# fgarciacardenas/SplaTAM

Hardware: AMD Instinct MI355X
Metric: rasterize fwd+bwd frames/sec @640×480, 300k Gaussians; HBM GB/s vs peak (higher is better)
Workload: dtype f32

## Files before the change

### include/gsr_glue.h

```cpp
#ifndef GSR_GLUE_H
#define GSR_GLUE_H

#include "gsr.h"

#ifdef __cplusplus
extern "C" {
#endif

int gsr_track_scratch_floats(int n);

int gsr_track_transform_fwd(int P, const float* means_world, const float* unnorm_rot, const float* logit_opac,
                            const float* log_scales, int scale_cols, const float* cam_q, const float* cam_t,
                            int q_stride, const float* w2c, float* means_cam, float* rotations, float* depth_colors,
                            float* opacities, float* scales, void* stream);

int gsr_track_transform_bwd(int P, const float* means_world, const float* unnorm_rot, int scale_cols,
                            const float* cam_q, const float* means_cam, const float* w2c,
                            const float* dL_dmeans_cam, const float* dL_drot, const float* dL_ddepth_colors,
                            float* dL_dcam_q, float* dL_dcam_t, int q_stride, float* scratch, void* stream);

typedef struct gsr_pose_track {
    const unsigned* status;
    unsigned capacity;
    const float* loss;
// ... 18 lines not shown
int gsr_track_l1_fwd_terms(int H, int W, const float* im, const float* depth_sil, const float* gt_im,
                           const float* gt_depth, float sil_thres, float w_im, float w_depth, float* loss,
                           float* terms, float* scratch, void* stream);
int gsr_track_l1_fwd_bwd_terms(int H, int W, const float* im, const float* depth_sil, const float* gt_im,
                               const float* gt_depth, float sil_thres, float w_im, float w_depth,
                               const float* dL_dloss, float* loss, float* terms, float* dL_dim, float* dL_ddepth_sil,
                               float* scratch, void* stream);

int gsr_track_l1_bwd(int H, int W, const float* im, const float* depth_sil, const float* gt_im,
                     const float* gt_depth, float sil_thres, float w_im, float w_depth, const float* dL_dloss,
                     float* dL_dim, float* dL_ddepth_sil, void* stream);

int gsr_track_forward_scratch_floats(int image_width, int image_height);
int gsr_track_forward_dual_static(const gsr_settings* settings, const gsr_gaussians* gaussians, const float* colors2,
                                  int capacity, unsigned* status, float* out_color, float* out_color2,
                                  float* out_depth, int* radii, const float* gt_im, const float* gt_depth,
                                  float sil_thres, float w_im, float w_depth, const float* dL_dloss, float* loss,
                                  float* dL_dim, float* dL_ddepth_sil, float* scratch, gsr_alloc_fn alloc,
                                  void* alloc_ctx, void* stream);
int gsr_track_forward_dual_static_terms(const gsr_settings* settings, const gsr_gaussians* gaussians,
                                        const float* colors2, int capacity, unsigned* status, float* out_color,
                                        float* out_color2, float* out_depth, int* radii, const float* gt_im,
                                        const float* gt_depth, float sil_thres, float w_im, float w_depth,
                                        const float* dL_dloss, float* loss, float* terms, float* dL_dim,
                                        float* dL_ddepth_sil, float* scratch, gsr_alloc_fn alloc, void* alloc_ctx,
                                        void* stream);

typedef struct gsr_track_xform {
    const float* means_world;
    const float* unnorm_rot;
    const float* logit_opac;
    const float* log_scales;
    int scale_cols;
    const float* cam_q;
    const float* cam_t;
    int q_stride;
    const float* w2c;
    int store_rendervars;
    const uint8_t* alive;
} gsr_track_xform;

int gsr_track_forward_dual_static_xf(const gsr_settings* settings, const gsr_gaussians* gaussians, float* colors2,
                                     const gsr_track_xform* xform, int capacity, unsigned* status, float* out_color,
                                     float* out_color2, float* out_depth, int* radii, const float* gt_im,
                                     const float* gt_depth, float sil_thres, float w_im, float w_depth,
                                     const float* dL_dloss, float* loss, float* dL_dim, float* dL_ddepth_sil,
                                     float* scratch, gsr_alloc_fn alloc, void* alloc_ctx, void* stream);
int gsr_track_forward_dual_static_xf_terms(const gsr_settings* settings, const gsr_gaussians* gaussians,
                                           float* colors2, const gsr_track_xform* xform, int capacity,
                                           unsigned* status, float* out_color, float* out_color2, float* out_depth,
                                           int* radii, const float* gt_im, const float* gt_depth, float sil_thres,
                                           float w_im, float w_depth, const float* dL_dloss, float* loss,
                                           float* terms, float* dL_dim, float* dL_ddepth_sil, float* scratch,
                                           gsr_alloc_fn alloc, void* alloc_ctx, void* stream);

int gsr_track_backward_scratch_floats(int P);
int gsr_track_backward_dual(const gsr_settings* settings, const gsr_gaussians* gaussians, const int* radii,
                            const float* colors2, const float* dL_dout_color, const float* dL_dout_color2,
                            int num_rendered, const void* geom_buffer, const void* binning_buffer,
                            const void* image_buffer, const float* means_world, const float* unnorm_rot,
                            int scale_cols, float* cam_q, float* cam_t, int q_stride, const float* w2c, double lr_q,
                            double lr_t, double beta1, double beta2, double eps, float* adam_state,
                            float* dL_dcam_q, float* dL_dcam_t, float* scratch, const gsr_pose_track* track,
                            const float* log_scales, gsr_alloc_fn alloc, void* alloc_ctx, void* stream);

int gsr_track_records_floats(int capacity);

int gsr_track_forward_backward_dual_static_xf(const gsr_settings* settings, const gsr_gaussians* gaussians,
                                              float* colors2, const gsr_track_xform* xform, int capacity,
                                              unsigned* status, float* out_color, float* out_color2,
                                              float* out_depth, int* radii, const float* gt_im,
                                              const float* gt_depth, float sil_thres, float w_im, float w_depth,
                                              const float* dL_dloss, float* loss, float* scratch,
                                              float* inst_records, gsr_alloc_fn alloc, void* alloc_ctx,
                                              void* stream);
int gsr_track_forward_backward_dual_static_xf_terms(const gsr_settings* settings, const gsr_gaussians* gaussians,
                                                    float* colors2, const gsr_track_xform* xform, int capacity,
                                                    unsigned* status, float* out_color, float* out_color2,
                                                    float* out_depth, int* radii, const float* gt_im,
                                                    const float* gt_depth, float sil_thres, float w_im,
                                                    float w_depth, const float* dL_dloss, float* loss, float* terms,
                                                    float* scratch, float* inst_records, gsr_alloc_fn alloc,
                                                    void* alloc_ctx, void* stream);
int gsr_track_backward_dual_records(const gsr_settings* settings, const gsr_gaussians* gaussians, const int* radii,
                                    const float* colors2, int num_rendered, const void* geom_buffer,
                                    const void* binning_buffer, const void* image_buffer, const float* means_world,
                                    const float* unnorm_rot, int scale_cols, float* cam_q, float* cam_t, int q_stride,
                                    const float* w2c, double lr_q, double lr_t, double beta1, double beta2,
                                    double eps, float* adam_state, float* dL_dcam_q, float* dL_dcam_t,
                                    float* scratch, const gsr_pose_track* track, const float* log_scales,
                                    const float* inst_records, gsr_alloc_fn alloc, void* alloc_ctx, void* stream);


int gsr_map_loss_scratch_floats(int H, int W);
int gsr_map_loss_state_floats(int H, int W);

int gsr_map_loss_fwd(int H, int W, const float* im, const float* depth_sil, const float* gt_im, const float* gt_depth,
                     float w_im, float w_depth, float* loss, float* state, float* scratch, void* stream);

int gsr_map_loss_bwd(int H, int W, const float* im, const float* depth_sil, const float* gt_im, const float* gt_depth,
                     float w_im, float w_depth, const float* dL_dloss, const float* state, float* dL_dim,
                     float* dL_ddepth_sil, void* stream);

int gsr_map_transform_bwd(int P, const float* unnorm_rot, const float* logit_opac, const float* log_scales,
                          int scale_cols, const float* cam_q, int q_stride, const float* means_cam, const float* w2c,
                          const float* dL_dmeans_cam, const float* dL_drot, const float* dL_ddepth_colors,
                          const float* dL_dopac, const float* dL_dscales, float* dL_dmeans, float* dL_dunnorm_rot,
                          float* dL_dlogit_opac, float* dL_dlog_scales, void* stream);

typedef struct gsr_map_adam {
    float* exp_avg[5];
    float* exp_avg_sq[5];
    double lr[5];
    int step;
    double beta1, beta2, eps;
    const unsigned* status;
    unsigned capacity;
    unsigned* halted;
} gsr_map_adam;

int gsr_backward_dual_sh_adam(const gsr_settings* settings, const gsr_gaussians* gaussians, const int* radii,
                              const float* colors2, const float* dL_dout_color, const float* dL_dout_color2,
                              int num_rendered, const void* geom_buffer, const void* binning_buffer,
                              const void* image_buffer, const gsr_grads* grads, float* dcolors2, int dl2_channels,
                              const gsr_map_adam* sh_adam, gsr_alloc_fn alloc, void* alloc_ctx, void* stream);

int gsr_map_transform_bwd_adam(int P, float* means_world, float* unnorm_rot, float* logit_opac, float* log_scales,
                               int scale_cols, float* colors, int color_cols, const float* cam_q, int q_stride,
                               const float* means_cam, const float* w2c, const float* dL_dmeans_cam,
                               const float* dL_drot, const float* dL_ddepth_colors, const float* dL_dopac,
                               const float* dL_dscales, const float* dL_dcolors, const gsr_map_adam* adam,
                               void* stream);

int gsr_map_prune(int P, const float* logit_opac, const float* log_scales, int scale_cols, float opac_thr,
                  float big_thr, int remove_big, unsigned char* alive, void* stream);
int gsr_forward_dual_static_alive(const gsr_settings* settings, const gsr_gaussians* gaussians, const float* colors2,
                                  int capacity, unsigned* status, float* out_color, float* out_color2,
                                  float* out_depth, int* radii, const unsigned char* alive, gsr_alloc_fn alloc,
                                  void* alloc_ctx, void* stream);
int gsr_forward_static_alive(const gsr_settings* settings, const gsr_gaussians* gaussians, int capacity,
                             unsigned* status, float* out_color, float* out_depth, int* radii,
                             const unsigned char* alive, gsr_alloc_fn alloc, void* alloc_ctx, void* stream);

int gsr_forward_dual_static_xf(const gsr_settings* settings, const gsr_gaussians* gaussians, float* colors2,
                               const gsr_track_xform* xform, int capacity, unsigned* status, float* out_color,
                               float* out_color2, float* out_depth, int* radii, gsr_alloc_fn alloc, void* alloc_ctx,
                               void* stream);

int gsr_accumulate_mean2d(int P, const int* radii, const float* dmeans2D, float* accum, float* denom,
                          float* max_2D_radius, void* stream);

typedef struct gsr_adam_tensor {
    float* param;
    const float* grad;
    float* exp_avg;
    float* exp_avg_sq;
    long long n;
    double lr;
} gsr_adam_tensor;
int gsr_adam_step(int n_tensors, const gsr_adam_tensor* tensors, int step, double beta1, double beta2, double eps,
                  void* stream);

int gsr_points_to_camera(int P, const float* means, const float* w2c, float* pts, void* stream);
int gsr_fisher_accumulate(int P, const float* dmeans3D, const float* dopacity, const float* weight, float* H,
                          void* stream);

// ... 52 lines not shown
```

### splatam_amd/_C.py

```python
from __future__ import annotations

import ctypes
import os
import threading
import weakref
from typing import NamedTuple

import torch

from ._lib import ALLOC_FN, GsrGaussians, GsrGrads, GsrSettings, GsrTrackXform, lib

_tls = threading.local()


def _alloc(ctx, kind, nbytes):
    try:
        t = torch.empty(max(int(nbytes), 1), dtype=torch.uint8, device=_tls.device)
        _tls.buffers[int(kind)] = t
        return t.data_ptr()
    except Exception as exc:
        _tls.alloc_error = exc
        return None


# ... 401 lines not shown
        if capacity > 0:
            _check_status(status, device)
            _check_alive(alive, P, device)
            static = (int(capacity), status.data_ptr())
            if xform is not None:
                _check_xform_outputs(device, means3D, colors2, opacity, scales, rotations)
                xf = xform_struct(xform)
                xf.store_rendervars, xf.alive = 1, _ptr(alive)
                fn, static = lib.gsr_forward_dual_static_xf, (ctypes.byref(xf),) + static
            elif alive is not None:
                fn, mask = lib.gsr_forward_dual_static_alive, (alive.data_ptr() if P else None,)
            else:
                fn = lib.gsr_forward_dual_static
        n, bufs = fr.call("rasterize_gaussians_dual", fn, _ptr(c2), *static, out_color.data_ptr(),
                          out_color2.data_ptr(), out_depth.data_ptr(), radii.data_ptr() if P else None, *mask)
        return (n, out_color, out_color2, radii, bufs[0], bufs[1], bufs[2], out_depth)


def rasterize_gaussians_dual_backward(background, means3D, radii, colors, colors2, scales, rotations, scale_modifier,
                                      cov3D_precomp, viewmatrix, projmatrix, tan_fovx, tan_fovy, dL_dout_color,
                                      dL_dout_color2, sh, degree, campos, geomBuffer, R, binningBuffer, imageBuffer,
                                      needs=None, dl2_channels=3, sh_adam=None, means2D_color1=False):
    if means2D_color1 and sh_adam is not None:
        raise ValueError("means2D_color1: gsr_backward_dual_sh_adam has no such sibling (step SH colours with "
                         "glue.FusedAdam)")
    device = means3D.device
    P = means3D.size(0)
    H, W = int(dL_dout_color.size(1)), int(dL_dout_color.size(2))
    M = sh.size(1) if (sh is not None and sh.numel() > 0 and sh.size(0) != 0) else 0
    f32 = dict(dtype=torch.float32, device=device)
    needs = [True] * 9 if needs is None else list(needs)
    needs[4] = True
    if sh_adam is not None:
        needs[6] = False
    shapes = [(P, 3), (P, 3), (P, 3), (P, 1), (P, 3), (P, 6), (P, M, 3), (P, 3), (P, 4)]
    res = [torch.empty(*sh_, **f32) if nd else None for sh_, nd in zip(shapes, needs)]
    out = [res[0], res[1], res[3], res[4], res[5], res[6], res[7], res[8]]
    dcolors2 = res[2]
    if P == 0:
        return (out[0], out[1], dcolors2, *out[2:])
    with torch.cuda.device(device):
        fr = _Frame(device, (background, viewmatrix, projmatrix, campos, tan_fovx, tan_fovy, H, W, scale_modifier,
                             degree, False), (means3D, sh, colors, None, scales, rotations, cov3D_precomp))
        c2 = _dev_f32(colors2, device, "colors2")
        dpix = _dev_f32(dL_dout_color, device, "dL_dout_color")
        dpix2 = _dev_f32(dL_dout_color2, device, "dL_dout_color2")
        radii_c = radii.to(device=device, dtype=torch.int32).contiguous()
        grads = GsrGrads(*[o.data_ptr() if (o is not None and o.numel() > 0) else None for o in out])
        fn, step = lib.gsr_backward_dual, ()
        if means2D_color1:
            if out[0] is None:
                raise ValueError("means2D_color1 needs dmeans2D among `needs`")
            grads.dmeans2D = None
            fn, step = lib.gsr_backward_dual_m2d, (out[0].data_ptr(),)
        if sh_adam is not None:
            if fr.keep_g[1] is None or fr.keep_g[1].data_ptr() != sh.data_ptr():
                raise RuntimeError("sh_adam steps the SH coefficients in place: sh must be contiguous float32")
            fn, step = lib.gsr_backward_dual_sh_adam, (ctypes.byref(sh_adam),)
        fr.call("rasterize_gaussians_dual_backward", fn, radii_c.data_ptr(), _ptr(c2), dpix.data_ptr(),
                dpix2.data_ptr(), *_forward_state(R, geomBuffer, binningBuffer, imageBuffer), ctypes.byref(grads),
                _ptr(dcolors2), int(dl2_channels), *step, release=True)
        return (out[0], out[1], dcolors2, *out[2:])


BINNING_CULLED, BINNING_REFERENCE = 0, 1


def binning_mode() -> int:
    return getattr(_tls, "binning", BINNING_CULLED)


class reference_binning:

    def __enter__(self):
        self.prev = binning_mode()
        _tls.binning = BINNING_REFERENCE
        return self

    def __exit__(self, *exc):
        _tls.binning = self.prev
        return False


def mark_visible(means3D, viewmatrix, projmatrix):
    device = means3D.device
    P = means3D.size(0)
    present = torch.zeros(P, dtype=torch.bool, device=device)
    if P == 0:
        return present
    with torch.cuda.device(device):
        m = _dev_f32(means3D, device, "means3D")
        v = _dev_f32(viewmatrix, device, "viewmatrix")
        p = _dev_f32(projmatrix, device, "projmatrix")
        rc = lib.gsr_mark_visible(P, m.data_ptr(), v.data_ptr(), p.data_ptr(), present.data_ptr(), _stream(device))
        _check(rc, "mark_visible")
    return present


def track_backward_dual(settings, means3D, radii, colors, colors2, scales, rotations, dL_dout_color, dL_dout_color2,
                        geomBuffer, R, binningBuffer, imageBuffer, means_world, unnorm_rot, scale_cols, cam_q_ptr,
                        cam_t_ptr, q_stride, w2c, scratch, adam=None, dq_ptr=None, dt_ptr=None, track=None,
                        log_scales=None, records=None):
    device = means3D.device
    with torch.cuda.device(device):
        fr = _Frame(device, _settings_of(settings, False), (means3D, None, colors, None, scales, rotations, None))
        c2 = _dev_f32(colors2, device, "colors2")
        lr_q, lr_t, b1, b2, eps, state = adam if adam is not None else (0.0, 0.0, 0.0, 0.0, 0.0, None)
        fn, what, images, rec = lib.gsr_track_backward_dual, "track_backward_dual", (), ()
        if records is not None:
            fn, what, rec = lib.gsr_track_backward_dual_records, "track_backward_dual_records", (records.data_ptr(),)
        else:
            dpix = _dev_f32(dL_dout_color, device, "dL_dout_color")
            dpix2 = _dev_f32(dL_dout_color2, device, "dL_dout_color2")
            images = (dpix.data_ptr(), dpix2.data_ptr())
        fr.call(what, fn, radii.data_ptr(), _ptr(c2), *images,
                *_forward_state(R, geomBuffer, binningBuffer, imageBuffer), means_world.data_ptr(),
                unnorm_rot.data_ptr(), int(scale_cols), cam_q_ptr, cam_t_ptr, int(q_stride), w2c.data_ptr(),
                float(lr_q), float(lr_t), float(b1), float(b2), float(eps), _ptr(state), dq_ptr, dt_ptr,
                scratch.data_ptr(), ctypes.byref(track) if track is not None else None, _ptr(log_scales), *rec,
                release=True)


def terms_ptr(terms: torch.Tensor, device) -> int:
    if (not torch.is_tensor(terms) or terms.device != device or terms.dtype != torch.float32 or
            terms.numel() != 2 or not terms.is_contiguous()):
        raise RuntimeError("terms: a contiguous float32 tensor of 2 elements on the forward's device")
    return terms.data_ptr()


def track_forward_dual_static(settings, means3D, colors, colors2, opacity, scales, rotations, capacity, status, gt_im,
                              gt_depth, sil_thres, w_im, w_depth, seed, scratch, xform=None, records=None,
                              images=True, terms=None):
    st = settings
    device = means3D.device
    P = means3D.size(0)
    H, W = int(st.image_height), int(st.image_width)
    f32 = dict(dtype=torch.float32, device=device)
    if records is not None and xform is None:
        raise RuntimeError("track_forward_dual_static: records needs the transform-fused forward (xform)")
    if not images and records is None:
        raise RuntimeError("track_forward_dual_static: images=False needs the fused render (xform and records)")
    with torch.cuda.device(device):
        fr = _Frame(device, _settings_of(st, st.prefiltered), (means3D, None, colors, opacity, scales, rotations, None))
        c2 = _dev_f32(colors2, device, "colors2")
        gi, gd, sd = (_dev_f32(gt_im, device, "gt_im"), _dev_f32(gt_depth, device, "gt_depth"),
                      _dev_f32(seed, device, "seed"))
        out_color = out_color2 = out_depth = None
        if images:
            out_color, out_color2 = torch.empty(3, H, W, **f32), torch.empty(3, H, W, **f32)
            out_depth = torch.empty(1, H, W, **f32)
        radii = torch.empty(P, dtype=torch.int32, device=device)
        loss = torch.empty((), **f32)
        _check_status(status, device)
        name, xf, dim, dds = "gsr_track_forward_dual_static", (), None, None
        if xform is not None:
            _check_xform_outputs(device, means3D, colors2, opacity, scales, rotations)
            _check_alive(xform.alive, P, device)
            xf_struct = xform_struct(xform)
            name, xf = name + "_xf", (ctypes.byref(xf_struct),)
        if records is not None:
            if (records.device != device or records.dtype != torch.float32 or not records.is_contiguous() or
                    records.numel() < lib.gsr_track_records_floats(int(capacity))):
                raise RuntimeError("records: contiguous float32 of gsr_track_records_floats(capacity) on the device")
            name = "gsr_track_forward_backward_dual_static_xf"
            tail = (scratch.data_ptr(), records.data_ptr())
        else:
            dim, dds = torch.empty(3, H, W, **f32), torch.empty(3, H, W, **f32)
            tail = (dim.data_ptr(), dds.data_ptr(), scratch.data_ptr())
        tp = () if terms is None else (terms_ptr(terms, device),)
        n, bufs = fr.call(name[4:], getattr(lib, name + "_terms" if tp else name), _ptr(c2), *xf, int(capacity),
                          status.data_ptr(), _ptr(out_color), _ptr(out_color2), _ptr(out_depth),
                          radii.data_ptr() if P else None, gi.data_ptr(), gd.data_ptr(), float(sil_thres),
                          float(w_im), float(w_depth), sd.data_ptr(), loss.data_ptr(), *tp, *tail)
        return (n, out_color, out_color2, radii, bufs[0], bufs[1], bufs[2], out_depth, loss, dim, dds)
```

### splatam_amd/_lib.py

```python
from __future__ import annotations

import ctypes
import os

_HERE = os.path.dirname(os.path.abspath(__file__))
LIB_PATH = os.environ.get("GSR_LIB", os.path.join(_HERE, "libgsr.so"))

c_int, c_float, c_void_p, c_size_t = ctypes.c_int, ctypes.c_float, ctypes.c_void_p, ctypes.c_size_t
c_double = ctypes.c_double


class GsrSettings(ctypes.Structure):
    _fields_ = [("image_height", c_int), ("image_width", c_int), ("tan_fovx", c_float), ("tan_fovy", c_float),
                ("bg", c_void_p), ("scale_modifier", c_float), ("viewmatrix", c_void_p), ("projmatrix", c_void_p),
                ("sh_degree", c_int), ("campos", c_void_p), ("prefiltered", c_int), ("binning", c_int)]


class GsrGaussians(ctypes.Structure):
    _fields_ = [("P", c_int), ("M", c_int), ("means3D", c_void_p), ("shs", c_void_p), ("colors_precomp", c_void_p),
                ("opacities", c_void_p), ("scales", c_void_p), ("rotations", c_void_p), ("cov3D_precomp", c_void_p)]


class GsrGrads(ctypes.Structure):
    _fields_ = [("dmeans2D", c_void_p), ("dcolors", c_void_p), ("dopacity", c_void_p), ("dmeans3D", c_void_p),
# ... 30 lines not shown
                             c_void_p, c_void_p, c_void_p, c_int, ctypes.POINTER(GsrGrads), ALLOC_FN, c_void_p,
                             c_void_p]),
    "gsr_forward_dual": (c_int, [ctypes.POINTER(GsrSettings), ctypes.POINTER(GsrGaussians), c_void_p, c_void_p,
                                 c_void_p, c_void_p, c_void_p, ALLOC_FN, c_void_p, c_void_p]),
    "gsr_forward_static": (c_int, [ctypes.POINTER(GsrSettings), ctypes.POINTER(GsrGaussians), c_int, c_void_p,
                                   c_void_p, c_void_p, c_void_p, ALLOC_FN, c_void_p, c_void_p]),
    "gsr_forward_dual_static": (c_int, [ctypes.POINTER(GsrSettings), ctypes.POINTER(GsrGaussians), c_void_p, c_int,
                                        c_void_p, c_void_p, c_void_p, c_void_p, c_void_p, ALLOC_FN, c_void_p,
                                        c_void_p]),
    "gsr_backward_dual": (c_int, [ctypes.POINTER(GsrSettings), ctypes.POINTER(GsrGaussians), c_void_p, c_void_p,
                                  c_void_p, c_void_p, c_int, c_void_p, c_void_p, c_void_p, ctypes.POINTER(GsrGrads),
                                  c_void_p, c_int, ALLOC_FN, c_void_p, c_void_p]),
    "gsr_backward_dual_m2d": (c_int, [ctypes.POINTER(GsrSettings), ctypes.POINTER(GsrGaussians), c_void_p, c_void_p,
                                      c_void_p, c_void_p, c_int, c_void_p, c_void_p, c_void_p,
                                      ctypes.POINTER(GsrGrads), c_void_p, c_int, c_void_p, ALLOC_FN, c_void_p,
                                      c_void_p]),
    "gsr_forward_reuse": (c_int, [ctypes.POINTER(GsrSettings), ctypes.POINTER(GsrGaussians), c_int, c_void_p,
                                  c_void_p, c_void_p, c_void_p, c_void_p, c_void_p, c_void_p, ALLOC_FN, c_void_p,
                                  c_void_p]),
    "gsr_forward_reuse_if_equal": (c_int, [ctypes.POINTER(GsrSettings), ctypes.POINTER(GsrGaussians), c_int,
                                           c_void_p, c_void_p, c_void_p, c_int, c_void_p, c_void_p, c_void_p,
                                           c_void_p, c_void_p, c_void_p, c_void_p, c_void_p, ALLOC_FN, c_void_p,
                                           c_void_p]),
    "gsr_bitwise_equal": (c_int, [c_int, c_void_p, c_void_p, c_void_p, c_void_p, c_void_p]),
    "gsr_mark_visible": (c_int, [c_int, c_void_p, c_void_p, c_void_p, c_void_p, c_void_p]),
    "gsr_geom_buffer_bytes": (c_size_t, [c_int]),
    "gsr_geom_counters_offset": (c_size_t, [c_int]),
    "gsr_binning_buffer_bytes": (c_size_t, [c_int, c_int, c_int]),
    "gsr_image_buffer_bytes": (c_size_t, [c_int, c_int]),
    "gsr_last_error": (ctypes.c_char_p, []),
    "gsr_abi_version": (c_int, []),
    "gsr_selftest_reduce9": (c_int, [c_void_p, c_void_p, c_void_p]),
    "gsr_timing_enable": (c_int, [c_int]),
    "gsr_timing_read": (c_int, [c_void_p, c_void_p, c_void_p, c_int]),
    "gsr_track_scratch_floats": (c_int, [c_int]),
    "gsr_track_transform_fwd": (c_int, [c_int, c_void_p, c_void_p, c_void_p, c_void_p, c_int, c_void_p, c_void_p,
                                        c_int, c_void_p, c_void_p, c_void_p, c_void_p, c_void_p, c_void_p, c_void_p]),
    "gsr_track_transform_bwd": (c_int, [c_int, c_void_p, c_void_p, c_int, c_void_p, c_void_p, c_void_p, c_void_p,
                                        c_void_p, c_void_p, c_void_p, c_void_p, c_int, c_void_p, c_void_p]),
    "gsr_track_transform_bwd_adam": (c_int, [c_int, c_void_p, c_void_p, c_int, c_void_p, c_void_p, c_int, c_void_p,
                                             c_void_p, c_void_p, c_void_p, c_void_p, c_double, c_double,
                                             c_double, c_double, c_double, c_void_p, c_void_p,
                                             ctypes.POINTER(GsrPoseTrack), c_void_p]),
    "gsr_track_l1_fwd": (c_int, [c_int, c_int, c_void_p, c_void_p, c_void_p, c_void_p, ctypes.c_float,
                                 ctypes.c_float, ctypes.c_float, c_void_p, c_void_p, c_void_p]),
    "gsr_track_l1_bwd": (c_int, [c_int, c_int, c_void_p, c_void_p, c_void_p, c_void_p, ctypes.c_float,
                                 ctypes.c_float, ctypes.c_float, c_void_p, c_void_p, c_void_p, c_void_p]),
    "gsr_track_l1_fwd_bwd": (c_int, [c_int, c_int, c_void_p, c_void_p, c_void_p, c_void_p, ctypes.c_float,
                                     ctypes.c_float, ctypes.c_float, c_void_p, c_void_p, c_void_p, c_void_p,
                                     c_void_p, c_void_p]),
    "gsr_track_forward_scratch_floats": (c_int, [c_int, c_int]),
    "gsr_track_forward_dual_static": (c_int, [ctypes.POINTER(GsrSettings), ctypes.POINTER(GsrGaussians), c_void_p,
                                              c_int, c_void_p, c_void_p, c_void_p, c_void_p, c_void_p, c_void_p,
                                              c_void_p, c_float, c_float, c_float, c_void_p, c_void_p, c_void_p,
                                              c_void_p, c_void_p, ALLOC_FN, c_void_p, c_void_p]),
    "gsr_track_forward_dual_static_xf": (c_int, [ctypes.POINTER(GsrSettings), ctypes.POINTER(GsrGaussians), c_void_p,
                                                 ctypes.POINTER(GsrTrackXform), c_int, c_void_p, c_void_p, c_void_p,
                                                 c_void_p, c_void_p, c_void_p, c_void_p, c_float, c_float, c_float,
                                                 c_void_p, c_void_p, c_void_p, c_void_p, c_void_p, ALLOC_FN, c_void_p,
                                                 c_void_p]),
    "gsr_track_l1_fwd_terms": (c_int, [c_int, c_int, c_void_p, c_void_p, c_void_p, c_void_p, ctypes.c_float,
                                       ctypes.c_float, ctypes.c_float, c_void_p, c_void_p, c_void_p, c_void_p]),
    "gsr_track_l1_fwd_bwd_terms": (c_int, [c_int, c_int, c_void_p, c_void_p, c_void_p, c_void_p, ctypes.c_float,
                                           ctypes.c_float, ctypes.c_float, c_void_p, c_void_p, c_void_p, c_void_p,
                                           c_void_p, c_void_p, c_void_p]),
    "gsr_track_forward_dual_static_terms": (c_int, [ctypes.POINTER(GsrSettings), ctypes.POINTER(GsrGaussians),
                                                    c_void_p, c_int, c_void_p, c_void_p, c_void_p, c_void_p, c_void_p,
                                                    c_void_p, c_void_p, c_float, c_float, c_float, c_void_p, c_void_p,
                                                    c_void_p, c_void_p, c_void_p, c_void_p, ALLOC_FN, c_void_p,
                                                    c_void_p]),
    "gsr_track_forward_dual_static_xf_terms": (c_int, [ctypes.POINTER(GsrSettings), ctypes.POINTER(GsrGaussians),
                                                       c_void_p, ctypes.POINTER(GsrTrackXform), c_int, c_void_p,
                                                       c_void_p, c_void_p, c_void_p, c_void_p, c_void_p, c_void_p,
                                                       c_float, c_float, c_float, c_void_p, c_void_p, c_void_p,
                                                       c_void_p, c_void_p, c_void_p, ALLOC_FN, c_void_p, c_void_p]),
    "gsr_track_forward_backward_dual_static_xf_terms": (c_int, [ctypes.POINTER(GsrSettings),
                                                                ctypes.POINTER(GsrGaussians), c_void_p,
                                                                ctypes.POINTER(GsrTrackXform), c_int, c_void_p,
                                                                c_void_p, c_void_p, c_void_p, c_void_p, c_void_p,
                                                                c_void_p, c_float, c_float, c_float, c_void_p,
                                                                c_void_p, c_void_p, c_void_p, c_void_p, ALLOC_FN,
                                                                c_void_p, c_void_p]),
    "gsr_track_records_floats": (c_int, [c_int]),
    "gsr_track_forward_backward_dual_static_xf": (c_int, [ctypes.POINTER(GsrSettings), ctypes.POINTER(GsrGaussians),
                                                          c_void_p, ctypes.POINTER(GsrTrackXform), c_int, c_void_p,
                                                          c_void_p, c_void_p, c_void_p, c_void_p, c_void_p, c_void_p,
                                                          c_float, c_float, c_float, c_void_p, c_void_p, c_void_p,
                                                          c_void_p, ALLOC_FN, c_void_p, c_void_p]),
    "gsr_track_backward_dual_records": (c_int, [ctypes.POINTER(GsrSettings), ctypes.POINTER(GsrGaussians), c_void_p,
                                                c_void_p, c_int, c_void_p, c_void_p, c_void_p, c_void_p, c_void_p,
                                                c_int, c_void_p, c_void_p, c_int, c_void_p, c_double, c_double,
                                                c_double, c_double, c_double, c_void_p, c_void_p, c_void_p, c_void_p,
                                                ctypes.POINTER(GsrPoseTrack), c_void_p, c_void_p, ALLOC_FN, c_void_p,
                                                c_void_p]),
    "gsr_backward_dual_sh_adam": (c_int, [ctypes.POINTER(GsrSettings), ctypes.POINTER(GsrGaussians), c_void_p,
                                          c_void_p, c_void_p, c_void_p, c_int, c_void_p, c_void_p, c_void_p,
                                          ctypes.POINTER(GsrGrads), c_void_p, c_int, ctypes.POINTER(GsrMapAdam),
                                          ALLOC_FN, c_void_p, c_void_p]),
    "gsr_track_backward_scratch_floats": (c_int, [c_int]),
    "gsr_track_backward_dual": (c_int, [ctypes.POINTER(GsrSettings), ctypes.POINTER(GsrGaussians), c_void_p, c_void_p,
                                        c_void_p, c_void_p, c_int, c_void_p, c_void_p, c_void_p, c_void_p, c_void_p,
                                        c_int, c_void_p, c_void_p, c_int, c_void_p, c_double, c_double, c_double,
                                        c_double, c_double, c_void_p, c_void_p, c_void_p, c_void_p,
                                        ctypes.POINTER(GsrPoseTrack), c_void_p, ALLOC_FN, c_void_p, c_void_p]),
    "gsr_map_loss_scratch_floats": (c_int, [c_int, c_int]),
    "gsr_map_loss_state_floats": (c_int, [c_int, c_int]),
    "gsr_map_loss_fwd": (c_int, [c_int, c_int, c_void_p, c_void_p, c_void_p, c_void_p, c_float, c_float, c_void_p,
                                 c_void_p, c_void_p, c_void_p]),
    "gsr_map_loss_bwd": (c_int, [c_int, c_int, c_void_p, c_void_p, c_void_p, c_void_p, c_float, c_float, c_void_p,
                                 c_void_p, c_void_p, c_void_p, c_void_p]),
    "gsr_map_transform_bwd": (c_int, [c_int, c_void_p, c_void_p, c_void_p, c_int, c_void_p, c_int, c_void_p,
                                      c_void_p, c_void_p, c_void_p, c_void_p, c_void_p, c_void_p, c_void_p, c_void_p,
                                      c_void_p, c_void_p, c_void_p]),
    "gsr_map_transform_bwd_adam": (c_int, [c_int, c_void_p, c_void_p, c_void_p, c_void_p, c_int, c_void_p, c_int,
                                           c_void_p, c_int, c_void_p, c_void_p, c_void_p, c_void_p, c_void_p,
                                           c_void_p, c_void_p, c_void_p, ctypes.POINTER(GsrMapAdam), c_void_p]),
    "gsr_adam_step": (c_int, [c_int, ctypes.POINTER(GsrAdamTensor), c_int, c_double, c_double, c_double, c_void_p]),
    "gsr_map_prune": (c_int, [c_int, c_void_p, c_void_p, c_int, c_float, c_float, c_int, c_void_p, c_void_p]),
    "gsr_forward_dual_static_alive": (c_int, [ctypes.POINTER(GsrSettings), ctypes.POINTER(GsrGaussians), c_void_p,
                                              c_int, c_void_p, c_void_p, c_void_p, c_void_p, c_void_p, c_void_p,
                                              ALLOC_FN, c_void_p, c_void_p]),
    "gsr_forward_static_alive": (c_int, [ctypes.POINTER(GsrSettings), ctypes.POINTER(GsrGaussians), c_int, c_void_p,
                                         c_void_p, c_void_p, c_void_p, c_void_p, ALLOC_FN, c_void_p, c_void_p]),
    "gsr_forward_dual_static_xf": (c_int, [ctypes.POINTER(GsrSettings), ctypes.POINTER(GsrGaussians), c_void_p,
                                           ctypes.POINTER(GsrTrackXform), c_int, c_void_p, c_void_p, c_void_p,
                                           c_void_p, c_void_p, ALLOC_FN, c_void_p, c_void_p]),
    "gsr_accumulate_mean2d": (c_int, [c_int, c_void_p, c_void_p, c_void_p, c_void_p, c_void_p, c_void_p]),
    "gsr_points_to_camera": (c_int, [c_int, c_void_p, c_void_p, c_void_p, c_void_p]),
    "gsr_fisher_accumulate": (c_int, [c_int, c_void_p, c_void_p, c_void_p, c_void_p, c_void_p]),
    "gsr_silhouette_count": (c_int, [ctypes.POINTER(GsrSettings), c_int, c_int, c_void_p, c_void_p, c_void_p, c_float,
                                     c_void_p, c_void_p]),
    "gsr_fisher_score_workspace_bytes": (c_size_t, []),
    "gsr_fisher_score": (c_int, [c_int, c_void_p, c_void_p, c_void_p, c_void_p, c_void_p, c_void_p, c_void_p]),
    "gsr_keyframe_workspace_bytes": (c_size_t, [c_int, c_int]),
    "gsr_keyframe_select": (c_int, [c_int, c_int, c_void_p, c_float, c_float, c_float, c_float, c_void_p, c_void_p,
                                    c_int, c_int, c_int, c_void_p, c_void_p, c_int, c_void_p, c_void_p,
                                    ctypes.c_longlong, c_int, c_void_p, c_void_p, c_void_p, c_void_p, c_void_p,
                                    c_void_p, c_void_p, c_void_p, c_void_p]),
    "gsr_eval_workspace_bytes": (c_size_t, [c_int, c_int, c_int]),
    "gsr_eval_frame": (c_int, [c_int, c_int, c_void_p, c_void_p, c_void_p, c_void_p, c_float, c_int, c_int, c_void_p,
                               c_void_p, c_void_p]),
    "gsr_densify_workspace_bytes": (c_size_t, [c_int, c_int]),
    "gsr_densify_frame": (c_int, [c_int, c_int, c_void_p, c_void_p, c_void_p, c_float, c_float, c_float, c_float,
                                  c_void_p, c_float, c_int, c_void_p, c_void_p, c_void_p, c_void_p, c_void_p,
                                  c_void_p, c_void_p, c_void_p, c_void_p, c_void_p, c_void_p, c_void_p]),
    "gsr_densify_frame_capped": (c_int, [c_int, c_int, c_void_p, c_void_p, c_void_p, c_float, c_float, c_float,
                                         c_float, c_void_p, c_float, c_int, c_void_p, c_void_p, c_void_p, c_void_p,
                                         c_void_p, c_void_p, c_void_p, c_void_p, c_void_p, c_void_p, c_void_p,
                                         c_void_p, c_int, c_float, c_float]),
    "gsr_init_frame": (c_int, [c_int, c_int, c_void_p, c_void_p, c_float, c_float, c_float, c_float, c_void_p, c_int,
                               c_void_p, c_void_p, c_void_p, c_void_p, c_void_p, c_void_p, c_void_p, c_void_p,
                               c_void_p, c_void_p, c_void_p, c_void_p]),
    "gsr_resize_frame": (c_int, [c_int, c_int, c_void_p, c_void_p, c_int, c_int, c_void_p, c_void_p, c_int, c_int,
                                 c_void_p, c_void_p, c_void_p]),
    "gsr_ingest_frame": (c_int, [c_int, c_int, c_void_p, c_void_p, c_double, c_int, c_float, c_void_p, c_void_p,
                                 c_int, c_int, c_void_p, c_void_p, c_int, c_int, c_void_p, c_void_p, c_void_p]),
}


def load(path: str = LIB_PATH) -> ctypes.CDLL:
    if not os.path.exists(path):
        raise ImportError(f"libgsr.so not found at {path}: build it with `python -m splatam_amd.build` "
                          "(no CPU fallback exists for the rasterizer)")
    lib = ctypes.CDLL(path)
    ab = os.environ.get("GSR_LIB_AB") == "1" and bool(os.environ.get("GSR_LIB"))
    for name, (res, args) in SIGNATURES.items():
# ... 16 lines not shown
```

### splatam_amd/csrc/gsr_backward.hip

```cpp
#include <cstdlib>

#include "gsr_chain.h"
#include "gsr_clock.h"
#include "gsr_diag.h"
#include "gsr_dispatch.h"
#include "gsr_glue_common.h"
#include "gsr_launch.h"
#include "gsr_layout.h"
#include "gsr_math.h"
#include "gsr_render_bwd.h"
#include "gsr_render_fwd.h"
#include "gsr_wave.h"

namespace gsr {

__global__ void __launch_bounds__(TILE_PIX, GSR_BWD_M2D_WAVES)
render_bwd_m2d_kernel(Camera cam, const uint2* __restrict__ ranges, const PointEntry* __restrict__ point_list,
                      const float4* __restrict__ rr, const uint32_t* __restrict__ blocksums,
                      const float* __restrict__ final_T, const uint32_t* __restrict__ n_contrib,
                      const float* __restrict__ dL_dpix, const float* __restrict__ dL_dpix2, float* __restrict__ inst,
                      BwdGuard guard, unsigned long long* clk) {
    using V = MapM2dVariant;
    kclock_begin(clk);
    RenderDiag dg;
    dg.begin();
    if (guard.overflow()) {
        kclock_end(clk);
        return;
    }
    __shared__ __attribute__((aligned(16))) char smem[BwdShape<V>::bytes];
    const int tid = threadIdx.x;
    const int tile = sched_tile(cam), tx = tile % cam.gx, ty = tile / cam.gx;
    dg.tile(tile);
    const int px = tx * TILE_X + tile_px(tid);
    const int py = ty * TILE_Y + tile_py(tid);
    BwdPix pin{0.f, 0u, 0.f, 0.f, 0.f, 0.f, 0.f, 0.f};
    load_bwd_pix<V::DUAL, V::Q2>(pin, cam, px, py, final_T, n_contrib, dL_dpix, dL_dpix2);
    bwd_tile<V>(cam, tile, pin, ranges, point_list, rr, blocksums, inst, guard, smem, dg);
    dg.end();
    kclock_end(clk);
}

constexpr size_t track_lds_bytes() {
    return FwdShape<true>::bytes > BwdShape<TrackVariant>::bytes ? FwdShape<true>::bytes : BwdShape<TrackVariant>::bytes;
}
template <bool IMAGES>
__global__ void __launch_bounds__(TILE_PIX, 5)
render_track_kernel(Camera cam, const uint2* __restrict__ ranges, PointEntry* __restrict__ point_list,
                    uint64_t* __restrict__ keys, const float4* __restrict__ rr, const uint32_t* __restrict__ blocksums,
                    float* __restrict__ final_T, uint32_t* __restrict__ n_contrib, float* __restrict__ out_color,
                    float* __restrict__ out_color2, float* __restrict__ out_depth, SpecGuard guard,
                    unsigned long long* clk, TrackL1 l1, float* __restrict__ inst) {
    kclock_begin(clk);
    RenderDiag dg;
    dg.begin();
    if (guard.overflow()) {
        kclock_end(clk);
        return;
    }
    __shared__ __attribute__((aligned(16))) char smem[track_lds_bytes()];
    if constexpr (!IMAGES) {
        final_T = nullptr;
        cam.rowmax = nullptr;
    }
    const int tile = sched_tile(cam);
    dg.tile(tile);
    const FwdPix f = fwd_tile<true>(cam, tile, ranges, point_list, keys, rr, guard, smem, dg);
    float grad[4];
    constexpr bool kStoreGrads = false;
    static_assert(!kStoreGrads, "render_track_kernel's callers pass no gradient images");
    fwd_epilogue<true, true, kStoreGrads>(cam, tile, f, final_T, n_contrib, out_color, out_color2, out_depth, l1,
                                          grad);
    __syncthreads();
    const BwdPix pin{f.T, f.last16 >> 4, grad[0], grad[1], grad[2], grad[3], 0.f, 0.f};
    Camera cb = cam;
    cb.rowmax = nullptr;
    bwd_tile<TrackVariant>(cb, tile, pin, ranges, point_list, rr, blocksums, inst,
                           BwdGuard{guard.counters, guard.cap_inst}, smem, dg);
    dg.end();
    kclock_end(clk);
}

int track_records_stride() { return BwdShape<TrackVariant>::RS; }

hipError_t launch_render_track(const Camera& cam, const uint2* ranges, uint64_t* point_list, uint64_t* keys,
                               GeomPtrs geo, float* final_T, uint32_t* n_contrib, float* out_color,
                               float* out_color2, float* out_depth, SpecGuard guard, const TrackL1& l1, float* inst,
                               hipStream_t s, unsigned long long* clk) {
    auto k = final_T != nullptr ? render_track_kernel<true> : render_track_kernel<false>;
    hipLaunchKernelGGL(k, dim3(cam.gx * cam.gy), dim3(TILE_PIX), 0, s, cam, ranges, point_list,
                       keys, geo.rr, geo.blocksums, final_T, n_contrib, out_color, out_color2, out_depth, guard, clk,
                       l1, inst);
    return hipGetLastError();
}

struct BwdTerms {
    bool op, c1, c2;
    int q2;
};
static BwdTerms bwd_terms(unsigned need, bool dual) {
    return {(need & NEED_OPACITY) != 0, (need & NEED_COLORS) != 0, dual && (need & NEED_COLORS2),
            (dual && (need & NEED_DL2_CH0_ONLY)) ? 1 : 3};
}

RecLayout bwd_rec_layout(unsigned need, bool dual) {
    const auto [op, c1, c2, q2] = bwd_terms(need, dual);
    return rec_sums(op, c1, c2, q2).rec;
}

using RenderBwdFn = decltype(render_bwd_of<TrackVariant>());
struct PickRenderBwd {
    template <bool DUAL, bool OP, bool C1, bool C2, bool Q1>
    RenderBwdFn operator()() const {
        if constexpr (!DUAL && (C2 || Q1)) return nullptr;
        else return render_bwd_of<BwdVariant<DUAL, OP, C1, C2, Q1 ? 1 : 3>>();
    }
};

hipError_t launch_render_bwd(const Camera& cam, const uint2* ranges, const uint64_t* point_list, GeomPtrs geo,
                             const float* final_T, const uint32_t* n_contrib, const float* dL_dpix,
                             const float* colors2, const float* dL_dpix2, unsigned need, float* inst,
                             BwdGuard guard, hipStream_t s, unsigned long long* clk) {
    const auto [op, c1, c2, q2] = bwd_terms(need, colors2 != nullptr);
    const auto k = dispatch_bools(PickRenderBwd{}, colors2 != nullptr, op, c1, c2, q2 == 1);
    hipLaunchKernelGGL(k, dim3(cam.gx * cam.gy), dim3(TILE_PIX), 0, s, cam, ranges, point_list, geo.rr, geo.blocksums,
                       final_T, n_contrib, dL_dpix, dL_dpix2, inst, guard, clk);
    return hipGetLastError();
}

int m2d_record_stride() { return BwdShape<MapM2dVariant>::RS; }
static_assert(BwdShape<MapM2dVariant>::O_M1 == M2D_REC_PAIR && BwdShape<MapM2dVariant>::NV == M2D_REC_PAIR + 2 &&
                  BwdShape<MapM2dVariant>::RS <= INST_REC_MAX,
              "the M2D1 record: the mapping variant's ten sums, then the pair");

hipError_t launch_render_bwd_m2d(const Camera& cam, const uint2* ranges, const uint64_t* point_list, GeomPtrs geo,
                                 const float* final_T, const uint32_t* n_contrib, const float* dL_dpix,
                                 const float* dL_dpix2, float* inst, BwdGuard guard, hipStream_t s,
                                 unsigned long long* clk) {
    hipLaunchKernelGGL(render_bwd_m2d_kernel, dim3(cam.gx * cam.gy), dim3(TILE_PIX), 0, s, cam, ranges, point_list,
                       geo.rr, geo.blocksums, final_T, n_contrib, dL_dpix, dL_dpix2, inst, guard, clk);
    return hipGetLastError();
}

template <bool POSE, bool SHL, bool M2D1 = false>
__device__ __forceinline__ void gauss_bwd_body(Camera cam, GaussIn g, GeomPtrs geo, const int* __restrict__ radii,
                                               const float* __restrict__ inst, RecLayout rec, GradsOut out,
                                               BwdGuard guard, PoseFuse pf, M2dOut m1 = M2dOut{}) {
    static_assert(!M2D1 || !POSE, "M2D1: the mapping backward only");
    if constexpr (!SHL) {
        g.shs = nullptr;
        g.M = 0;
    }
    const int i = blockIdx.x * blockDim.x + threadIdx.x;
    if (!POSE && i >= g.P) return;
    const bool live = i < g.P;
    const int nsh = g.shs ? (cam.sh_degree + 1) * (cam.sh_degree + 1) : 0;
    float g2[9] = {0.f, 0.f, 0.f, 0.f, 0.f, 0.f, 0.f, 0.f, 0.f};
    float dcol2[3] = {0.f, 0.f, 0.f};
    [[maybe_unused]] float m2d1[2] = {0.f, 0.f};
    float dmean[3] = {0.f, 0.f, 0.f}, dcov[6] = {0.f, 0.f, 0.f, 0.f, 0.f, 0.f}, dscale[3] = {0.f, 0.f, 0.f},
          drot[4] = {0.f, 0.f, 0.f, 0.f};
    float dsh[48];
#pragma unroll
    for (int k = 0; k < 48; k++) dsh[k] = 0.f;
    GaussGeom gg;
    gg.m = make_float3(0.f, 0.f, 0.f);
    gg.s = make_float3(0.f, 0.f, 0.f);
    gg.q = make_float4(0.f, 0.f, 0.f, 0.f);
    const int rad = live ? radii[i] : 0;
    const bool xf_geom = POSE && pf.ls;
    TrackXf x;
    x.mw = pf.means_world; x.ur = pf.unnorm_rot; x.ls = pf.ls; x.scols = pf.scols;
    XfRaw xr{};
    if (xf_geom && live) xr = track_xform_load(x, i, false);
    uint32_t off = 0, cnt = 0, tl = 0xFFFFFFFFu;
    if (POSE && live && rad > 0) {
        off = geo.offsets[i];
        cnt = geo.tiles[i];
        tl = reinterpret_cast<const uint32_t*>(geo.bin)[4 * (size_t)i + 3];
    }
    __shared__ Pose s_pose;
    if constexpr (POSE) {
        if (pf.ls || pf.scols != 1) {
            if (threadIdx.x == 0) s_pose = make_pose(pf.cam_q, pf.cam_t, pf.qs);
            __syncthreads();
        }
    }
    if (live && (POSE || rad > 0)) {
        if (xf_geom) {
            const Pose ps = s_pose;
            float m[3], sv[3];
            track_xform_geom_raw(xr, x.scols, ps, m, gg.q, sv);
            gg.m = make_float3(m[0], m[1], m[2]);
            gg.s = make_float3(sv[0], sv[1], sv[2]);
        } else {
            gg = load_geom(g, i);
        }
    }
    if (live && rad > 0 && !guard.overflow()) {
        if (!POSE) {
            off = geo.offsets[i];
            cnt = geo.tiles[i];
            tl = reinterpret_cast<const uint32_t*>(geo.bin)[4 * (size_t)i + 3];
        }
        float acc[INST_REC_MAX];
#pragma unroll
        for (int m = 0; m < INST_REC_MAX; m++) acc[m] = 0.f;
        const int np = rec.stride / 2;
        constexpr int RU = 4;
// ... 258 lines not shown
```

### splatam_amd/csrc/gsr_binning.hip

```cpp
#include "gsr_clock.h"
#include "gsr_dispatch.h"
#include "gsr_launch.h"
#include "gsr_layout.h"
#include "gsr_wave.h"

namespace gsr {

constexpr int SCAN_THREADS = 1024;
constexpr int SCAN_ITEMS = 4;

template <bool AGENT_TILES>
__device__ void scan_counts_body(const uint32_t* __restrict__ wgsum, uint32_t* __restrict__ blocksums, uint32_t nb,
                                 const uint32_t* __restrict__ tile_count, uint32_t tile_stride, uint32_t ntiles,
                                 uint2* __restrict__ ranges, uint32_t* __restrict__ counters, uint32_t sort_cap,
                                 uint32_t* __restrict__ status) {
    __shared__ uint32_t wsums[SCAN_THREADS / 64];
    __shared__ uint32_t s_carry, s_max, s_viol;
    const int tid = threadIdx.x, lane = tid & 63, w = tid >> 6;
    if (tid == 0) s_viol = 0;
    for (int pass = 0; pass < 2; pass++) {
        const uint32_t n = pass == 0 ? nb : ntiles;
        const uint32_t* src = pass == 0 ? wgsum : tile_count;
        if (tid == 0) { s_carry = 0; s_max = 0; }
        __syncthreads();
        uint32_t vmax = 0, viol = 0;
        for (uint32_t base = 0; base < n; base += SCAN_THREADS * SCAN_ITEMS) {
            uint32_t x[SCAN_ITEMS], sum = 0;
            const uint32_t i0 = base + (uint32_t)tid * SCAN_ITEMS;
#pragma unroll
            for (int k = 0; k < SCAN_ITEMS; k++) {
                const uint32_t* ps = src + (size_t)(i0 + k) * (pass == 0 ? 1u : tile_stride);
                x[k] = (i0 + k < n) ? ((AGENT_TILES && pass == 1) ? ld_agent(ps) : *ps) : 0u;
                if (pass == 0) {
                    viol |= x[k] >> 31;
                    x[k] &= 0x7fffffffu;
                }
                sum += x[k];
                vmax = max(vmax, x[k]);
            }
            uint32_t incl = wave_incl_scan(sum);
            if (lane == 63) wsums[w] = incl;
            __syncthreads();
            if (w == 0) {
                uint32_t ws = (lane < SCAN_THREADS / 64) ? wsums[lane] : 0u;
                uint32_t wi = wave_incl_scan(ws);
                if (lane < SCAN_THREADS / 64) wsums[lane] = wi - ws;
            }
            __syncthreads();
            uint32_t run = s_carry + wsums[w] + incl - sum;
#pragma unroll
            for (int k = 0; k < SCAN_ITEMS; k++) {
                if (i0 + k < n) {
                    if (pass == 0) blocksums[i0 + k] = run;
                    else ranges[i0 + k] = make_uint2(run, run + x[k]);
                }
                run += x[k];
            }
            __syncthreads();
            if (tid == SCAN_THREADS - 1) s_carry = run;
            __syncthreads();
        }
        atomicMax(&s_max, vmax);
        if (viol) atomicOr(&s_viol, 1u);
        __syncthreads();
        if (tid == 0) {
            if (pass == 0) {
                counters[0] = s_carry;
                counters[1] = s_viol;
                if (status) status_merge(status, s_carry, s_viol, 0u, 0u);
            } else {
                counters[2] = s_max;
                counters[3] = sort_cap;
                if (status) status_merge(status, 0u, 0u, s_max, sort_cap);
            }
        }
        __syncthreads();
    }
}

__global__ void __launch_bounds__(SCAN_THREADS)
scan_counts_kernel(const uint32_t* __restrict__ wgsum, uint32_t* __restrict__ blocksums, uint32_t nb,
                   const uint32_t* __restrict__ tile_count,
                   uint32_t tile_stride, uint32_t ntiles, uint2* __restrict__ ranges,
                   uint32_t* __restrict__ counters, uint32_t sort_cap, uint32_t* __restrict__ status) {
    scan_counts_body<false>(wgsum, blocksums, nb, tile_count, tile_stride, ntiles, ranges, counters, sort_cap, status);
}
// ... 31 lines not shown
    const bool in_regs = rq <= CS_RQ;
    if (t < ntiles) {
        if (in_regs) {
#pragma unroll
            for (int k = 0; k < CS_RQ; k++) {
                vals[k] = b0 + k < b1 ? counts[(size_t)(b0 + k) * ntiles + t] : 0u;
                sum += vals[k];
            }
        } else {
#pragma unroll 4
            for (int b = b0; b < b1; b++) sum += counts[(size_t)b * ntiles + t];
        }
    }
    s_part[q][tl] = sum;
    __syncthreads();
    {
        static_assert(CS_PARTS == 64 || CS_PARTS == 32, "one or two tile columns per wave");
        constexpr int CPW = 64 / CS_PARTS;
        const int w = threadIdx.x >> 6, lane = threadIdx.x & 63;
        const int part = lane % CS_PARTS, colw = CPW * w + lane / CS_PARTS;
        const uint32_t v = s_part[part][colw];
        uint32_t inc = wave_incl_scan(v);
        if (CPW == 2) {
            const uint32_t lo_tot = (uint32_t)__shfl((int)inc, 31);
            if (lane >= 32) inc -= lo_tot;
        }
        s_part[part][colw] = inc - v;
    }
    __syncthreads();
    uint32_t run = s_part[q][tl];
    if (t < ntiles) {
        if (in_regs) {
#pragma unroll
            for (int k = 0; k < CS_RQ; k++)
                if (b0 + k < b1) {
                    counts[(size_t)(b0 + k) * ntiles + t] = run;
                    run += vals[k];
                }
        } else {
#pragma unroll 4
            for (int b = b0; b < b1; b++) {
                const uint32_t v = counts[(size_t)b * ntiles + t];
                counts[(size_t)b * ntiles + t] = run;
                run += v;
            }
        }
        if (q == CS_PARTS - 1) {
            if (TAIL) st_agent(&tot[t], run);
            else tot[t] = run;
        }
    }
    if (!TAIL) return;
    if (!last_block_arrive(&geo.counters[4])) return;
    scan_counts_body<true>(geo.wgsum, geo.blocksums, (uint32_t)nb, tot, 1u, (uint32_t)ntiles, ranges, geo.counters,
                           sort_cap, status);
}
template <bool TAIL, int CT, bool CLK>
__global__ void __launch_bounds__(CS_THREADS)
tile_colscan_kernel(uint32_t* __restrict__ counts, int nb, int ntiles, uint32_t* __restrict__ tot, GeomPtrs geo,
                    uint2* __restrict__ ranges, uint32_t sort_cap, uint32_t* __restrict__ status,
                    unsigned long long* clk, Gate gate) {
    if (gate.off()) return;
    if constexpr (CLK) kclock_begin(clk);
    tile_colscan_body<TAIL, CT>(counts, nb, ntiles, tot, geo, ranges, sort_cap, status);
    if constexpr (CLK) kclock_end(clk);
}

struct PickTileColscan {
    template <bool TAIL, bool WIDE, bool CLK>
    auto operator()() const { return &tile_colscan_kernel<TAIL, WIDE ? 32 : 16, CLK>; }
};

hipError_t launch_tile_colscan(uint32_t* counts, int nb, int ntiles, uint32_t* tot, GeomPtrs geo, uint2* ranges,
                               uint32_t* status, bool tail, hipStream_t s, unsigned long long* clk, Gate gate) {
    static_assert(CS_THREADS == SCAN_THREADS, "the last colscan workgroup runs the scan body");
    const bool wide = nb > CS_ROWS_SMALL;
    const int ct = wide ? 32 : 16;
    const auto k = dispatch_bools(PickTileColscan{}, tail, wide, clk != nullptr);
    hipLaunchKernelGGL(k, dim3((ntiles + ct - 1) / ct), dim3(CS_THREADS), 0, s, counts, nb, ntiles, tot, geo, ranges,
                       (uint32_t)TILE_SORT_CAP, status, clk, gate);
    return hipGetLastError();
}

constexpr int PLAN_BUCKETS = 1024, PLAN_SHIFT = 2;
__device__ __forceinline__ uint32_t plan_bucket(uint32_t len) {
    return (uint32_t)(PLAN_BUCKETS - 1) - min(len >> PLAN_SHIFT, (uint32_t)(PLAN_BUCKETS - 1));
}
__device__ __forceinline__ uint32_t plan_slot(uint32_t p, uint32_t n, uint32_t ncu) {
    const uint32_t q = n / ncu, m = n - q * ncu, heavy = q * (ncu - m);
    const bool hv = p < heavy;
    const uint32_t g0 = hv ? m : 0u, gs = hv ? ncu - m : m, pp = hv ? p : p - heavy;
    const uint32_t rd = pp / gs, k = pp - rd * gs;
    return rd * ncu + g0 + ((rd & 1u) ? gs - 1u - k : k);
}
template <int NT, int TPT = 0>
__device__ void tile_plan(const uint32_t* __restrict__ tot, int ntiles, int ncu, uint32_t* __restrict__ order,
                          uint32_t* s_hist, uint32_t* s_wsum, const uint32_t* tv = nullptr, int t0 = 0,
                          int t1 = 0) {
    constexpr int BPT = PLAN_BUCKETS / NT;
    static_assert(BPT * NT == PLAN_BUCKETS, "buckets per thread");
    const int tid = threadIdx.x, lane = tid & 63, w = tid >> 6;
#pragma unroll
    for (int k = 0; k < BPT; k++) s_hist[tid * BPT + k] = 0u;
    __syncthreads();
    if constexpr (TPT > 0) {
#pragma unroll
        for (int k = 0; k < TPT; k++)
            if (t0 + k < t1) atomicAdd(&s_hist[plan_bucket(tv[k])], 1u);
    } else {
        for (int u = tid; u < ntiles; u += NT) atomicAdd(&s_hist[plan_bucket(tot[u])], 1u);
    }
    __syncthreads();
    uint32_t c[BPT], cs = 0;
#pragma unroll
    for (int k = 0; k < BPT; k++) {
        c[k] = s_hist[tid * BPT + k];
        cs += c[k];
    }
    const uint32_t incl = wave_incl_scan(cs);
    if (lane == 63) s_wsum[w] = incl;
    __syncthreads();
    uint32_t run = incl - cs;
    for (int k = 0; k < w; k++) run += s_wsum[k];
#pragma unroll
    for (int k = 0; k < BPT; k++) {
        s_hist[tid * BPT + k] = run;
        run += c[k];
    }
    __syncthreads();
    if constexpr (TPT > 0) {
#pragma unroll
        for (int k = 0; k < TPT; k++)
            if (t0 + k < t1) {
                const uint32_t p = atomicAdd(&s_hist[plan_bucket(tv[k])], 1u);
                order[plan_slot(p, (uint32_t)ntiles, (uint32_t)ncu)] = (uint32_t)(t0 + k);
            }
    } else {
        for (int u = tid; u < ntiles; u += NT) {
            const uint32_t p = atomicAdd(&s_hist[plan_bucket(tot[u])], 1u);
            order[plan_slot(p, (uint32_t)ntiles, (uint32_t)ncu)] = (uint32_t)u;
        }
    }
}

__global__ void identity_order_kernel(uint32_t* __restrict__ order, int n) {
    const int i = blockIdx.x * blockDim.x + threadIdx.x;
    if (i < n) order[i] = (uint32_t)i;
}
hipError_t launch_identity_order(uint32_t* order, int ntiles, hipStream_t s) {
    if (ntiles <= 0) return hipSuccess;
    hipLaunchKernelGGL(identity_order_kernel, dim3((ntiles + 255) / 256), dim3(256), 0, s, order, ntiles);
    return hipGetLastError();
}

constexpr int DUP_T = 512;
#ifndef GSR_DUP_LOOP_MAX
#define GSR_DUP_LOOP_MAX 16
#endif
__device__ __forceinline__ void store_host_snap(uint32_t* snap, uint4 lo, uint4 hi) {
    reinterpret_cast<uint4*>(snap)[0] = lo;
    reinterpret_cast<uint4*>(snap)[1] = hi;
}
__device__ __forceinline__ void dup_gate_off_snap(const Camera& cam, const GeomPtrs& geo) {
    if (cam.host_snap && blockIdx.x == 0 && threadIdx.x == 0)
        store_host_snap(cam.host_snap, *reinterpret_cast<const uint4*>(geo.counters),
                        *reinterpret_cast<const uint4*>(geo.counters + 4));
}
template <bool LDS_HIST, int DUP_G, bool EXACT>
__device__ __forceinline__ void duplicate_bucket_body(Camera cam, int P, GeomPtrs geo, uint2* __restrict__ ranges,
                                                      const uint32_t* __restrict__ tot, uint32_t* __restrict__ cursor,
                                                      int ntiles, uint64_t* __restrict__ keys,
                                                      uint64_t* __restrict__ point_list, SpecGuard guard,
                                                      uint32_t sort_cap, uint32_t* __restrict__ status,
                                                      uint32_t* __restrict__ s_cur) {
    constexpr int ROW = DUP_G * DUP_T;
    __shared__ uint32_t s_incl[ROW];
    __shared__ uint32_t s_x0[ROW], s_y0[ROW], s_w[ROW], s_depth[ROW], s_live[ROW];
    __shared__ uint32_t s_cx[EXACT ? ROW : 1];
    __shared__ uint32_t wsum[DUP_T / 64], s_tmax[DUP_T / 64], s_cws[DUP_T / 64];
    __shared__ uint32_t s_cred[2][DUP_T / 64];
    const int tid = threadIdx.x, lane = tid & 63, w = tid >> 6;
    const int i0 = blockIdx.x * ROW + DUP_G * tid;
    uint32_t t[DUP_G];
    uint4 r[DUP_G];
#pragma unroll
    for (int g = 0; g < DUP_G; g++) {
        t[g] = (i0 + g < P) ? geo.tiles[i0 + g] : 0u;
        r[g] = (i0 + g < P) ? geo.bin[i0 + g] : make_uint4(0u, 0u, 0u, 0u);
    }
    uint32_t base, ctail = 0, ltot = 0xFFFFFFFFu;
    if (LDS_HIST) {
        constexpr int TPT = 4;
        __shared__ uint32_t s_red[5][DUP_T / 64];
        const uint32_t b = blockIdx.x, nb = gridDim.x;
        const int per = (ntiles + DUP_T - 1) / DUP_T;
        const int t0 = min(ntiles, tid * per), t1 = min(ntiles, t0 + per);
        const bool in_regs = per <= TPT;
        uint32_t tv[TPT], cv[TPT];
#pragma unroll
        for (int k = 0; k < TPT; k++) {
            const bool ok = in_regs && t0 + k < t1;
            tv[k] = ok ? tot[t0 + k] : 0u;
            cv[k] = ok ? cursor[(size_t)b * ntiles + t0 + k] : 0u;
        }
        uint32_t pre = 0, all = 0, viol = 0, vmax = 0, cpre = 0, call = 0;
        for (uint32_t k = tid; k < nb; k += 2 * DUP_T) {
            const uint32_t k2 = k + DUP_T;
            const uint32_t v = geo.wgsum[k], v2 = k2 < nb ? geo.wgsum[k2] : 0u;
            const uint32_t c = EXACT ? geo.wgcull[k] : 0u, c2 = (EXACT && k2 < nb) ? geo.wgcull[k2] : 0u;
            viol |= (v | v2) >> 31;
            all += (v & 0x7fffffffu) + (v2 & 0x7fffffffu);
            pre += (k < b ? (v & 0x7fffffffu) : 0u) + (k2 < b ? (v2 & 0x7fffffffu) : 0u);
            if (EXACT) {
                call += c + c2;
                cpre += (k < b ? c : 0u) + (k2 < b ? c2 : 0u);
            }
        }
        uint32_t csum = 0;
        if (in_regs) {
#pragma unroll
            for (int k = 0; k < TPT; k++) {
                csum += tv[k];
                vmax = max(vmax, tv[k]);
            }
        } else {
            for (int u = t0; u < t1; u++) {
                const uint32_t v = tot[u];
// ... 254 lines not shown
```

### splatam_amd/csrc/gsr_capi.hip

```cpp
#include <cstdio>
#include <cstdlib>
#include <cstring>
#include <algorithm>
#include <atomic>
#include <string>

#include "../../include/gsr.h"
#include "../../include/gsr_glue.h"
#include "gsr_adam.h"
#include "gsr_errors.h"
#include "gsr_host.h"
#include "gsr_launch.h"
#include "gsr_layout.h"

using namespace gsr;

namespace {
thread_local std::string g_last_error;

__global__ void zero_words_kernel(uint32_t* __restrict__ p, size_t n) {
    for (size_t k = blockIdx.x * (size_t)blockDim.x + threadIdx.x; k < n; k += (size_t)gridDim.x * blockDim.x) p[k] = 0u;
}
std::atomic<int> g_cus[kMaxDevices];
}

namespace gsr {
int fail(int code, const std::string& msg) {
    g_last_error = msg;
    return code;
}

int hip_fail(hipError_t e, const char* where) {
    return fail(GSR_ERR_HIP, std::string(where) + ": " + hipGetErrorString(e));
}

int check_terms(const char* entry, const float* terms) {
    if (!terms) return fail(GSR_ERR_INVALID_ARG, std::string(entry) + ": null terms");
    if ((uintptr_t)terms % sizeof(float) != 0)
        return fail(GSR_ERR_INVALID_ARG, std::string(entry) + ": terms must be 4-byte aligned");
    return GSR_OK;
}

int stream_device(hipStream_t s) {
    thread_local hipStream_t last_s = nullptr;
    thread_local int last_d = -1;
    if (last_d >= 0 && s == last_s && s != nullptr) return last_d;
    int d = 0;
    if (hipStreamGetDevice(s, &d) != hipSuccess && hipGetDevice(&d) != hipSuccess) d = 0;
    (void)hipGetLastError();
    if (d < 0 || d >= kMaxDevices) d = 0;
    last_s = s;
    last_d = d;
    return d;
}
int current_device() {
    int d = 0;
    if (hipGetDevice(&d) != hipSuccess || d < 0 || d >= kMaxDevices) d = 0;
    return d;
}
int device_cus(int dev) {
    int n = g_cus[dev].load(std::memory_order_relaxed);
    if (n > 0) return n;
    if (hipDeviceGetAttribute(&n, hipDeviceAttributeMultiprocessorCount, dev) != hipSuccess || n <= 0) n = 256;
    (void)hipGetLastError();
    g_cus[dev].store(n, std::memory_order_relaxed);
    return n;
}
hipError_t zero_async(void* p, size_t bytes, hipStream_t s) {
    const size_t n = bytes / 4;
    if (n == 0) return hipSuccess;
    const unsigned blocks = (unsigned)std::min<size_t>(1024, (n + 255) / 256);
    hipLaunchKernelGGL(zero_words_kernel, dim3(blocks), dim3(256), 0, s, (uint32_t*)p, n);
    return hipGetLastError();
}
int geom_pre_shift(int P) { return pre_shift_for(P, device_cus(current_device())); }
int current_device_cus() { return device_cus(current_device()); }
}

namespace {

struct Pinned {
    uint32_t* p = nullptr;
    uint32_t* dp = nullptr;
    hipEvent_t ev = nullptr;
    ~Pinned() {
        if (p) (void)hipHostFree(p);
        if (ev) (void)hipEventDestroy(ev);
    }
    int ensure(int dev) {
        hipError_t e;
        if (!p) {
            if ((e = hipHostMalloc((void**)&p, 32,
                                   hipHostMallocMapped | hipHostMallocCoherent | hipHostMallocPortable)) != hipSuccess)
                return hip_fail(e, "hipHostMalloc");
            if ((e = hipHostGetDevicePointer((void**)&dp, p, 0)) != hipSuccess)
// ... 33 lines not shown
    c.bg = s->bg;
    c.scale_modifier = s->scale_modifier;
    c.sh_degree = s->sh_degree;
    c.prefiltered = s->prefiltered;
    return c;
}

GaussIn make_gauss(const gsr_gaussians* g) {
    GaussIn o;
    o.P = g->P;
    o.M = g->shs ? g->M : 0;
    o.means3D = g->means3D;
    o.shs = (g->shs && g->M > 0) ? g->shs : nullptr;
    o.colors = g->colors_precomp;
    o.opacities = g->opacities;
    o.scales = g->scales;
    o.rotations = g->rotations;
    o.cov3D = g->cov3D_precomp;
    o.colors2 = nullptr;
    o.sh_staged = 0;
    o.alive = nullptr;
    return o;
}

int validate(const gsr_settings* s, const gsr_gaussians* g, bool forward) {
    if (!s || !g) return fail(GSR_ERR_INVALID_ARG, "null settings or gaussians");
    if (g->P < 0) return fail(GSR_ERR_INVALID_ARG, "P must be >= 0");
    if (s->binning != GSR_BINNING_CULLED && s->binning != GSR_BINNING_REFERENCE)
        return fail(GSR_ERR_INVALID_ARG, "settings.binning must be GSR_BINNING_CULLED or GSR_BINNING_REFERENCE");
    if (s->image_width <= 0 || s->image_height <= 0) return fail(GSR_ERR_INVALID_ARG, "image size must be positive");
    if (s->image_width > 16 * 65535 || s->image_height > 16 * 65535)
        return fail(GSR_ERR_INVALID_ARG, "image too large for 16-bit tile coordinates");
    if (g->P == 0) return GSR_OK;
    if (!g->means3D) return fail(GSR_ERR_INVALID_ARG, "means3D is required");
    if (forward && !g->opacities) return fail(GSR_ERR_INVALID_ARG, "opacities are required");
    if (!s->viewmatrix || !s->projmatrix || !s->bg) return fail(GSR_ERR_INVALID_ARG, "camera matrices / bg missing");
    const bool has_sh = g->shs && g->M > 0;
    if (!g->colors_precomp && !has_sh)
        return fail(GSR_ERR_INVALID_ARG, "Please provide excatly one of either SHs or precomputed colors!");
    if (!g->colors_precomp && !s->campos) return fail(GSR_ERR_INVALID_ARG, "campos required for SH colours");
    if (has_sh && (s->sh_degree < 0 || s->sh_degree > 3 || (s->sh_degree + 1) * (s->sh_degree + 1) > g->M))
        return fail(GSR_ERR_INVALID_ARG, "sh_degree must be in [0,3] with (deg+1)^2 <= M");
    const bool has_sr = g->scales && g->rotations;
    if (!has_sr && !g->cov3D_precomp)
        return fail(GSR_ERR_INVALID_ARG,
                    "Please provide exactly one of either scale/rotation pair or precomputed 3D covariance!");
    return GSR_OK;
}

template <class T>
int obtain(gsr_alloc_fn alloc, void* ctx, int kind, size_t bytes, const char* what, T** out) {
    *out = (T*)alloc(ctx, kind, bytes);
    return *out ? GSR_OK : fail(GSR_ERR_ALLOC, std::string("allocator returned NULL (") + what + ")");
}

struct ReuseIn {
    EqualPairs pairs;
    int prev_num_rendered;
    const void* prev_geom;
    void* prev_binning;
    void* prev_image;
    const int* prev_radii;
    int* reused;
};

struct FwdCall {
    const gsr_settings* settings = nullptr;
    const gsr_gaussians* gaussians = nullptr;
    const float* colors2 = nullptr;
    float* out_color = nullptr;
    float* out_color2 = nullptr;
    float* out_depth = nullptr;
    int* radii = nullptr;
    gsr_alloc_fn alloc = nullptr;
    void* alloc_ctx = nullptr;
    void* stream = nullptr;
    int capacity = 0;
    uint32_t* status = nullptr;
    const TrackL1* l1 = nullptr;
    const TrackXf* xf = nullptr;
    float* track_inst = nullptr;
    const uint8_t* alive = nullptr;
    const ReuseIn* reuse = nullptr;
};

FwdCall fwd_call(const gsr_settings* settings, const gsr_gaussians* gaussians, float* out_color, float* out_depth,
                 int* radii, gsr_alloc_fn alloc, void* alloc_ctx, void* stream) {
    FwdCall c;
    c.settings = settings; c.gaussians = gaussians;
    c.out_color = out_color; c.out_depth = out_depth; c.radii = radii;
    c.alloc = alloc; c.alloc_ctx = alloc_ctx; c.stream = stream;
    return c;
}
FwdCall& dual(FwdCall& c, const float* colors2, float* out_color2) {
    c.colors2 = colors2; c.out_color2 = out_color2;
    return c;
}
FwdCall& statics(FwdCall& c, int capacity, uint32_t* status) {
    c.capacity = capacity; c.status = status;
    return c;
}

bool stores_no_images(const FwdCall& c) { return c.track_inst && !c.out_color && !c.out_color2 && !c.out_depth; }

int check_forward(const FwdCall& c) {
    const int rc = validate(c.settings, c.gaussians, true);
    if (c.track_inst && (!c.l1 || !c.colors2 || c.capacity <= 0))
        return fail(GSR_ERR_INVALID_ARG, "the fused render backward needs the static dual forward with the L1 loss");
    if (rc != GSR_OK) return rc;
    if (!c.alloc) return fail(GSR_ERR_INVALID_ARG, "allocator callback required");
    if (!stores_no_images(c)) {
        if (!c.out_color || !c.out_depth) return fail(GSR_ERR_INVALID_ARG, "output image pointers required");
        if (c.colors2 && !c.out_color2) return fail(GSR_ERR_INVALID_ARG, "out_color2 required with colors2");
    }
    if (c.colors2 && c.gaussians->P > 0 && !c.gaussians->means3D)
        return fail(GSR_ERR_INVALID_ARG, "means3D is required");
    return GSR_OK;
}

struct Forward {
    const FwdCall& c;
    hipStream_t stream;
    int dev;
    Pinned& pin;
    Camera cam;
    GaussIn g;
    int P, W, H, ntiles;
    GeomLayout GL;
    ImgLayout IL;
    void* geom = nullptr;
    GeomPtrs geo{};
    ImgPtrs img{};
    uint32_t* cursor = nullptr;
    bool lds_hist;
    uint32_t* cmat = nullptr;
    uint32_t* tile_tot = nullptr;
    bool force_radix;
    bool scan_in_duplicate;
    bool eager;
    bool gated = false;
    Gate eq_gate;
    uint32_t epoch = 0;
    uint32_t cap = 0;

    static bool force_radix_env() {
        static const bool on = getenv("GSR_FORCE_RADIX") && atoi(getenv("GSR_FORCE_RADIX")) != 0;
        return on;
    }
    explicit Forward(const FwdCall& call)
        : c(call), stream((hipStream_t)call.stream), dev(stream_device(stream)), pin(g_pinned[dev]),
          cam(make_camera(call.settings)), g(make_gauss(call.gaussians)), P(g.P), W(cam.W), H(cam.H),
          ntiles(cam.gx * cam.gy), GL(GeomLayout::make(P)), IL(ImgLayout::make(W, H)),
          lds_hist(ntiles <= MAX_LDS_TILES), force_radix(force_radix_env() && call.capacity <= 0),
          scan_in_duplicate(lds_hist && !force_radix), eager(call.capacity <= 0) {
        g.colors2 = c.colors2;
        g.alive = c.alive;
        if (c.xf) g.xf = *c.xf;
        cam.pre_shift = GL.shift;
        cam.cull = c.settings->binning != GSR_BINNING_REFERENCE ? 1 : 0;
        cam.tail_exact = eager ? 1 : 0;
    }
    uint32_t* status() const { return eager ? nullptr : c.status; }
    template <class T>
    int obtain(int kind, size_t bytes, const char* what, T** out) {
        return ::obtain(c.alloc, c.alloc_ctx, kind, bytes, what, out);
    }
// ... 53 lines not shown
            return hip_fail(e, "geometry comparison");
        cam.gate = Gate{word, epoch, 1u};
        eq_gate = Gate{word, epoch, 0u};
        if ((e = launch_reuse_copy(eq_gate, c.reuse->prev_geom, geom, GL.counters, GL.tiles, g.colors,
                                   c.reuse->prev_radii, c.radii, P, stream)) != hipSuccess)
            return hip_fail(e, "geometry reuse");
        return GSR_OK;
    }

    int snapshot_counters(bool stored_by_kernel) {
        if (int rc = pin.ensure(dev)) return rc;
        hipError_t e;
        if (!stored_by_kernel &&
            (e = hipMemcpyAsync(pin.p, geo.counters, 32, hipMemcpyDeviceToHost, stream)) != hipSuccess)
            return hip_fail(e, "copy num_rendered");
        if ((e = hipEventRecord(pin.ev, stream)) != hipSuccess) return hip_fail(e, "record num_rendered");
        return GSR_OK;
    }

    int counts_and_ranges() {
        hipError_t e;
        if (!scan_in_duplicate && (e = launch_identity_order(img.order, ntiles, stream)) != hipSuccess)
            return hip_fail(e, "render schedule");
        if (!c.radii) return fail(GSR_ERR_INVALID_ARG, "radii output required");
        {
            StageTimer t(GSR_STAGE_PREPROCESS, P, stream, true);
            if (sh_staged(cam, g)) {
                if ((e = launch_sh_eval(cam, g, geo, stream)) != hipSuccess) return hip_fail(e, "sh_eval");
                g.sh_staged = 1;
            }
            if ((e = launch_preprocess(cam, g, geo, c.radii, lds_hist ? cmat : img.tile_count, lds_hist, ntiles,
                                       GL.nb, stream, t.kclock())) != hipSuccess)
                return hip_fail(e, "preprocess");
        }
        {
            StageTimer t(GSR_STAGE_RANGES, ntiles, stream, lds_hist);
            if (lds_hist) {
                if ((e = launch_tile_colscan(cmat, GL.nb, ntiles, tile_tot, geo, img.ranges, status(),
                                             !scan_in_duplicate, stream, t.kclock(), cam.gate)) != hipSuccess)
                    return hip_fail(e, "tile count scan");
            } else if ((e = launch_scan_counts(geo, GL.nb, img.tile_count, TILE_CTR_STRIDE, ntiles, img.ranges,
                                               status(), stream)) != hipSuccess) {
                return hip_fail(e, "scan");
            }
        }
        if (eager && !scan_in_duplicate) return snapshot_counters(false);
        return GSR_OK;
    }

    int render(const BinPtrs& bin, uint64_t* keys, const SpecGuard& guard, long long units) {
        StageTimer t(GSR_STAGE_RENDER_FWD, units, stream, true);
        hipError_t e;
        if (c.track_inst) {
            if ((e = launch_render_track(cam, img.ranges, bin.point_list, keys, geo,
                                         stores_no_images(c) ? nullptr : img.final_T, img.n_contrib, c.out_color,
                                         c.out_color2, c.out_depth, guard, *c.l1, c.track_inst, stream,
                                         t.kclock())) != hipSuccess)
                return hip_fail(e, "render (fused tracking forward + backward)");
        } else if ((e = launch_render_fwd(cam, img.ranges, bin.point_list, keys, geo, c.colors2, img.final_T,
                                          img.n_contrib, c.out_color, c.out_color2, c.out_depth, guard, stream,
                                          t.kclock(), c.l1)) != hipSuccess) {
            return hip_fail(e, "render");
        }
        return GSR_OK;
    }

    int duplicate_render(const BinPtrs& bin, const SpecGuard& guard, uint32_t* host_snap, bool snapshot,
                         long long units) {
        Camera cplan = cam;
        cplan.tile_order_out = scan_in_duplicate ? img.order : nullptr;
        cplan.host_snap = host_snap;
        {
            StageTimer t(GSR_STAGE_DUPLICATE, P, stream, true);
            hipError_t e = launch_duplicate_bucket(cplan, P, geo, img.ranges, tile_tot, lds_hist ? cmat : cursor,
                                                   lds_hist, ntiles, bin.keys[0], bin.point_list, GL.nb, guard,
                                                   status(), stream, t.kclock());
            if (e != hipSuccess) return hip_fail(e, "duplicate");
        }
        if (snapshot)
            if (int rc = snapshot_counters(host_snap != nullptr)) return rc;
        return render(bin, bin.keys[0], guard, units);
    }

    int speculate() {
        void* buf;
        if (int rc = obtain(GSR_BUF_BINNING, BinLayout::make((int)cap, W, H).total, "binning buffer", &buf)) return rc;
        const BinPtrs bin = BinPtrs::at(buf, BinLayout::make((int)cap, W, H));
        const bool snapshot = eager && scan_in_duplicate;
        const bool dup_snap = snapshot && !g_snap_copy;
        if (dup_snap)
            if (int rc = pin.ensure(dev)) return rc;
        const SpecGuard guard{geo.counters, cap, (uint32_t)TILE_SORT_CAP};
        if (int rc = duplicate_render(bin, guard, dup_snap ? pin.dp : nullptr, snapshot, 0)) return rc;
        if (gated) {
            Camera cr = cam;
            cr.gate = eq_gate;
            const ImgPtrs prev = ImgPtrs::at(c.reuse->prev_image, IL);
            bind_schedule(cr, prev, dev);
            const SpecGuard rg{geo.counters, (uint32_t)c.reuse->prev_num_rendered, 0xFFFFFFFFu};
            hipError_t e = launch_render_fwd(cr, prev.ranges, (uint64_t*)c.reuse->prev_binning, nullptr, geo, nullptr,
                                             prev.final_T, prev.n_contrib, c.out_color, nullptr, c.out_depth, rg,
                                             stream);
            if (e != hipSuccess) return hip_fail(e, "render (geometry reuse)");
        }
        return GSR_OK;
    }

    int radix_binning(const BinPtrs& bin, const BinLayout& BL, uint32_t I) {
        hipError_t e;
        if ((e = hipMemsetD32Async((hipDeviceptr_t)(geo.counters + 3), 0xffffffffu, 1, stream)) != hipSuccess)
            return hip_fail(e, "sort path flag");
        {
            StageTimer t(GSR_STAGE_DUPLICATE, P, stream);
            if ((e = launch_duplicate(cam, P, geo, bin.keys[0], bin.gid, GL.nb, stream)) != hipSuccess)
                return hip_fail(e, "duplicate");
        }
        {
            StageTimer t(GSR_STAGE_SORT, I, stream);
            uint64_t* keys[2] = {bin.keys[0], bin.keys[1]};
            uint32_t* vals[2] = {bin.vals[0], bin.vals[1]};
            if ((e = launch_radix_sort(keys, vals, bin.hist, I, BL.nsb, BL.npass, stream)) != hipSuccess)
                return hip_fail(e, "radix sort");
        }
        StageTimer t(GSR_STAGE_RANGES, I, stream);
        if ((e = launch_gather_ids(bin.vals[BL.final_buf], bin.gid, bin.point_list, I, stream)) != hipSuccess)
            return hip_fail(e, "gather ids");
        return GSR_OK;
    }

    int wait_and_finish() {
        hipError_t e;
        if ((e = hipEventSynchronize(pin.ev)) != hipSuccess) return hip_fail(e, "sync num_rendered");
        if (gated && pin.p[5] != epoch) {
            *c.reuse->reused = 1;
            return c.reuse->prev_num_rendered;
        }
        const uint32_t I = pin.p[0];
        const uint32_t longest = pin.p[2];
        if (pin.p[1] != 0)
            return fail(GSR_ERR_PREFILTERED, "Point is filtered although prefiltered is set. This shouldn't happen!");
        if (I > 0x7fffffffu) return fail(GSR_ERR_INVALID_ARG, "num_rendered overflows int32");
        g_inst_ratio[dev].v.store(std::max(0.05, (double)I / P), std::memory_order_relaxed);
        if (!force_radix && I <= cap && longest <= (uint32_t)TILE_SORT_CAP) {
            g_timing_units(dev, GSR_STAGE_SORT, I);
            g_timing_units(dev, GSR_STAGE_RENDER_FWD, I);
            return (int)I;
        }
        const BinLayout BL = BinLayout::make((int)I, W, H);
        void* buf;
        if (int rc = obtain(GSR_BUF_BINNING, BL.total, "binning buffer", &buf)) return rc;
        const BinPtrs bin = BinPtrs::at(buf, BL);
        const SpecGuard none{geo.counters, 0xffffffffu, 0xffffffffu};
        int rc;
        if (I > 0 && longest <= (uint32_t)TILE_SORT_CAP && !force_radix) {
            rc = duplicate_render(bin, none, nullptr, false, I);
        } else {
            rc = I > 0 ? radix_binning(bin, BL, I) : GSR_OK;
            if (rc == GSR_OK) rc = render(bin, nullptr, none, I);
        }
        return rc != GSR_OK ? rc : (int)I;
    }
};

int forward_impl(const FwdCall& c) {
    if (int rc = check_forward(c)) return rc;
    Forward F(c);
    if (int rc = F.setup_buffers()) return rc;
    if (F.P == 0) return F.empty_map();
    int rc;
    if ((rc = F.gate_on_comparison()) != GSR_OK || (rc = F.counts_and_ranges()) != GSR_OK) return rc;
    const double ratio = g_inst_ratio[F.dev].v.load(std::memory_order_relaxed);
    F.cap = F.eager ? (uint32_t)std::min(2.0e9, std::max(1024.0, 1.5 * ratio * F.P)) : (uint32_t)c.capacity;
    if (!F.force_radix && (rc = F.speculate()) != GSR_OK) return rc;
    if (!F.eager) return (int)F.cap;
    return F.wait_and_finish();
}

struct BwdCall {
    const gsr_settings* settings = nullptr;
    const gsr_gaussians* gaussians = nullptr;
    const int* radii = nullptr;
    const float* dL_dout_color = nullptr;
    const float* colors2 = nullptr;
    const float* dL_dout_color2 = nullptr;
    int num_rendered = 0;
    const void* geom_buffer = nullptr;
    const void* binning_buffer = nullptr;
    const void* image_buffer = nullptr;
    int power = 1;
    const gsr_grads* grads = nullptr;
    float* dcolors2 = nullptr;
    int dl2_channels = 3;
    gsr_alloc_fn alloc = nullptr;
    void* alloc_ctx = nullptr;
    void* stream = nullptr;
    const PoseFuse* pose = nullptr;
    const ShAdam* sh_adam = nullptr;
    const float* pre_inst = nullptr;
    float* dmeans2D_c1 = nullptr;
};

BwdCall bwd_call(const gsr_settings* settings, const gsr_gaussians* gaussians, const int* radii, int num_rendered,
                 const void* geom_buffer, const void* binning_buffer, const void* image_buffer) {
    BwdCall c;
    c.settings = settings; c.gaussians = gaussians; c.radii = radii; c.num_rendered = num_rendered;
    c.geom_buffer = geom_buffer; c.binning_buffer = binning_buffer; c.image_buffer = image_buffer;
    return c;
}
BwdCall& on(BwdCall& c, gsr_alloc_fn alloc, void* alloc_ctx, void* stream) {
    c.alloc = alloc; c.alloc_ctx = alloc_ctx; c.stream = stream;
    return c;
}

struct Backward {
    const BwdCall& c;
    hipStream_t stream;
    Camera cam;
    GaussIn g;
    int P, R;
    GeomPtrs geo{};
    ImgPtrs img{};
    const uint64_t* point_list = nullptr;
    GradsOut out;
    BwdGuard guard{};

    explicit Backward(const BwdCall& call)
        : c(call), stream((hipStream_t)call.stream), cam(make_camera(call.settings)),
          g(make_gauss(call.gaussians)), P(g.P), R(call.num_rendered),
          out{c.grads->dmeans2D, c.grads->dcolors, c.grads->dopacity, c.grads->dmeans3D,
              c.grads->dcov3D,   c.grads->dsh,     c.grads->dscales,  c.grads->drotations} {}

    void bind_forward_state() {
        const GeomLayout GL = GeomLayout::make(P);
        cam.pre_shift = GL.shift;
        geo = GeomPtrs::at(const_cast<void*>(c.geom_buffer), GL);
        img = ImgPtrs::at(const_cast<void*>(c.image_buffer), ImgLayout::make(cam.W, cam.H));
        bind_schedule(cam, img, current_device());
        if (c.binning_buffer)
            point_list = (const uint64_t*)((const char*)c.binning_buffer + BinLayout::make(R, cam.W, cam.H).point_list);
        guard = BwdGuard{geo.counters, (uint32_t)R};
    }

    int power_scratch(size_t bytes, char** scratch) {
        *scratch = nullptr;
        if (R > 0 && !c.binning_buffer) return fail(GSR_ERR_INVALID_ARG, "missing binning buffer");
        if (!c.alloc) return fail(GSR_ERR_INVALID_ARG, "allocator callback required");
        if (bytes == 0) return GSR_OK;
        return obtain(c.alloc, c.alloc_ctx, GSR_BUF_SCRATCH, bytes, "backward scratch", scratch);
    }

    int fisher() {
// ... 340 lines not shown
    return track_forward_static(
        fwd_call(settings, gaussians, out_color, out_depth, radii, alloc, alloc_ctx, stream), colors2, out_color2,
        capacity, status,
        TrackL1{gt_im, gt_depth, sil_thres, w_im, w_depth, dL_dloss, dL_dim, dL_ddepth_sil, scratch, loss, nullptr});
}

int gsr_track_forward_dual_static_terms(const gsr_settings* settings, const gsr_gaussians* gaussians,
                                        const float* colors2, int capacity, unsigned* status, float* out_color,
                                        float* out_color2, float* out_depth, int* radii, const float* gt_im,
                                        const float* gt_depth, float sil_thres, float w_im, float w_depth,
                                        const float* dL_dloss, float* loss, float* terms, float* dL_dim,
                                        float* dL_ddepth_sil, float* scratch, gsr_alloc_fn alloc, void* alloc_ctx,
                                        void* stream) {
    if (int rc = check_terms("track_forward_dual_static_terms", terms)) return rc;
    return track_forward_static(
        fwd_call(settings, gaussians, out_color, out_depth, radii, alloc, alloc_ctx, stream), colors2, out_color2,
        capacity, status,
        TrackL1{gt_im, gt_depth, sil_thres, w_im, w_depth, dL_dloss, dL_dim, dL_ddepth_sil, scratch, loss, terms});
}

int gsr_track_forward_dual_static_xf(const gsr_settings* settings, const gsr_gaussians* gaussians, float* colors2,
                                     const gsr_track_xform* xform, int capacity, unsigned* status, float* out_color,
                                     float* out_color2, float* out_depth, int* radii, const float* gt_im,
                                     const float* gt_depth, float sil_thres, float w_im, float w_depth,
                                     const float* dL_dloss, float* loss, float* dL_dim, float* dL_ddepth_sil,
                                     float* scratch, gsr_alloc_fn alloc, void* alloc_ctx, void* stream) {
    FwdCall c = fwd_call(settings, gaussians, out_color, out_depth, radii, alloc, alloc_ctx, stream);
    statics(dual(c, colors2, out_color2), capacity, status);
    return track_forward_xf(c, xform,
                            TrackL1{gt_im, gt_depth, sil_thres, w_im, w_depth, dL_dloss, dL_dim, dL_ddepth_sil,
                                    scratch, loss, nullptr});
}

int gsr_track_forward_dual_static_xf_terms(const gsr_settings* settings, const gsr_gaussians* gaussians,
                                           float* colors2, const gsr_track_xform* xform, int capacity,
                                           unsigned* status, float* out_color, float* out_color2, float* out_depth,
                                           int* radii, const float* gt_im, const float* gt_depth, float sil_thres,
                                           float w_im, float w_depth, const float* dL_dloss, float* loss,
                                           float* terms, float* dL_dim, float* dL_ddepth_sil, float* scratch,
                                           gsr_alloc_fn alloc, void* alloc_ctx, void* stream) {
    if (int rc = check_terms("track_forward_dual_static_xf_terms", terms)) return rc;
    FwdCall c = fwd_call(settings, gaussians, out_color, out_depth, radii, alloc, alloc_ctx, stream);
    statics(dual(c, colors2, out_color2), capacity, status);
    return track_forward_xf(c, xform,
                            TrackL1{gt_im, gt_depth, sil_thres, w_im, w_depth, dL_dloss, dL_dim, dL_ddepth_sil,
                                    scratch, loss, terms});
}

int gsr_track_records_floats(int capacity) { return track_records_stride() * (capacity > 1 ? capacity : 1); }

static int track_forward_backward_xf(FwdCall c, float* colors2, float* out_color2, const gsr_track_xform* xform,
                                     int capacity, unsigned* status, float* inst_records, const TrackL1& l1) {
    if (!inst_records) return fail(GSR_ERR_INVALID_ARG, "track_forward_backward_dual_static_xf: null records");
    statics(dual(c, colors2, out_color2), capacity, status).track_inst = inst_records;
    return track_forward_xf(c, xform, l1);
}

int gsr_track_forward_backward_dual_static_xf(const gsr_settings* settings, const gsr_gaussians* gaussians,
                                              float* colors2, const gsr_track_xform* xform, int capacity,
                                              unsigned* status, float* out_color, float* out_color2,
                                              float* out_depth, int* radii, const float* gt_im,
                                              const float* gt_depth, float sil_thres, float w_im, float w_depth,
                                              const float* dL_dloss, float* loss, float* scratch,
                                              float* inst_records, gsr_alloc_fn alloc, void* alloc_ctx,
                                              void* stream) {
    return track_forward_backward_xf(
        fwd_call(settings, gaussians, out_color, out_depth, radii, alloc, alloc_ctx, stream), colors2, out_color2,
        xform, capacity, status, inst_records,
        TrackL1{gt_im, gt_depth, sil_thres, w_im, w_depth, dL_dloss, nullptr, nullptr, scratch, loss, nullptr});
}

int gsr_track_forward_backward_dual_static_xf_terms(const gsr_settings* settings, const gsr_gaussians* gaussians,
                                                    float* colors2, const gsr_track_xform* xform, int capacity,
                                                    unsigned* status, float* out_color, float* out_color2,
                                                    float* out_depth, int* radii, const float* gt_im,
                                                    const float* gt_depth, float sil_thres, float w_im,
                                                    float w_depth, const float* dL_dloss, float* loss, float* terms,
                                                    float* scratch, float* inst_records, gsr_alloc_fn alloc,
                                                    void* alloc_ctx, void* stream) {
    if (int rc = check_terms("track_forward_backward_dual_static_xf_terms", terms)) return rc;
    return track_forward_backward_xf(
        fwd_call(settings, gaussians, out_color, out_depth, radii, alloc, alloc_ctx, stream), colors2, out_color2,
        xform, capacity, status, inst_records,
        TrackL1{gt_im, gt_depth, sil_thres, w_im, w_depth, dL_dloss, nullptr, nullptr, scratch, loss, terms});
}

int gsr_forward_reuse(const gsr_settings* settings, const gsr_gaussians* gaussians, int num_rendered,
                      const void* prev_geom, void* binning_buffer, void* image_buffer, const int* prev_radii,
                      float* out_color, float* out_depth, int* radii, gsr_alloc_fn alloc, void* alloc_ctx,
                      void* stream_) {
    int rc = validate(settings, gaussians, true);
    if (rc != GSR_OK) return rc;
    if (!alloc) return fail(GSR_ERR_INVALID_ARG, "allocator callback required");
    if (!gaussians->colors_precomp || (gaussians->shs && gaussians->M > 0))
        return fail(GSR_ERR_INVALID_ARG, "geometry reuse needs precomputed colours (no SH)");
    if (gaussians->P <= 0 || num_rendered < 0 || !prev_geom || !binning_buffer || !image_buffer || !prev_radii ||
        !out_color || !out_depth || !radii)
        return fail(GSR_ERR_INVALID_ARG, "geometry reuse needs the previous call's state and the outputs");
    hipStream_t stream = (hipStream_t)stream_;
    const int dev = stream_device(stream);
    Camera cam = make_camera(settings);
    const GaussIn g = make_gauss(gaussians);
    const int P = g.P;
    const GeomLayout GL = GeomLayout::make(P);
    cam.pre_shift = GL.shift;
    void* geom;
    if ((rc = obtain(alloc, alloc_ctx, GSR_BUF_GEOM, GL.total, "geom buffer", &geom)) != GSR_OK) return rc;
    const GeomPtrs geo = GeomPtrs::at(geom, GL);
    const ImgPtrs img = ImgPtrs::at(image_buffer, ImgLayout::make(cam.W, cam.H));
    bind_schedule(cam, img, dev);
    hipError_t e;
    {
        StageTimer t(GSR_STAGE_PREPROCESS, P, stream);
        if ((e = hipMemcpyAsync(geom, prev_geom, GL.total, hipMemcpyDeviceToDevice, stream)) != hipSuccess ||
            (e = hipMemcpyAsync(radii, prev_radii, sizeof(int) * (size_t)P, hipMemcpyDeviceToDevice, stream)) !=
                hipSuccess)
            return hip_fail(e, "copy previous geometry");
        if ((e = launch_recolour(P, g.colors, geo, stream)) != hipSuccess) return hip_fail(e, "recolour");
    }
    const SpecGuard guard{geo.counters, (uint32_t)num_rendered, 0xFFFFFFFFu};
    StageTimer t(GSR_STAGE_RENDER_FWD, num_rendered, stream, true);
    if ((e = launch_render_fwd(cam, img.ranges, (uint64_t*)binning_buffer, nullptr, geo, nullptr, img.final_T,
                               img.n_contrib, out_color, nullptr, out_depth, guard, stream, t.kclock())) != hipSuccess)
        return hip_fail(e, "render");
    return num_rendered;
}

int gsr_forward_reuse_if_equal(const gsr_settings* settings, const gsr_gaussians* gaussians, int npairs,
                               const float* const* a, const float* const* b, const long long* n,
                               int prev_num_rendered, const void* prev_geom, void* prev_binning, void* prev_image,
                               const int* prev_radii, float* out_color, float* out_depth, int* radii, int* reused,
                               gsr_alloc_fn alloc, void* alloc_ctx, void* stream) {
    if (!gaussians || !gaussians->colors_precomp || (gaussians->shs && gaussians->M > 0) || gaussians->cov3D_precomp)
        return fail(GSR_ERR_INVALID_ARG, "geometry reuse needs precomputed colours (no SH, no cov3D)");
    if (npairs < 1 || npairs > 8 || !a || !b || !n || !reused)
        return fail(GSR_ERR_INVALID_ARG, "gsr_forward_reuse_if_equal: 1..8 pairs and `reused`");
    if (prev_num_rendered < 0 || !prev_geom || !prev_binning || !prev_image || !prev_radii)
        return fail(GSR_ERR_INVALID_ARG, "geometry reuse needs the previous call's state");
    ReuseIn r{};
    r.pairs.npairs = npairs;
    for (int k = 0; k < npairs; k++) {
        if (n[k] < 0 || (n[k] > 0 && (!a[k] || !b[k])))
            return fail(GSR_ERR_INVALID_ARG, "gsr_forward_reuse_if_equal: pair");
        r.pairs.a[k] = a[k];
        r.pairs.b[k] = b[k];
        r.pairs.n[k] = n[k];
    }
    r.prev_num_rendered = prev_num_rendered;
    r.prev_geom = prev_geom;
    r.prev_binning = prev_binning;
    r.prev_image = prev_image;
    r.prev_radii = prev_radii;
    r.reused = reused;
    FwdCall c = fwd_call(settings, gaussians, out_color, out_depth, radii, alloc, alloc_ctx, stream);
    c.reuse = &r;
    return forward_impl(c);
}

int gsr_bitwise_equal(int npairs, const float* const* a, const float* const* b, const long long* n, int* flag,
                      void* stream) {
    if (npairs < 0 || npairs > 8 || (npairs > 0 && (!a || !b || !n)) || !flag)
        return fail(GSR_ERR_INVALID_ARG, "gsr_bitwise_equal: 0..8 pairs and a flag");
    EqualPairs q{};
    q.npairs = npairs;
    for (int k = 0; k < npairs; k++) {
        if (n[k] < 0 || (n[k] > 0 && (!a[k] || !b[k]))) return fail(GSR_ERR_INVALID_ARG, "gsr_bitwise_equal: pair");
// ... 125 lines not shown
```

### splatam_amd/csrc/gsr_forward.hip

```cpp
#include "gsr_clock.h"
#include "gsr_diag.h"
#include "gsr_launch.h"
#include "gsr_layout.h"
#include "gsr_render_fwd.h"
#include "gsr_wave.h"

namespace gsr {

template <bool DUAL, bool L1 = false>
__global__ void __launch_bounds__(TILE_PIX, 5)
render_fwd_kernel(Camera cam, const uint2* __restrict__ ranges, PointEntry* __restrict__ point_list,
                  uint64_t* __restrict__ keys, const float4* __restrict__ rr, float* __restrict__ final_T, uint32_t* __restrict__ n_contrib,
                  float* __restrict__ out_color, float* __restrict__ out_color2, float* __restrict__ out_depth,
                  SpecGuard guard, unsigned long long* clk, TrackL1 l1) {
    static_assert(DUAL || !L1, "the tracking loss needs the depth / silhouette colour set");
    if (cam.gate.off()) return;
    kclock_begin(clk);
    RenderDiag dg;
    dg.begin();
    if (guard.overflow()) {
        kclock_end(clk);
        return;
    }
    __shared__ __attribute__((aligned(16))) char smem[FwdShape<DUAL>::bytes];
    const int tile = sched_tile(cam);
    dg.tile(tile);
    const FwdPix f = fwd_tile<DUAL>(cam, tile, ranges, point_list, keys, rr, guard, smem, dg);
    float g[4];
    fwd_epilogue<DUAL, L1, true>(cam, tile, f, final_T, n_contrib, out_color, out_color2, out_depth, l1, g);
    dg.phase(5);
    dg.end();
    kclock_end(clk);
}

#if GSR_PHASE
extern "C" int gsr_diag_phase_fwd(unsigned long long* host) {
    if (hipMemcpyFromSymbol(host, HIP_SYMBOL(g_phase), sizeof(g_phase), 0, hipMemcpyDeviceToHost) != hipSuccess)
        return -1;
    const unsigned long long z[8] = {0, 0, 0, 0, 0, 0, 0, 0};
    return hipMemcpyToSymbol(HIP_SYMBOL(g_phase), z, sizeof(z), 0, hipMemcpyHostToDevice) == hipSuccess ? 0 : -1;
}
#endif
#if GSR_WGTIME
extern "C" int gsr_diag_wgtime_fwd(unsigned long long* host, int n) {
    const size_t bytes = sizeof(unsigned long long) * 4 * (size_t)(n < GSR_WGTIME_MAX ? n : GSR_WGTIME_MAX);
    return hipMemcpyFromSymbol(host, HIP_SYMBOL(g_wgtime), bytes, 0, hipMemcpyDeviceToHost) == hipSuccess ? 0 : -1;
}
#endif

int track_l1_fused_scratch_floats(int ntiles) { return 2 * ntiles + ARRIVE_GROUPED_WORDS; }

hipError_t launch_render_fwd(const Camera& cam, const uint2* ranges, uint64_t* point_list,
                             uint64_t* keys, GeomPtrs geo,
                             const float* colors2, float* final_T, uint32_t* n_contrib, float* out_color,
                             float* out_color2, float* out_depth, SpecGuard guard, hipStream_t s,
                             unsigned long long* clk, const TrackL1* l1) {
    auto k = colors2 ? (l1 ? render_fwd_kernel<true, true> : render_fwd_kernel<true, false>)
                     : render_fwd_kernel<false, false>;
    hipLaunchKernelGGL(k, dim3(cam.gx * cam.gy), dim3(TILE_PIX), 0, s, cam, ranges, point_list, keys,
                       geo.rr, final_T,
                       n_contrib, out_color, out_color2, out_depth, guard, clk, l1 ? *l1 : TrackL1{});
    return hipGetLastError();
}

}
```

### splatam_amd/csrc/gsr_launch.h

```cpp
#pragma once
#include "gsr_adam.h"
#include "gsr_layout.h"

namespace gsr {

hipError_t launch_preprocess(const Camera& cam, const GaussIn& g, GeomPtrs geo, int* radii, uint32_t* counts,
                             bool lds_hist, int ntiles, int nb, hipStream_t s, unsigned long long* clk = nullptr);
hipError_t launch_mark_visible(int P, const float* means3D, const float* view, uint8_t* vis, hipStream_t s);
hipError_t launch_tile_colscan(uint32_t* counts, int nb, int ntiles, uint32_t* tot, GeomPtrs geo, uint2* ranges,
                               uint32_t* status, bool tail, hipStream_t s, unsigned long long* clk = nullptr,
                               Gate gate = Gate{});
hipError_t launch_scan_counts(GeomPtrs geo, int nb, const uint32_t* tile_count, int tile_stride, int ntiles,
                              uint2* ranges, uint32_t* status, hipStream_t s);
hipError_t launch_identity_order(uint32_t* order, int ntiles, hipStream_t s);
hipError_t launch_duplicate_bucket(const Camera& cam, int P, GeomPtrs geo, uint2* ranges, const uint32_t* tot,
                                   uint32_t* cursor, bool lds_hist, int ntiles, uint64_t* keys, uint64_t* point_list,
                                   int nb, SpecGuard guard, uint32_t* status, hipStream_t s, unsigned long long* clk = nullptr);
hipError_t launch_duplicate(const Camera& cam, int P, GeomPtrs geo, uint64_t* keys, uint32_t* gid,
                            int nb, hipStream_t s);
hipError_t launch_radix_sort(uint64_t* keys[2], uint32_t* vals[2], uint32_t* hist, uint32_t n, int nsb, int npass,
                             hipStream_t s);
hipError_t launch_gather_ids(const uint32_t* vals, const uint32_t* gid, uint64_t* point_list, uint32_t n, hipStream_t s);
struct TrackL1 {
    const float* gt_im;
    const float* gt_depth;
    float sil_thres, w_im, w_depth;
    const float* seed;
    float* dL_dim;
    float* dL_dds;
    float* scratch;
    float* loss;
    float* terms;
};
int track_l1_fused_scratch_floats(int ntiles);
hipError_t launch_render_fwd(const Camera& cam, const uint2* ranges, uint64_t* point_list, uint64_t* keys,
                             GeomPtrs geo, const float* colors2, float* final_T, uint32_t* n_contrib,
                             float* out_color, float* out_color2, float* out_depth, SpecGuard guard, hipStream_t s,
                             unsigned long long* clk = nullptr, const TrackL1* l1 = nullptr);
hipError_t launch_recolour(int P, const float* colors, GeomPtrs geo, hipStream_t s, Gate gate = Gate{});
hipError_t launch_reuse_copy(Gate gate, const void* prev_geom, void* geom, size_t geom_bytes, size_t tiles_offset,
                             const float* colors, const int* prev_radii, int* radii, int P, hipStream_t s);
struct EqualPairs {
    int npairs;
    const float* a[8];
    const float* b[8];
    long long n[8];
};
hipError_t launch_epoch_mismatch(const EqualPairs& q, uint32_t* word, uint32_t e, hipStream_t s);
hipError_t launch_bitwise_equal(const EqualPairs& q, int* flag, hipStream_t s);
hipError_t launch_render_track(const Camera& cam, const uint2* ranges, uint64_t* point_list, uint64_t* keys,
                               GeomPtrs geo, float* final_T, uint32_t* n_contrib, float* out_color,
                               float* out_color2, float* out_depth, SpecGuard guard, const TrackL1& l1, float* inst,
                               hipStream_t s, unsigned long long* clk = nullptr);
int track_records_stride();
struct RecLayout {
    int stride;
    int o_op, o_c1, o_c2, n_c2;
};
struct RecSums {
    RecLayout rec;
    int o_col;
    int o_m1;
    int nv;
};
constexpr RecSums rec_sums(bool op, bool c1, bool c2, int q2, bool m2d = false) {
    RecSums s{};
    int nv = 5;
    s.rec.o_op = op ? nv : -1;
    nv += op ? 1 : 0;
    s.o_col = nv;
    s.rec.o_c1 = c1 ? nv : -1;
    nv += c1 ? 3 : 0;
    s.rec.o_c2 = c2 ? nv : -1;
    s.rec.n_c2 = c2 ? q2 : 0;
    nv += s.rec.n_c2;
    s.o_m1 = m2d ? nv : -1;
    nv += m2d ? 2 : 0;
    s.nv = nv;
    s.rec.stride = (nv + 1) & ~1;
    return s;
}
static_assert(rec_sums(true, true, true, 3).rec.stride == INST_REC_MAX && rec_sums(true, true, true, 1, true).nv == INST_REC_MAX,
              "INST_REC_MAX: the largest records, every sum of a dual render and the M2D1 form");
RecLayout bwd_rec_layout(unsigned need, bool dual);
hipError_t launch_render_bwd(const Camera& cam, const uint2* ranges, const uint64_t* point_list, GeomPtrs geo,
                             const float* final_T, const uint32_t* n_contrib, const float* dL_dpix,
                             const float* colors2, const float* dL_dpix2, unsigned need, float* inst, BwdGuard guard,
                             hipStream_t s, unsigned long long* clk = nullptr);
constexpr unsigned NEED_OPACITY = 1u, NEED_COLORS = 2u, NEED_COLORS2 = 4u;
constexpr unsigned NEED_DL2_CH0_ONLY = 8u;
struct GradsOut {
    float* dmeans2D;
    float* dcolors;
    float* dopacity;
    float* dmeans3D;
    float* dcov3D;
    float* dsh;
    float* dscales;
    float* drot;
    float* dcolors2;
};
constexpr int M2D_REC_PAIR = rec_sums(true, true, true, 1, true).o_m1;
static_assert(M2D_REC_PAIR == 10, "the mapping variant's ten sums, then the pair");
struct M2dOut {
    float* dmeans2D_c1 = nullptr;
    int o_m1 = -1;
};
int m2d_record_stride();
hipError_t launch_render_bwd_m2d(const Camera& cam, const uint2* ranges, const uint64_t* point_list, GeomPtrs geo,
                                 const float* final_T, const uint32_t* n_contrib, const float* dL_dpix,
                                 const float* dL_dpix2, float* inst, BwdGuard guard, hipStream_t s,
                                 unsigned long long* clk = nullptr);
hipError_t launch_gauss_bwd_m2d(const Camera& cam, const GaussIn& g, GeomPtrs geo, const int* radii, const float* inst,
                                RecLayout rec, const GradsOut& out, M2dOut m1, BwdGuard guard, hipStream_t s,
                                unsigned long long* clk = nullptr);
struct PoseFuse {
    const float* means_world;
    const float* unnorm_rot;
    int scols;
    float* cam_q;
    float* cam_t;
    int qs;
    const float* w2c;
    float* scratch;
    float* adam_state;
    double lr_q, lr_t, beta1, beta2, eps;
    float* dq;
    float* dt;
    const uint32_t* guard = nullptr;
    uint32_t cap = 0;
    const float* loss = nullptr;
    float* best = nullptr;
    const float* ls = nullptr;
};
int pose_fuse_scratch_floats(int P);
hipError_t launch_gauss_bwd(const Camera& cam, const GaussIn& g, GeomPtrs geo, const int* radii, const float* inst,
// ... 43 lines not shown
```

### splatam_amd/csrc/gsr_layout.h

```cpp
#pragma once
#include <hip/hip_runtime.h>
#include <stddef.h>
#include <stdint.h>

namespace gsr {

constexpr int TILE_X = 16;
constexpr int TILE_Y = 16;
constexpr int TILE_PIX = TILE_X * TILE_Y;
constexpr int PRE_BLOCK = 1024;
__host__ __device__ inline int pre_shift_for(int P, int cus) { return ((P + 1023) >> 10) < 2 * cus ? 9 : 10; }
int geom_pre_shift(int P);
int current_device_cus();
constexpr int MAX_LDS_TILES = 16384;
constexpr int SORT_THREADS = 256;
constexpr int SORT_ITEMS = 8;
constexpr int SORT_TILE = SORT_THREADS * SORT_ITEMS;
constexpr int RADIX = 256;
constexpr int RENDER_BATCH = 256;
constexpr int INST_REC_MAX = 12;
constexpr int TILE_CTR_STRIDE = 64;

__host__ __device__ inline size_t align_up(size_t x, size_t a) { return (x + a - 1) / a * a; }

// ... 60 lines not shown
    while (b < 32 && (n >> b) != 0) b++;
    return b;
}

constexpr int TILE_SORT_CAP = 4096;

struct BinLayout {
    size_t point_list;
    size_t keys[2];
    size_t vals[2];
    size_t gid;
    size_t hist;
    size_t total;
    int nsb;
    int npass;
    int final_buf;
    static BinLayout make(int I, int W, int H) {
        BinLayout L;
        size_t n = (size_t)(I > 0 ? I : 1);
        uint32_t tiles = (uint32_t)(((W + TILE_X - 1) / TILE_X) * ((H + TILE_Y - 1) / TILE_Y));
        int bits = 32 + higher_msb(tiles);
        L.npass = (bits + 7) / 8;
        L.final_buf = L.npass & 1;
        L.nsb = (int)((n + SORT_TILE - 1) / SORT_TILE);
        size_t o = 0;
        L.point_list = o; o = align_up(o + 8 * n, 256);
        L.keys[0] = o; o = align_up(o + 8 * n, 256);
        L.keys[1] = o; o = align_up(o + 8 * n, 256);
        L.vals[0] = o; o = align_up(o + 4 * n, 256);
        L.vals[1] = o; o = align_up(o + 4 * n, 256);
        L.gid = o; o = align_up(o + 4 * n, 256);
        L.hist = o; o = align_up(o + 4 * ((size_t)RADIX * L.nsb + RADIX), 256);
        L.total = o;
        return L;
    }
};

struct Gate {
    const uint32_t* p = nullptr;
    uint32_t e = 0;
    uint32_t run = 1;
    __device__ __forceinline__ bool off() const { return p != nullptr && ((*p == e) != (run != 0u)); }
};

struct Camera {
    int W, H;
    float tan_fovx, tan_fovy, focal_x, focal_y;
    int gx, gy;
    const float* view;
    const float* proj;
    const float* campos;
    const float* bg;
    float scale_modifier;
    int sh_degree;
    int prefiltered;
    const uint32_t* tile_order = nullptr;
    uint32_t* tile_order_out = nullptr;
    uint32_t* rowmax = nullptr;
    int sched_cus = 256;
    int pre_shift = 10;
    int cull = 0;
    int tail_exact = 0;
    Gate gate;
    uint32_t* host_snap = nullptr;
};
__device__ __forceinline__ bool tile_live(uint32_t live, uint32_t k) { return k >= 32u || ((live >> k) & 1u); }
__device__ __forceinline__ uint32_t culled_below(uint32_t live, uint32_t k) {
    const uint32_t m = k >= 32u ? 0xFFFFFFFFu : ((1u << k) - 1u);
    return (uint32_t)__popc(~live & m);
}
__device__ __forceinline__ void prio_by_remaining(int remaining, uint32_t mean4, bool multi) {
    const uint32_t r = 4u * (uint32_t)remaining;
    const uint32_t t3 = multi ? 200u : 70u, t2 = multi ? 100u : 45u, t1 = multi ? 50u : 22u;
    if (100u * r > t3 * mean4) __builtin_amdgcn_s_setprio(3);
    else if (100u * r > t2 * mean4) __builtin_amdgcn_s_setprio(2);
    else if (100u * r > t1 * mean4) __builtin_amdgcn_s_setprio(1);
    else __builtin_amdgcn_s_setprio(0);
}
__device__ __forceinline__ bool sched_multi_round(const Camera& cam) { return cam.gx * cam.gy > 5 * cam.sched_cus; }
__device__ __forceinline__ uint32_t sched_mean4(const Camera& cam, const uint32_t* counters) {
    const uint32_t nt = (uint32_t)(cam.gx * cam.gy);
    return max(1u, (uint32_t)(4ull * counters[0] / (nt ? nt : 1u)));
}
__device__ __forceinline__ int sched_tile(const Camera& cam) {
    return cam.tile_order ? (int)cam.tile_order[blockIdx.x] : (int)blockIdx.x;
}

struct TrackXf {
    const float* mw = nullptr;
    const float* ur = nullptr;
    const float* lo = nullptr;
    const float* ls = nullptr;
    int scols = 1;
    const float* cq = nullptr;
    const float* ct = nullptr;
    int qs = 1;
    const float* w2c = nullptr;
    int store = 1;
};

struct GaussIn {
    TrackXf xf;
    int P, M;
    const float* means3D;
    const float* shs;
    const float* colors;
    const float* opacities;
    const float* scales;
    const float* rotations;
    const float* cov3D;
    const float* colors2;
    int sh_staged;
    const uint8_t* alive = nullptr;
};

struct GeomPtrs {
    float4* rr;
    uint32_t* clamp;
    uint4* bin;
    uint32_t* tiles;
    uint32_t* offsets;
    uint32_t* blocksums;
    uint32_t* counters;
    uint32_t* wgsum;
    uint32_t* wgcull;
    static GeomPtrs at(void* base, const GeomLayout& L) {
        char* b = (char*)base;
        return {(float4*)(b + L.rr), (uint32_t*)(b + L.clamp), (uint4*)(b + L.bin), (uint32_t*)(b + L.tiles),
                (uint32_t*)(b + L.offsets), (uint32_t*)(b + L.blocksums), (uint32_t*)(b + L.counters),
                (uint32_t*)(b + L.wgsum), (uint32_t*)(b + L.wgcull)};
    }
};

struct SpecGuard {
    const uint32_t* counters;
    uint32_t cap_inst, cap_tile;
    __device__ __forceinline__ bool overflow() const {
        return counters[0] > cap_inst || counters[2] > cap_tile;
    }
};
struct BwdGuard {
    const uint32_t* counters;
    uint32_t cap_inst;
    __device__ __forceinline__ bool overflow() const {
        return counters[0] > cap_inst || counters[2] > counters[3];
    }
};
__device__ __forceinline__ void status_merge(uint32_t* st, uint32_t n, uint32_t viol, uint32_t longest,
                                             uint32_t sort_cap) {
    if (n) atomicMax(st + 0, n);
    if (viol) atomicOr(st + 1, viol);
    if (longest) atomicMax(st + 2, longest);
    if (sort_cap) atomicMax(st + 3, sort_cap);
}

struct RenderRec {
    float4 q0, q1, q2, q3;
};
__device__ __forceinline__ RenderRec load_rr(const float4* __restrict__ rr, uint32_t i) {
    const float4* r = rr + (size_t)RR_F4 * i;
    return {r[0], r[1], r[2], r[3]};
}
__device__ __forceinline__ uint2 rr_rect(const RenderRec& r) {
    return make_uint2(__float_as_uint(r.q2.w), __float_as_uint(r.q3.w));
}
__device__ __forceinline__ uint32_t rr_offset(const RenderRec& r, const uint32_t* blocksums, uint32_t i, int shift) {
// ... 10 lines not shown
```

### splatam_amd/csrc/gsr_preprocess.hip

```cpp
#include "gsr_clock.h"
#include "gsr_dispatch.h"
#include "gsr_glue_common.h"
#include "gsr_launch.h"
#include "gsr_layout.h"
#include "gsr_math.h"
#include "gsr_wave.h"

namespace gsr {

template <bool LDS_HIST, bool XF, bool CLK, bool EXACT>
__global__ void __launch_bounds__(PRE_BLOCK)
preprocess_kernel(Camera cam, GaussIn g, GeomPtrs geo, int* radii, uint32_t* __restrict__ counts, int ntiles,
                  unsigned long long* clk) {
#pragma clang fp contract(off)
    if (cam.gate.off()) return;
    if constexpr (CLK) kclock_begin(clk);
    extern __shared__ uint32_t s_hist[];
    __shared__ float s_pose[16];
    const int i = (blockIdx.x << cam.pre_shift) + threadIdx.x;
    XfRaw xr{};
    if (XF && i < g.P) xr = track_xform_load(g.xf, i, true);
    float pre_rgb[3] = {0.f, 0.f, 0.f}, pre_c2[3] = {0.f, 0.f, 0.f}, pre_op = 0.f;
    if (!XF && i < g.P) {
        if (g.colors) {
            pre_rgb[0] = g.colors[3 * i]; pre_rgb[1] = g.colors[3 * i + 1]; pre_rgb[2] = g.colors[3 * i + 2];
        } else if (g.sh_staged) {
            const uint4 c = geo.bin[i];
            pre_rgb[0] = __uint_as_float(c.x); pre_rgb[1] = __uint_as_float(c.y); pre_rgb[2] = __uint_as_float(c.z);
        }
        pre_op = g.opacities[i];
        if (g.colors2) {
            pre_c2[0] = g.colors2[3 * i]; pre_c2[1] = g.colors2[3 * i + 1]; pre_c2[2] = g.colors2[3 * i + 2];
        }
    }
    if (XF && threadIdx.x < 64) {
        const Pose ps = make_pose(g.xf.cq, g.xf.ct, g.xf.qs);
        if (threadIdx.x == 0) {
#pragma unroll
            for (int k = 0; k < 9; k++) s_pose[k] = ps.R[k / 3][k % 3];
#pragma unroll
            for (int k = 0; k < 3; k++) s_pose[9 + k] = ps.t[k];
#pragma unroll
            for (int k = 0; k < 4; k++) s_pose[12 + k] = ps.c[k];
        }
    }
    if (LDS_HIST)
        for (int t = threadIdx.x; t < ntiles; t += blockDim.x) s_hist[t] = 0u;
    if (LDS_HIST || XF) __syncthreads();
    if (i == 0) geo.counters[4] = 0u;
    uint32_t tiles = 0, culled = 0;
    bool violation = false;
    float4 q0, q1, q2, q3;
    if (i < g.P) {
        int radius = 0;
        float3 p;
        float xs[3], xc2[3], xop = 0.f;
        float4 xq;
        if (XF) {
            Pose ps;
#pragma unroll
            for (int k = 0; k < 9; k++) ps.R[k / 3][k % 3] = s_pose[k];
#pragma unroll
            for (int k = 0; k < 3; k++) ps.t[k] = s_pose[9 + k];
#pragma unroll
            for (int k = 0; k < 4; k++) ps.c[k] = s_pose[12 + k];
            float m[3];
            track_xform_compute_raw(g.xf, xr, ps, m, xq, xc2, xop, xs);
            p = make_float3(m[0], m[1], m[2]);
        } else {
            p = make_float3(g.means3D[3 * i], g.means3D[3 * i + 1], g.means3D[3 * i + 2]);
        }
        float4 hom = xform4x4(p, cam.proj);
        float pw = 1.0f / (hom.w + 0.0000001f);
        float3 pv = xform4x3(p, cam.view);
        bool ok = pv.z > 0.001f;
        if (!ok && cam.prefiltered) violation = true;
        if (g.alive != nullptr && g.alive[i] == 0) ok = false;
        float cov3[6];
        Proj pj;
        float det = 0.f, ca = 0.f, cb = 0.f, cc = 0.f;
        if (ok) {
            if (g.cov3D) {
#pragma unroll
                for (int k = 0; k < 6; k++) cov3[k] = g.cov3D[6 * i + k];
            } else {
                float3 s = XF ? make_float3(xs[0], xs[1], xs[2])
                              : make_float3(g.scales[3 * i], g.scales[3 * i + 1], g.scales[3 * i + 2]);
                float4 q = XF ? xq : make_float4(g.rotations[4 * i], g.rotations[4 * i + 1], g.rotations[4 * i + 2],
                                                 g.rotations[4 * i + 3]);
                cov3d_fwd(s, cam.scale_modifier, q, cov3);
            }
            cov2d_fwd(p, cam.focal_x, cam.focal_y, cam.tan_fovx, cam.tan_fovy, cov3, cam.view, pj);
            det = conic_of(pj, ca, cb, cc);
            ok = det != 0.0f;
        }
        if (ok) {
            float mid = 0.5f * (pj.a + pj.c);
            float l1 = mid + sqrtf(fmaxf(0.1f, mid * mid - det));
            float l2 = mid - sqrtf(fmaxf(0.1f, mid * mid - det));
            float rad = ceilf(3.f * sqrtf(fmaxf(l1, l2)));
            float px = ndc2pix(hom.x * pw, cam.W), py = ndc2pix(hom.y * pw, cam.H);
            int x0, y0, x1, y1;
            get_rect(px, py, (int)rad, cam.gx, cam.gy, x0, y0, x1, y1);
            tiles = (uint32_t)((x1 - x0) * (y1 - y0));
            if (tiles != 0) {
                float rgb[3] = {pre_rgb[0], pre_rgb[1], pre_rgb[2]};
                unsigned clamped = 0;
                if (XF && g.colors) {
                    rgb[0] = g.colors[3 * i]; rgb[1] = g.colors[3 * i + 1]; rgb[2] = g.colors[3 * i + 2];
                } else if (XF && g.sh_staged) {
                    const uint4 c = geo.bin[i];
                    rgb[0] = __uint_as_float(c.x); rgb[1] = __uint_as_float(c.y); rgb[2] = __uint_as_float(c.z);
                } else if (!g.colors && !g.sh_staged) {
                    sh_fwd(cam.sh_degree, p, cam.campos, g.shs + (size_t)3 * g.M * i, rgb, clamped);
                }
                radius = (int)rad;
                float c2[3] = {0.f, 0.f, 0.f};
                if (XF) {
                    c2[0] = xc2[0]; c2[1] = xc2[1]; c2[2] = xc2[2];
                } else if (g.colors2) {
                    c2[0] = pre_c2[0]; c2[1] = pre_c2[1]; c2[2] = pre_c2[2];
                }
                const uint32_t rlo = (uint32_t)x0 | ((uint32_t)y0 << 16), rhi = (uint32_t)x1 | ((uint32_t)y1 << 16);
                q0 = make_float4(px, py, K_AC * ca, K_AC * cc);
                q2 = make_float4(rgb[0], rgb[1], rgb[2], __uint_as_float(rlo));
                q3 = make_float4(c2[0], c2[1], c2[2], __uint_as_float(rhi));
                if (XF) {
                    float4* rr = geo.rr + (size_t)RR_F4 * i;
                    rr[0] = q0;
                    rr[2] = q2;
                    rr[3] = q3;
                }
                q1 = make_float4(K_B * cb, XF ? xop : pre_op, pv.z, 0.f);
                uint32_t live = 0xFFFFFFFFu;
                if (cam.cull && tiles <= 32u) {
                    const MaskGeom mg = mask_geom(q0, q1);
                    live = 0u;
                    for (int ty = y0, k = 0; ty < y1; ty++)
                        for (int tx = x0; tx < x1; tx++, k++)
                            live |= tile_reached(mg, (float)(tx * TILE_X), (float)(ty * TILE_Y)) ? 1u << k : 0u;
                }
                if constexpr (EXACT) culled = culled_below(live, tiles);
                geo.bin[i] = make_uint4(rlo, rhi, __float_as_uint(pv.z), live);
                if (!g.sh_staged && !g.colors) geo.clamp[i] = clamped;
                for (int ty = y0, k = 0; ty < y1; ty++)
                    for (int tx = x0; tx < x1; tx++, k++) {
                        if (!tile_live(live, (uint32_t)k)) continue;
                        if (LDS_HIST) atomicAdd(&s_hist[ty * cam.gx + tx], 1u);
                        else atomicAdd(&counts[(ty * cam.gx + tx) * TILE_CTR_STRIDE], 1u);
                    }
            }
        }
        radii[i] = radius;
        geo.tiles[i] = tiles;
        if (tiles == 0) geo.bin[i] = make_uint4(0u, 0u, 0u, 0u);
        if (XF && g.xf.store) {
            const float m[3] = {p.x, p.y, p.z};
            track_xform_store(i, m, xq, xc2, xop, xs, const_cast<float*>(g.means3D), const_cast<float*>(g.rotations),
                              const_cast<float*>(g.colors2), const_cast<float*>(g.opacities),
                              const_cast<float*>(g.scales));
        }
    }
    __shared__ uint32_t wsum[PRE_BLOCK / 64], wcul[PRE_BLOCK / 64];
    const int lane = threadIdx.x & 63, wv = threadIdx.x >> 6;
    uint32_t incl = wave_incl_scan(tiles);
    if (lane == 63) wsum[wv] = incl;
    if constexpr (EXACT) {
        const uint32_t cincl = wave_incl_scan(culled);
        if (lane == 63) wcul[wv] = cincl;
    }
    __syncthreads();
    uint32_t woff = 0;
    for (int k = 0; k < wv; k++) woff += wsum[k];
    if (tiles) {
        q1.w = __uint_as_float(woff + incl - tiles);
        float4* rr = geo.rr + (size_t)RR_F4 * i;
        if (!XF) {
            rr[0] = q0;
            rr[2] = q2;
            rr[3] = q3;
        }
        rr[1] = q1;
    }
    const bool viol = __syncthreads_or(violation);
    if (threadIdx.x == blockDim.x - 1) {
        geo.wgsum[blockIdx.x] = (woff + incl) | (viol ? 0x80000000u : 0u);
        if constexpr (EXACT) {
            uint32_t cw = 0;
            for (int k = 0; k < (int)(blockDim.x >> 6); k++) cw += wcul[k];
            geo.wgcull[blockIdx.x] = cw;
        }
    }
    if (LDS_HIST)
        for (int t = threadIdx.x; t < ntiles; t += blockDim.x) counts[(size_t)blockIdx.x * ntiles + t] = s_hist[t];
    if constexpr (CLK) kclock_end(clk);
}

struct PickPreprocess {
    template <bool LDS_HIST, bool XF, bool CLK, bool EXACT>
    auto operator()() const { return &preprocess_kernel<LDS_HIST, XF, CLK, EXACT && !XF>; }
};

hipError_t launch_preprocess(const Camera& cam, const GaussIn& g, GeomPtrs geo, int* radii, uint32_t* counts,
                             bool lds_hist, int ntiles, int nb, hipStream_t s, unsigned long long* clk) {
    if (nb == 0) return hipSuccess;
    const bool xf = g.xf.mw != nullptr;
    const bool exact = cam.tail_exact && cam.cull && !xf;
    const auto k = dispatch_bools(PickPreprocess{}, lds_hist, xf, clk != nullptr, exact);
    hipLaunchKernelGGL(k, dim3(nb), dim3(1 << cam.pre_shift), lds_hist ? sizeof(uint32_t) * ntiles : 0, s, cam, g,
                       geo, radii, counts, ntiles, clk);
    return hipGetLastError();
}

__global__ void mark_visible_kernel(int P, const float* __restrict__ means3D, const float* __restrict__ view,
                                    uint8_t* __restrict__ vis) {
    const int i = blockIdx.x * blockDim.x + threadIdx.x;
    if (i >= P) return;
    float3 p = make_float3(means3D[3 * i], means3D[3 * i + 1], means3D[3 * i + 2]);
    vis[i] = xform4x3(p, view).z > 0.001f ? 1 : 0;
}

hipError_t launch_mark_visible(int P, const float* means3D, const float* view, uint8_t* vis, hipStream_t s) {
    if (P == 0) return hipSuccess;
    hipLaunchKernelGGL(mark_visible_kernel, dim3((P + 255) / 256), dim3(256), 0, s, P, means3D, view, vis);
    return hipGetLastError();
}

}
```

### splatam_amd/csrc/gsr_render_bwd.h

```cpp
#pragma once
#include "gsr_clock.h"
#include "gsr_diag.h"
#include "gsr_launch.h"
#include "gsr_layout.h"
#include "gsr_math.h"
#include "gsr_moments.h"
#include "gsr_wave.h"

namespace gsr {

template <bool DUAL_, bool OPAC_, bool COL1_, bool COL2_, int Q2_ = 3, int MOM_ = 0, int C1_ = 3, bool M2D1_ = false>
struct BwdVariant {
    static constexpr bool DUAL = DUAL_, OPAC = OPAC_, COL1 = COL1_, COL2 = COL2_, M2D1 = M2D1_;
    static constexpr int Q2 = Q2_, MOM = MOM_, C1 = C1_;
    static_assert(DUAL || !COL2, "COL2 needs the dual colour set");
    static_assert(!MOM || (!DUAL && OPAC && COL1), "the moment variants form every single-image gradient");
    static_assert(Q2 == 1 || Q2 == 3, "Q2 is 1 or 3 channels");
    static_assert(C1 == 3 || (C1 == 1 && COL1 && !DUAL && !MOM), "one colour sum: single-image colour variants only");
    static_assert(!M2D1 || (DUAL && OPAC && COL1 && COL2 && Q2 == 1 && !MOM && C1 == 3), "M2D1: the mapping form only");
};
using TrackVariant = BwdVariant<true, false, false, true, 1>;
using MapM2dVariant = BwdVariant<true, true, true, true, 1, 0, 3, true>;
template <int MOM>
using MomVariant = BwdVariant<false, true, true, false, 3, MOM>;
// ... 64 lines not shown
template <int NV, int MOM = 0>
constexpr int bwd_batch() { return MOM ? 128 : (NV <= 6 ? GSR_BWD_BB : GSR_BWD_WBB); }
#ifndef GSR_BWD_WBS
#define GSR_BWD_WBS 384
#endif
#ifndef GSR_BWD_BS
#define GSR_BWD_BS (4 * GSR_BWD_BB)
#endif
#ifndef GSR_BWD_M2D_BS
#define GSR_BWD_M2D_BS GSR_BWD_WBS
#endif
template <int NV, int MOM = 0>
constexpr int bwd_slots() { return MOM == 1 ? 256 : (MOM == 2 ? 128 : (NV <= 6 ? GSR_BWD_BS : GSR_BWD_WBS)); }

template <class V>
constexpr RecSums bwd_sums() { return rec_sums(V::OPAC, V::COL1, V::COL2, V::Q2, V::M2D1); }
template <class V>
constexpr int bwd_nv() { return V::MOM ? mom_nv(V::MOM) : bwd_sums<V>().nv - (V::COL1 ? 3 - V::C1 : 0); }
#ifndef GSR_BWD_WIDE_WAVES
#define GSR_BWD_WIDE_WAVES 5
#endif
#ifndef GSR_BWD_MAP_WAVES
#define GSR_BWD_MAP_WAVES 4
#endif
#ifndef GSR_BWD_M2D_WAVES
#define GSR_BWD_M2D_WAVES 4
#endif
template <class V>
constexpr int bwd_waves() {
    return V::MOM ? 4 : ((V::DUAL && V::Q2 == 3) ? GSR_BWD_MAP_WAVES : ((V::OPAC && V::COL1) ? GSR_BWD_WIDE_WAVES : 5));
}

template <class V>
struct BwdShape {
    static constexpr int NV = bwd_nv<V>();
    static constexpr int NV3 = V::MOM ? NV : bwd_sums<V>().nv;
    static constexpr int O_COL = bwd_sums<V>().o_col, O_M1 = bwd_sums<V>().o_m1;
    static constexpr int BB = bwd_batch<NV3, V::MOM>(), BS = V::M2D1 ? GSR_BWD_M2D_BS : bwd_slots<NV3, V::MOM>();
    static constexpr int RS = V::MOM ? (NV3 + 1) & ~1 : bwd_sums<V>().rec.stride;
    static constexpr int LS = BB + 4;
    static constexpr int SL = BB + 1;
    static constexpr bool PACKC = V::DUAL && V::Q2 == 1;
    static constexpr size_t o_a = 0, o_b = o_a + 16 * SL, o_c = o_b + 16 * SL, o_d = o_c + 16 * SL;
    static constexpr size_t o_acc = o_d + 16 * ((V::DUAL && !PACKC) ? SL : 1);
    static constexpr size_t o_list = o_acc + (4 * (BS + 1) * NV + 15) / 16 * 16;
    static constexpr size_t o_u = o_list + 4 * 16 * LS, o_mask = o_u + 4 * BB, o_base = o_mask + 2 * BB;
    static constexpr size_t o_rmax = (o_base + 2 * BB + 3) / 4 * 4;
    static constexpr size_t bytes = o_rmax + 64;
};

struct BwdPix {
    float T_final;
    uint32_t last;
    float dp0, dp1, dp2, dq0, dq1, dq2;
};
template <bool DUAL, int Q2>
__device__ __forceinline__ void load_bwd_pix(BwdPix& pin, const Camera& cam, int px, int py,
                                             const float* __restrict__ final_T, const uint32_t* __restrict__ n_contrib,
                                             const float* __restrict__ dL_dpix, const float* __restrict__ dL_dpix2) {
    const bool inside = px < cam.W && py < cam.H;
    const int pid = py * cam.W + px;
    const int HW = cam.W * cam.H;
    if (inside) {
        pin.T_final = final_T[pid];
        pin.last = n_contrib[pid];
        pin.dp0 = dL_dpix[pid];
        pin.dp1 = dL_dpix[HW + pid];
        pin.dp2 = dL_dpix[2 * HW + pid];
        if (DUAL) {
            pin.dq0 = dL_dpix2[pid];
            if (Q2 == 3) {
                pin.dq1 = dL_dpix2[HW + pid];
                pin.dq2 = dL_dpix2[2 * HW + pid];
            }
        }
    }
}

template <class V>
__device__ __forceinline__ void bwd_tile(const Camera& cam, int tile, const BwdPix& pin,
                                         const uint2* __restrict__ ranges, const PointEntry* __restrict__ point_list,
                                         const float4* __restrict__ rr, const uint32_t* __restrict__ blocksums,
                                         float* __restrict__ inst, const BwdGuard& guard, char* smem,
                                         RenderDiag& dg) {
    constexpr bool DUAL = V::DUAL, OPAC = V::OPAC, COL1 = V::COL1, COL2 = V::COL2, M2D1 = V::M2D1;
    constexpr int Q2 = V::Q2, MOM = V::MOM, C1 = V::C1;
    using L = BwdShape<V>;
    constexpr int NV = L::NV;
    constexpr int BB = L::BB, BS = L::BS, RS = L::RS, LS = L::LS;
    constexpr bool PACKC = L::PACKC;
    float4* const s_a = reinterpret_cast<float4*>(smem + L::o_a);
    float4* const s_b = reinterpret_cast<float4*>(smem + L::o_b);
    float4* const s_c = reinterpret_cast<float4*>(smem + L::o_c);
    [[maybe_unused]] float4* const s_d = reinterpret_cast<float4*>(smem + L::o_d);
    uint32_t* const s_u = reinterpret_cast<uint32_t*>(smem + L::o_u);
    uint16_t* const s_mask = reinterpret_cast<uint16_t*>(smem + L::o_mask);
    uint16_t* const s_base = reinterpret_cast<uint16_t*>(smem + L::o_base);
    float* const s_acc = reinterpret_cast<float*>(smem + L::o_acc);
    uint32_t* const s_rmax = reinterpret_cast<uint32_t*>(smem + L::o_rmax);
    uint32_t* const s_list = reinterpret_cast<uint32_t*>(smem + L::o_list);
    const int tid = threadIdx.x, lane = tid & 63, w = tid >> 6, row = (tid >> 4) & 3;
    const int tx = tile % cam.gx, ty = tile / cam.gx;
    const int px = tx * TILE_X + tile_px(tid);
    const int py = ty * TILE_Y + tile_py(tid);
    const float x0 = (float)(tx * TILE_X), y0 = (float)(ty * TILE_Y);
    const uint2 range = ranges[tile];
    const float T_final = pin.T_final;
    const uint32_t last = pin.last;
    const float dp0 = pin.dp0, dp1 = pin.dp1, dp2 = pin.dp2, dq0 = pin.dq0, dq1 = pin.dq1, dq2 = pin.dq2;
    uint32_t bmax = 0;
    int rm[4];
    if (cam.rowmax) {
        const uint4* rp = reinterpret_cast<const uint4*>(cam.rowmax + 16 * tile);
#pragma unroll
        for (int b = 0; b < 4; b++) {
            const uint4 q = rp[b];
            bmax = max(bmax, max(max(q.x, q.y), max(q.z, q.w)));
        }
        const uint4 qw = rp[w];
        rm[0] = (int)qw.x; rm[1] = (int)qw.y; rm[2] = (int)qw.z; rm[3] = (int)qw.w;
    } else {
        uint32_t rmax = last;
#pragma unroll
        for (int o = 8; o > 0; o >>= 1) rmax = max(rmax, (uint32_t)__shfl_xor((int)rmax, o));
        if ((lane & 15) == 0) s_rmax[4 * w + row] = rmax;
        __syncthreads();
#pragma unroll
        for (int b = 0; b < 16; b++) bmax = max(bmax, s_rmax[b]);
#pragma unroll
        for (int r = 0; r < 4; r++) rm[r] = (int)s_rmax[4 * w + r];
    }
    for (uint32_t k = range.x + bmax + tid; k < range.y; k += TILE_PIX) {
        const uint32_t gk = pe_id(point_list[k]);
        const RenderRec r = load_rr(rr, gk);
        const uint32_t u = instance_slot(rr_rect(r), rr_offset(r, blocksums, gk, cam.pre_shift), tx, ty);
        float2* dst = reinterpret_cast<float2*>(inst + (size_t)RS * u);
#pragma unroll
        for (int m = 0; m < RS / 2; m++) dst[m] = make_float2(0.f, 0.f);
    }
    float bg_dot = cam.bg[0] * dp0 + cam.bg[1] * dp1 + cam.bg[2] * dp2;
    [[maybe_unused]] float A1 = 0.f;
    if constexpr (M2D1) A1 = bg_dot;
    if (DUAL) bg_dot += cam.bg[0] * dq0 + cam.bg[1] * dq1 + cam.bg[2] * dq2;
    const v2f pix = v2f{(float)px, (float)py};
    const v2f dp01 = v2f{dp0, dp1}, dq01 = v2f{dq0, dq1};
    const v2f dp2q0 = v2f{dp2, dq0};
    [[maybe_unused]] const float mdp2[3] = {dp0 * dp0, dp1 * dp1, dp2 * dp2};
    [[maybe_unused]] const float mdpp[6] = {dp0 * dp0, dp0 * dp1, dp0 * dp2, dp1 * dp1, dp1 * dp2, dp2 * dp2};
    float T = T_final, A = bg_dot;
    [[maybe_unused]] float ablate_sink = 0.f;
    const int my_e = row_entry(lane);
    constexpr bool kBulkClear = !OPAC;
    for (int q = tid; q < (BS + 1) * NV; q += TILE_PIX) s_acc[q] = 0.f;
    const uint32_t* my_list = s_list + (4 * w + row) * LS;
    if (tid == 0) {
        const float4 z = make_float4(0.f, 0.f, 0.f, 0.f);
        s_a[BB] = z;
        s_b[BB] = z;
        s_c[BB] = z;
        if (DUAL && !PACKC) s_d[BB] = z;
    }
    float4 pa = make_float4(0.f, 0.f, 0.f, 0.f), pb = pa, pc = pa, pd = pa;
    uint32_t pbs = 0, pm = 0, prh = 0;
    PointEntry pn = 0;
    auto fetch_entry = [&](int hi_) {
        if (tid < min(BB, hi_)) pn = point_list[range.x + (uint32_t)(hi_ - 1 - tid)];
    };
    auto fetch_rec = [&](int hi_) {
        if (tid < min(BB, hi_)) {
            const uint32_t gi = pe_id(pn);
            pm = pe_mask(pn);
            const RenderRec r = load_rr(rr, gi);
            pbs = blocksums[gi >> cam.pre_shift];
            pa = r.q0; pb = r.q1; pc = r.q2;
            if (DUAL && !PACKC) {
                pd = r.q3;
            } else {
                prh = __float_as_uint(r.q3.w);
                if (PACKC) pd.x = r.q3.x;
            }
        }
    };
    fetch_entry((int)bmax);
    fetch_rec((int)bmax);
    fetch_entry((int)bmax - BB);
    const uint32_t mean4 = sched_mean4(cam, guard.counters);
    const bool multi_round = sched_multi_round(cam);
    int hi_pf = (int)bmax;
    dg.phase(0);
// ... 266 lines not shown
```

### splatam_amd/csrc/gsr_render_fwd.h

```cpp
#pragma once
#include "gsr_diag.h"
#include "gsr_launch.h"
#include "gsr_layout.h"
#include "gsr_math.h"
#include "gsr_wave.h"

namespace gsr {

constexpr int TILE_SORT_THREADS = 256;
constexpr uint32_t TILE_SORT_REGS = 1024;

template <int M>
__device__ __forceinline__ uint32_t lane_xor(uint32_t x) {
    static_assert(M == 1 || M == 2 || M == 4 || M == 8 || M == 16 || M == 32, "lane xor distance");
    if constexpr (M == 1) {
        return (uint32_t)__builtin_amdgcn_mov_dpp((int)x, 0xB1, 0xF, 0xF, false);
    } else if constexpr (M == 2) {
        return (uint32_t)__builtin_amdgcn_mov_dpp((int)x, 0x4E, 0xF, 0xF, false);
    } else if constexpr (M == 4) {
        const uint32_t up = (uint32_t)__builtin_amdgcn_mov_dpp((int)x, 0x104, 0xF, 0xF, false);
        const uint32_t dn = (uint32_t)__builtin_amdgcn_mov_dpp((int)x, 0x114, 0xF, 0xF, false);
        return (__lane_id() & 4) ? dn : up;
    } else if constexpr (M == 8) {
        return (uint32_t)__builtin_amdgcn_mov_dpp((int)x, 0x128, 0xF, 0xF, false);
    } else if constexpr (M == 16) {
        const auto p = __builtin_amdgcn_permlane16_swap(x, x, false, false);
        return (__lane_id() & 16) ? p[0] : p[1];
    } else {
        const auto p = __builtin_amdgcn_permlane32_swap(x, x, false, false);
        return (__lane_id() & 32) ? p[0] : p[1];
    }
}
template <int M>
__device__ __forceinline__ uint64_t lane_xor64(uint64_t v) {
    return ((uint64_t)lane_xor<M>((uint32_t)(v >> 32)) << 32) | lane_xor<M>((uint32_t)v);
}

template <int E, int J>
__device__ __forceinline__ void bitonic_reg_stage(uint64_t (&v)[E], uint32_t base, uint32_t k) {
#pragma unroll
    for (int e = 0; e < E; e++) {
        if (e & J) continue;
        const bool up = ((base + (uint32_t)e) & k) == 0;
        const uint64_t a = v[e], b = v[e + J];
        const bool sw = (b < a) == up;
        v[e] = sw ? b : a;
        v[e + J] = sw ? a : b;
    }
}

__device__ __forceinline__ uint64_t bitonic_pick(uint64_t v, uint64_t o, bool keep_min) {
    return ((o < v) == keep_min) ? o : v;
}

template <int E, int LK, int LJ>
__device__ __forceinline__ void bitonic_net(uint64_t (&v)[E], uint32_t base, uint64_t* sk) {
    constexpr uint32_t k = 1u << LK, j = 1u << LJ;
    if constexpr (j >= (uint32_t)E) {
        const bool up = (base & k) == 0, keep_min = ((base & j) == 0) == up;
        if constexpr (j >= 64u * E) {
#pragma unroll
            for (int e = 0; e < E; e++) sk[base + e] = v[e];
            __syncthreads();
#pragma unroll
            for (int e = 0; e < E; e++) v[e] = bitonic_pick(v[e], sk[(base + e) ^ j], keep_min);
            __syncthreads();
        } else {
#pragma unroll
            for (int e = 0; e < E; e++) v[e] = bitonic_pick(v[e], lane_xor64<(int)(j / E)>(v[e]), keep_min);
        }
    } else {
        bitonic_reg_stage<E, (int)j>(v, base, k);
    }
    constexpr int LOGN = E == 1 ? 8 : E == 2 ? 9 : 10;
    if constexpr (LJ > 0) bitonic_net<E, LK, LJ - 1>(v, base, sk);
    else if constexpr (LK < LOGN) bitonic_net<E, LK + 1, LK>(v, base, sk);
}

template <int E, typename Emit>
__device__ void tile_sort_regs(const uint64_t* __restrict__ src, uint32_t cnt, Emit emit, uint64_t* sk) {
    static_assert(E == 1 || E == 2 || E == 4, "256 x E keys");
    const uint32_t base = threadIdx.x * E;
    uint64_t v[E];
#pragma unroll
    for (int e = 0; e < E; e++) v[e] = base + e < cnt ? src[base + e] : ~0ull;
    bitonic_net<E, 1, 0>(v, base, sk);
#pragma unroll
    for (int e = 0; e < E; e++)
        if (base + e < cnt) emit(base + e, v[e] == ~0ull ? 0u : (uint32_t)v[e]);
}

#if GSR_FWD_ABLATE == 7
static __device__ uint16_t g_fab_mask[1u << 23];
#endif
__device__ __forceinline__ void tile_sort_bucket(uint64_t* __restrict__ src, uint32_t cnt,
                                                 PointEntry* __restrict__ dst, uint64_t* sk) {
    auto emit = [&](uint32_t i, uint32_t gi) { dst[i] = (PointEntry)gi; };
    if (GSR_FWD_ABLATE == 1) {
        for (uint32_t i = threadIdx.x; i < cnt; i += TILE_SORT_THREADS) emit(i, (uint32_t)src[i]);
        return;
    }
    if (cnt <= 1) {
        if (cnt == 1 && threadIdx.x == 0) emit(0, (uint32_t)src[0]);
        return;
    }
    if (cnt <= 256) {
        tile_sort_regs<1>(src, cnt, emit, sk);
        return;
    }
    if (cnt <= 512) {
        tile_sort_regs<2>(src, cnt, emit, sk);
        return;
    }
    const uint32_t nch = (cnt + TILE_SORT_REGS - 1) / TILE_SORT_REGS;
    const uint32_t base = threadIdx.x * 4;
    for (uint32_t c = 0; c < nch; c++) {
        const uint32_t c0 = c * TILE_SORT_REGS, len = min(TILE_SORT_REGS, cnt - c0);
        uint64_t v[4];
#pragma unroll
        for (int e = 0; e < 4; e++) v[e] = base + e < len ? src[c0 + base + e] : ~0ull;
        bitonic_net<4, 1, 0>(v, base, sk);
#pragma unroll
        for (int e = 0; e < 4; e++) {
            if (base + e >= len) continue;
            if (nch == 1) emit(base + e, v[e] == ~0ull ? 0u : (uint32_t)v[e]);
            else src[c0 + base + e] = v[e];
        }
    }
    if (nch == 1) return;
    __syncthreads();
    for (uint32_t c = 0; c < nch; c++) {
        const uint32_t c0 = c * TILE_SORT_REGS, len = min(TILE_SORT_REGS, cnt - c0);
        uint64_t v[4];
        uint32_t pos[4];
#pragma unroll
        for (int e = 0; e < 4; e++) {
            v[e] = base + e < len ? src[c0 + base + e] : ~0ull;
            pos[e] = base + e;
        }
        for (uint32_t c2 = 0; c2 < nch; c2++) {
            if (c2 == c) continue;
            const uint32_t d0 = c2 * TILE_SORT_REGS, dlen = min(TILE_SORT_REGS, cnt - d0);
            __syncthreads();
            for (uint32_t i = threadIdx.x; i < dlen; i += TILE_SORT_THREADS) sk[i] = src[d0 + i];
            __syncthreads();
#pragma unroll
            for (int e = 0; e < 4; e++) {
                uint32_t lo = 0;
#pragma unroll
                for (uint32_t st = TILE_SORT_REGS; st > 0; st >>= 1)
                    if (lo + st <= dlen && sk[lo + st - 1] < v[e]) lo += st;
                pos[e] += lo;
            }
        }
#pragma unroll
        for (int e = 0; e < 4; e++)
            if (base + e < len) emit(pos[e], (uint32_t)v[e]);
    }
    __syncthreads();
}

template <bool DUAL>
struct FwdShape {
    static constexpr int LS = RENDER_BATCH + 4;
    static constexpr size_t o_ab = 0, o_c = o_ab + 2 * 16 * (RENDER_BATCH + 1), o_d = o_c + 16 * (RENDER_BATCH + 1);
    static constexpr size_t o_list = o_d + 16 * (DUAL ? RENDER_BATCH + 1 : 1);
    static constexpr size_t o_mask = o_list + 2 * 16 * LS;
    static constexpr size_t bytes = o_mask + 2 * RENDER_BATCH;
    static_assert(2 * 16 * (RENDER_BATCH + 1) >= TILE_SORT_REGS * sizeof(uint64_t) && TILE_SORT_THREADS == TILE_PIX,
                  "tile sort (256 x 4 keys) LDS aliases s_a / s_b");
};

struct FwdPix {
    float T, C2, C5, D;
    v2f C01, C34;
    uint32_t last16;
};

template <bool DUAL>
__device__ __forceinline__ FwdPix fwd_tile(const Camera& cam, int tile, const uint2* __restrict__ ranges,
                                           PointEntry* __restrict__ point_list, uint64_t* __restrict__ keys,
                                           const float4* __restrict__ rr, const SpecGuard& guard, char* smem,
                                           RenderDiag& dg) {
    using L = FwdShape<DUAL>;
    constexpr int LS = L::LS;
    float4* const s_ab = reinterpret_cast<float4*>(smem + L::o_ab);
    float4* const s_a = s_ab;
    float4* const s_b = s_ab + RENDER_BATCH + 1;
    float4* const s_c = reinterpret_cast<float4*>(smem + L::o_c);
    [[maybe_unused]] float4* const s_d = reinterpret_cast<float4*>(smem + L::o_d);
    uint16_t* const s_mask = reinterpret_cast<uint16_t*>(smem + L::o_mask);
    uint16_t* const s_list = reinterpret_cast<uint16_t*>(smem + L::o_list);
    const int tid = threadIdx.x, w = tid >> 6, row = (tid >> 4) & 3;
    const int tx = tile % cam.gx, ty = tile / cam.gx;
    const int px = tx * TILE_X + tile_px(tid);
    const int py = ty * TILE_Y + tile_py(tid);
    const float x0 = (float)(tx * TILE_X), y0 = (float)(ty * TILE_Y);
    const bool inside = px < cam.W && py < cam.H;
    const v2f pix = v2f{(float)px, (float)py};
    const uint2 range = ranges[tile];
    bool done = !inside;
    float T = 1.f, C2 = 0.f, D = 15.0f;
    float C5 = 0.f;
    v2f C01 = v2f{0.f, 0.f}, C34 = v2f{0.f, 0.f};
    uint32_t last16 = 0;
    float4 pa = make_float4(0.f, 0.f, 0.f, 0.f), pb = pa, pc = pa, pd = pa;
    uint32_t pg = 0, pgn = 0;
    if (keys != nullptr) {
        tile_sort_bucket(keys + range.x, range.y - range.x, point_list + range.x,
                         reinterpret_cast<uint64_t*>(s_ab));
        __syncthreads();
        if constexpr (kDupPhase == 1) {
            tile_sort_bucket(keys + range.x, range.y - range.x, point_list + range.x,
                             reinterpret_cast<uint64_t*>(s_ab));
            __syncthreads();
        }
    }
    if (tid == 0) {
        s_a[RENDER_BATCH] = pa;
        s_b[RENDER_BATCH] = pa;
        s_c[RENDER_BATCH] = pa;
        if (DUAL) s_d[RENDER_BATCH] = pa;
    }
    auto fetch_id = [&](uint32_t s0) {
        if (s0 + tid < range.y) pgn = pe_id(point_list[s0 + tid]);
    };
    auto fetch_rec = [&](uint32_t s0) {
        if (s0 + tid < range.y) {
            pg = pgn;
            const RenderRec r = load_rr(rr, pg);
            pa = r.q0; pb = r.q1; pc = r.q2;
            if (DUAL) pd = r.q3;
        }
    };
    fetch_id(range.x);
    fetch_rec(range.x);
    fetch_id(range.x + RENDER_BATCH);
    const uint32_t mean4 = sched_mean4(cam, guard.counters);
    const bool multi_round = sched_multi_round(cam);
    dg.phase(0);
    for (uint32_t start = range.x; start < range.y; start += RENDER_BATCH) {
        prio_by_remaining((int)(range.y - start), mean4, multi_round);
        if (__syncthreads_and(done)) break;
        const int cnt = (int)min((uint32_t)RENDER_BATCH, range.y - start);
        PointEntry ent = 0;
        if (tid < cnt) {
            float xs = x0, ys = y0;
            asm volatile("" : "+v"(xs), "+v"(ys));
            uint32_t pm = GSR_FWD_ABLATE == 5 ? block_mask(pa, pb, xs, ys)
                        : GSR_FWD_ABLATE == 6 ? 0xFFFFu : 0u;
#if GSR_FWD_ABLATE == 7
            pm = g_fab_mask[start + tid];
            if (pm == 0u) {
                pm = block_mask_exact(pa, pb, xs, ys);
                g_fab_mask[start + tid] = (uint16_t)pm;
            }
#else
            if (GSR_FWD_ABLATE != 5 && GSR_FWD_ABLATE != 6) pm = block_mask_exact(pa, pb, xs, ys);
#endif
            s_a[tid] = pa;
            s_b[tid] = pb;
            s_c[tid] = DUAL ? make_float4(pc.x, pc.y, pc.z, pd.z) : pc;
            if (DUAL) s_d[tid] = pd;
            s_mask[tid] = (uint16_t)pm;
            ent = ((PointEntry)pm << 32) | pg;
        }
        __syncthreads();
        dg.phase(1);
        fetch_rec(start + RENDER_BATCH);
        fetch_id(start + 2 * RENDER_BATCH);
        if (tid < cnt) point_list[start + tid] = ent;
        const int jmin0[4] = {0, 0, 0, 0};
        static_assert(16 * RENDER_BATCH < 65536, "16-bit byte offsets");
        int n = build_row_lists(s_mask, cnt, w, jmin0, s_list + 4 * w * LS, LS, (uint16_t)(16 * RENDER_BATCH), 16u);
        if constexpr (kDupPhase == 2) {
            asm volatile("" ::: "memory");
            n = build_row_lists(s_mask, cnt, w, jmin0, s_list + 4 * w * LS, LS, (uint16_t)(16 * RENDER_BATCH), 16u);
        }
        const uint16_t* my_list = s_list + (4 * w + row) * LS;
        const uint32_t pos16 = 16u * (start - range.x) + 16u;
        dg.phase(2);
        for (int i = 0; i < (GSR_FWD_ABLATE == 2 ? 0 : n); i += 4) {
            if (done) break;
            int jb[4];
#pragma unroll
            for (int k = 0; k < 4; k++)
                jb[k] = (int)((const volatile __attribute__((address_space(3))) uint16_t*)my_list)[i + k];
            auto rec = [&](const float4* arr, int k) {
                return *reinterpret_cast<const float4*>(reinterpret_cast<const char*>(arr) + jb[k]);
            };
            float alpha[4], depth[4];
// ... 173 lines not shown
```

Measured before the change: 6658.

## Add row-local binning path for fused tracking forward+backward render

After: 6444. -3.2%, worse.

```diff
diff --git a/include/gsr_glue.h b/include/gsr_glue.h
--- a/include/gsr_glue.h
+++ b/include/gsr_glue.h
@@ -124,6 +124,15 @@
                                                     float w_depth, const float* dL_dloss, float* loss, float* terms,
                                                     float* scratch, float* inst_records, gsr_alloc_fn alloc,
                                                     void* alloc_ctx, void* stream);
+int gsr_track_rowbins_row_cap(int P, int image_width, int image_height, int capacity);
+int gsr_track_forward_backward_dual_static_xf_scan(const gsr_settings* settings, const gsr_gaussians* gaussians,
+                                                   float* colors2, const gsr_track_xform* xform, int capacity,
+                                                   unsigned* status, float* out_color, float* out_color2,
+                                                   float* out_depth, int* radii, const float* gt_im,
+                                                   const float* gt_depth, float sil_thres, float w_im, float w_depth,
+                                                   const float* dL_dloss, float* loss, float* terms, float* scratch,
+                                                   float* inst_records, gsr_alloc_fn alloc, void* alloc_ctx,
+                                                   void* stream);
 int gsr_track_backward_dual_records(const gsr_settings* settings, const gsr_gaussians* gaussians, const int* radii,
                                     const float* colors2, int num_rendered, const void* geom_buffer,
                                     const void* binning_buffer, const void* image_buffer, const float* means_world,
diff --git a/splatam_amd/_C.py b/splatam_amd/_C.py
--- a/splatam_amd/_C.py
+++ b/splatam_amd/_C.py
@@ -507,6 +507,24 @@
         return False
 
 
+class scan_binning:
+
+    def __enter__(self):
+        self.prev = getattr(_tls, "scan_binning", False)
+        _tls.scan_binning = True
+        return self
+
+    def __exit__(self, *exc):
+        _tls.scan_binning = self.prev
+        return False
+
+
+def rowbins_row_cap(P: int, W: int, H: int, capacity: int) -> int:
+    if getattr(_tls, "scan_binning", False) or binning_mode() != BINNING_CULLED:
+        return 0
+    return int(lib.gsr_track_rowbins_row_cap(int(P), int(W), int(H), int(capacity)))
+
+
 def mark_visible(means3D, viewmatrix, projmatrix):
     device = means3D.device
     P = means3D.size(0)
@@ -589,6 +607,10 @@
                 raise RuntimeError("records: contiguous float32 of gsr_track_records_floats(capacity) on the device")
             name = "gsr_track_forward_backward_dual_static_xf"
             tail = (scratch.data_ptr(), records.data_ptr())
+            if getattr(_tls, "scan_binning", False):
+                name += "_scan"
+                tail = (None if terms is None else terms_ptr(terms, device), *tail)
+                terms = None
         else:
             dim, dds = torch.empty(3, H, W, **f32), torch.empty(3, H, W, **f32)
             tail = (dim.data_ptr(), dds.data_ptr(), scratch.data_ptr())
diff --git a/splatam_amd/_lib.py b/splatam_amd/_lib.py
--- a/splatam_amd/_lib.py
+++ b/splatam_amd/_lib.py
@@ -136,6 +136,14 @@
                                                                 c_void_p, c_void_p, c_void_p, c_void_p, ALLOC_FN,
                                                                 c_void_p, c_void_p]),
     "gsr_track_records_floats": (c_int, [c_int]),
+    "gsr_track_rowbins_row_cap": (c_int, [c_int, c_int, c_int, c_int]),
+    "gsr_track_forward_backward_dual_static_xf_scan": (c_int, [ctypes.POINTER(GsrSettings),
+                                                               ctypes.POINTER(GsrGaussians), c_void_p,
+                                                               ctypes.POINTER(GsrTrackXform), c_int, c_void_p,
+                                                               c_void_p, c_void_p, c_void_p, c_void_p, c_void_p,
+                                                               c_void_p, c_float, c_float, c_float, c_void_p,
+                                                               c_void_p, c_void_p, c_void_p, c_void_p, ALLOC_FN,
+                                                               c_void_p, c_void_p]),
     "gsr_track_forward_backward_dual_static_xf": (c_int, [ctypes.POINTER(GsrSettings), ctypes.POINTER(GsrGaussians),
                                                           c_void_p, ctypes.POINTER(GsrTrackXform), c_int, c_void_p,
                                                           c_void_p, c_void_p, c_void_p, c_void_p, c_void_p, c_void_p,
diff --git a/splatam_amd/csrc/gsr_backward.hip b/splatam_amd/csrc/gsr_backward.hip
--- a/splatam_amd/csrc/gsr_backward.hip
+++ b/splatam_amd/csrc/gsr_backward.hip
@@ -44,13 +44,15 @@
 constexpr size_t track_lds_bytes() {
     return FwdShape<true>::bytes > BwdShape<TrackVariant>::bytes ? FwdShape<true>::bytes : BwdShape<TrackVariant>::bytes;
 }
-template <bool IMAGES>
-__global__ void __launch_bounds__(TILE_PIX, 5)
-render_track_kernel(Camera cam, const uint2* __restrict__ ranges, PointEntry* __restrict__ point_list,
-                    uint64_t* __restrict__ keys, const float4* __restrict__ rr, const uint32_t* __restrict__ blocksums,
-                    float* __restrict__ final_T, uint32_t* __restrict__ n_contrib, float* __restrict__ out_color,
-                    float* __restrict__ out_color2, float* __restrict__ out_depth, SpecGuard guard,
-                    unsigned long long* clk, TrackL1 l1, float* __restrict__ inst) {
+template <bool IMAGES, bool RB = false>
+__device__ __forceinline__ void render_track_body(Camera& cam, const uint2* __restrict__ ranges,
+                                                  PointEntry* __restrict__ point_list, uint64_t* __restrict__ keys,
+                                                  const float4* __restrict__ rr,
+                                                  const uint32_t* __restrict__ blocksums, float* __restrict__ final_T,
+                                                  uint32_t* __restrict__ n_contrib, float* __restrict__ out_color,
+                                                  float* __restrict__ out_color2, float* __restrict__ out_depth,
+                                                  const SpecGuard& guard, unsigned long long* clk, const TrackL1& l1,
+                                                  float* __restrict__ inst, const RowBins rb) {
     kclock_begin(clk);
     RenderDiag dg;
     dg.begin();
@@ -65,7 +67,8 @@
     }
     const int tile = sched_tile(cam);
     dg.tile(tile);
-    const FwdPix f = fwd_tile<true>(cam, tile, ranges, point_list, keys, rr, guard, smem, dg);
+    [[maybe_unused]] uint2 range_rb = make_uint2(0u, 0u);
+    const FwdPix f = fwd_tile<true, RB>(cam, tile, ranges, point_list, keys, rr, guard, smem, dg, rb, &range_rb);
     float grad[4];
     constexpr bool kStoreGrads = false;
     static_assert(!kStoreGrads, "render_track_kernel's callers pass no gradient images");
@@ -76,9 +79,29 @@
     Camera cb = cam;
     cb.rowmax = nullptr;
     bwd_tile<TrackVariant>(cb, tile, pin, ranges, point_list, rr, blocksums, inst,
-                           BwdGuard{guard.counters, guard.cap_inst}, smem, dg);
+                           BwdGuard{guard.counters, guard.cap_inst}, smem, dg, RB, range_rb);
     dg.end();
     kclock_end(clk);
+}
+template <bool IMAGES>
+__global__ void __launch_bounds__(TILE_PIX, 5)
+render_track_kernel(Camera cam, const uint2* __restrict__ ranges, PointEntry* __restrict__ point_list,
+                    uint64_t* __restrict__ keys, const float4* __restrict__ rr, const uint32_t* __restrict__ blocksums,
+                    float* __restrict__ final_T, uint32_t* __restrict__ n_contrib, float* __restrict__ out_color,
+                    float* __restrict__ out_color2, float* __restrict__ out_depth, SpecGuard guard,
+                    unsigned long long* clk, TrackL1 l1, float* __restrict__ inst) {
+    render_track_body<IMAGES>(cam, ranges, point_list, keys, rr, blocksums, final_T, n_contrib, out_color, out_color2,
+                              out_depth, guard, clk, l1, inst, RowBins{});
+}
+template <bool IMAGES>
+__global__ void __launch_bounds__(TILE_PIX, 5)
+render_track_rowbins_kernel(Camera cam, PointEntry* __restrict__ point_list, const float4* __restrict__ rr,
+                            const uint32_t* __restrict__ blocksums, float* __restrict__ final_T,
+                            uint32_t* __restrict__ n_contrib, float* __restrict__ out_color,
+                            float* __restrict__ out_color2, float* __restrict__ out_depth, SpecGuard guard,
+                            unsigned long long* clk, TrackL1 l1, float* __restrict__ inst, RowBins rb) {
+    render_track_body<IMAGES, true>(cam, nullptr, point_list, nullptr, rr, blocksums, final_T, n_contrib, out_color,
+                                    out_color2, out_depth, guard, clk, l1, inst, rb);
 }
 
 int track_records_stride() { return BwdShape<TrackVariant>::RS; }
@@ -125,6 +148,16 @@
     const auto k = dispatch_bools(PickRenderBwd{}, colors2 != nullptr, op, c1, c2, q2 == 1);
     hipLaunchKernelGGL(k, dim3(cam.gx * cam.gy), dim3(TILE_PIX), 0, s, cam, ranges, point_list, geo.rr, geo.blocksums,
                        final_T, n_contrib, dL_dpix, dL_dpix2, inst, guard, clk);
+    return hipGetLastError();
+}
+
+hipError_t launch_render_track_rowbins(const Camera& cam, uint64_t* point_list, GeomPtrs geo, float* final_T,
+                                       uint32_t* n_contrib, float* out_color, float* out_color2, float* out_depth,
+                                       SpecGuard guard, const TrackL1& l1, float* inst, const RowBins& rb,
+                                       hipStream_t s, unsigned long long* clk) {
+    auto k = final_T != nullptr ? render_track_rowbins_kernel<true> : render_track_rowbins_kernel<false>;
+    hipLaunchKernelGGL(k, dim3(cam.gx * cam.gy), dim3(TILE_PIX), 0, s, cam, point_list, geo.rr, geo.blocksums, final_T,
+                       n_contrib, out_color, out_color2, out_depth, guard, clk, l1, inst, rb);
     return hipGetLastError();
 }
 
diff --git a/splatam_amd/csrc/gsr_binning.hip b/splatam_amd/csrc/gsr_binning.hip
--- a/splatam_amd/csrc/gsr_binning.hip
+++ b/splatam_amd/csrc/gsr_binning.hip
@@ -2,6 +2,7 @@
 #include "gsr_dispatch.h"
 #include "gsr_launch.h"
 #include "gsr_layout.h"
+#include "gsr_tile_plan.h"
 #include "gsr_wave.h"
 
 namespace gsr {
@@ -199,67 +200,6 @@
     return hipGetLastError();
 }
 
-constexpr int PLAN_BUCKETS = 1024, PLAN_SHIFT = 2;
-__device__ __forceinline__ uint32_t plan_bucket(uint32_t len) {
-    return (uint32_t)(PLAN_BUCKETS - 1) - min(len >> PLAN_SHIFT, (uint32_t)(PLAN_BUCKETS - 1));
-}
-__device__ __forceinline__ uint32_t plan_slot(uint32_t p, uint32_t n, uint32_t ncu) {
-    const uint32_t q = n / ncu, m = n - q * ncu, heavy = q * (ncu - m);
-    const bool hv = p < heavy;
-    const uint32_t g0 = hv ? m : 0u, gs = hv ? ncu - m : m, pp = hv ? p : p - heavy;
-    const uint32_t rd = pp / gs, k = pp - rd * gs;
-    return rd * ncu + g0 + ((rd & 1u) ? gs - 1u - k : k);
-}
-template <int NT, int TPT = 0>
-__device__ void tile_plan(const uint32_t* __restrict__ tot, int ntiles, int ncu, uint32_t* __restrict__ order,
-                          uint32_t* s_hist, uint32_t* s_wsum, const uint32_t* tv = nullptr, int t0 = 0,
-                          int t1 = 0) {
-    constexpr int BPT = PLAN_BUCKETS / NT;
-    static_assert(BPT * NT == PLAN_BUCKETS, "buckets per thread");
-    const int tid = threadIdx.x, lane = tid & 63, w = tid >> 6;
-#pragma unroll
-    for (int k = 0; k < BPT; k++) s_hist[tid * BPT + k] = 0u;
-    __syncthreads();
-    if constexpr (TPT > 0) {
-#pragma unroll
-        for (int k = 0; k < TPT; k++)
-            if (t0 + k < t1) atomicAdd(&s_hist[plan_bucket(tv[k])], 1u);
-    } else {
-        for (int u = tid; u < ntiles; u += NT) atomicAdd(&s_hist[plan_bucket(tot[u])], 1u);
-    }
-    __syncthreads();
-    uint32_t c[BPT], cs = 0;
-#pragma unroll
-    for (int k = 0; k < BPT; k++) {
-        c[k] = s_hist[tid * BPT + k];
-        cs += c[k];
-    }
-    const uint32_t incl = wave_incl_scan(cs);
-    if (lane == 63) s_wsum[w] = incl;
-    __syncthreads();
-    uint32_t run = incl - cs;
-    for (int k = 0; k < w; k++) run += s_wsum[k];
-#pragma unroll
-    for (int k = 0; k < BPT; k++) {
-        s_hist[tid * BPT + k] = run;
-        run += c[k];
-    }
-    __syncthreads();
-    if constexpr (TPT > 0) {
-#pragma unroll
-        for (int k = 0; k < TPT; k++)
-            if (t0 + k < t1) {
-                const uint32_t p = atomicAdd(&s_hist[plan_bucket(tv[k])], 1u);
-                order[plan_slot(p, (uint32_t)ntiles, (uint32_t)ncu)] = (uint32_t)(t0 + k);
-            }
-    } else {
-        for (int u = tid; u < ntiles; u += NT) {
-            const uint32_t p = atomicAdd(&s_hist[plan_bucket(tot[u])], 1u);
-            order[plan_slot(p, (uint32_t)ntiles, (uint32_t)ncu)] = (uint32_t)u;
-        }
-    }
-}
-
 __global__ void identity_order_kernel(uint32_t* __restrict__ order, int n) {
     const int i = blockIdx.x * blockDim.x + threadIdx.x;
     if (i < n) order[i] = (uint32_t)i;
diff --git a/splatam_amd/csrc/gsr_capi.hip b/splatam_amd/csrc/gsr_capi.hip
--- a/splatam_amd/csrc/gsr_capi.hip
+++ b/splatam_amd/csrc/gsr_capi.hip
@@ -11,6 +11,7 @@
 #include "gsr_errors.h"
 #include "gsr_host.h"
 #include "gsr_launch.h"
+#include "gsr_wave.h"
 #include "gsr_layout.h"
 
 using namespace gsr;
@@ -210,6 +211,7 @@
     float* track_inst = nullptr;
     const uint8_t* alive = nullptr;
     const ReuseIn* reuse = nullptr;
+    bool scan_binning = false;
 };
 
 FwdCall fwd_call(const gsr_settings* settings, const gsr_gaussians* gaussians, float* out_color, float* out_depth,
@@ -429,6 +431,50 @@
         return render(bin, bin.keys[0], guard, units);
     }
 
+    static bool rowbins_eligible(int nb, int ntiles, int capacity) {
+        return nb > 0 && nb <= ROWBINS_MAX_ROWS && ntiles <= ROWBINS_MAX_TILES && ntiles <= MAX_LDS_TILES &&
+               capacity >= nb;
+    }
+    bool takes_rowbins() const {
+        return c.track_inst && c.l1 && c.xf && !eager && !c.scan_binning && cam.cull && c.radii &&
+               stores_no_images(c) && rowbins_eligible(GL.nb, ntiles, c.capacity);
+    }
+    int rowbins() {
+        cap = (uint32_t)c.capacity;
+        const size_t seg = sizeof(uint64_t) * (size_t)ntiles * TILE_SORT_CAP;
+        RowBins rb;
+        rb.rows = GL.nb;
+        rb.row_cap = rowbins_row_cap(GL.nb, c.capacity);
+        char* buf;
+        if (int rc = obtain(GSR_BUF_BINNING, 2 * seg + sizeof(uint64_t) * (size_t)GL.nb * rb.row_cap, "binning buffer",
+                            &buf))
+            return rc;
+        uint64_t* const point_list = (uint64_t*)buf;
+        rb.sort_scratch = (uint64_t*)(buf + seg);
+        rb.keys = (uint64_t*)(buf + 2 * seg);
+        rb.words = cmat;
+        rb.acc = scratch_counters(c.l1->scratch);
+        rb.lens = reinterpret_cast<uint32_t*>(c.l1->scratch) + track_l1_fused_scratch_floats(ntiles) - 2 * ntiles;
+        rb.plan = rb.lens + ntiles;
+        rb.status = status();
+        rb.counters = geo.counters;
+        cam.tile_order = rb.plan;
+        hipError_t e;
+        {
+            StageTimer t(GSR_STAGE_PREPROCESS, P, stream, true);
+            if ((e = launch_preprocess_rowbins(cam, g, geo, c.radii, ntiles, GL.nb, rb, stream, t.kclock())) !=
+                hipSuccess)
+                return hip_fail(e, "preprocess (row-local bins)");
+        }
+        const SpecGuard guard{geo.counters, cap, (uint32_t)TILE_SORT_CAP};
+        StageTimer t(GSR_STAGE_RENDER_FWD, 0, stream, true);
+        if ((e = launch_render_track_rowbins(cam, point_list, geo, stores_no_images(c) ? nullptr : img.final_T,
+                                             img.n_contrib, c.out_color, c.out_color2, c.out_depth, guard, *c.l1,
+                                             c.track_inst, rb, stream, t.kclock())) != hipSuccess)
+            return hip_fail(e, "render (fused tracking forward + backward, row-local bins)");
+        return (int)cap;
+    }
+
     int speculate() {
         void* buf;
         if (int rc = obtain(GSR_BUF_BINNING, BinLayout::make((int)cap, W, H).total, "binning buffer", &buf)) return rc;
@@ -514,6 +560,7 @@
     Forward F(c);
     if (int rc = F.setup_buffers()) return rc;
     if (F.P == 0) return F.empty_map();
+    if (F.takes_rowbins()) return F.rowbins();
     int rc;
     if ((rc = F.gate_on_comparison()) != GSR_OK || (rc = F.counts_and_ranges()) != GSR_OK) return rc;
     const double ratio = g_inst_ratio[F.dev].v.load(std::memory_order_relaxed);
@@ -1020,6 +1067,29 @@
     return track_forward_backward_xf(
         fwd_call(settings, gaussians, out_color, out_depth, radii, alloc, alloc_ctx, stream), colors2, out_color2,
         xform, capacity, status, inst_records,
+        TrackL1{gt_im, gt_depth, sil_thres, w_im, w_depth, dL_dloss, nullptr, nullptr, scratch, loss, terms});
+}
+
+int gsr_track_rowbins_row_cap(int P, int image_width, int image_height, int capacity) {
+    if (P <= 0 || capacity <= 0 || image_width <= 0 || image_height <= 0) return 0;
+    const int gx = (image_width + TILE_X - 1) / TILE_X, gy = (image_height + TILE_Y - 1) / TILE_Y;
+    const GeomLayout GL = GeomLayout::make(P);
+    if (!Forward::rowbins_eligible(GL.nb, gx * gy, capacity)) return 0;
+    return (int)rowbins_row_cap(GL.nb, capacity);
+}
+
+int gsr_track_forward_backward_dual_static_xf_scan(const gsr_settings* settings, const gsr_gaussians* gaussians,
+                                                   float* colors2, const gsr_track_xform* xform, int capacity,
+                                                   unsigned* status, float* out_color, float* out_color2,
+                                                   float* out_depth, int* radii, const float* gt_im,
+                                                   const float* gt_depth, float sil_thres, float w_im, float w_depth,
+                                                   const float* dL_dloss, float* loss, float* terms, float* scratch,
+                                                   float* inst_records, gsr_alloc_fn alloc, void* alloc_ctx,
+                                                   void* stream) {
+    FwdCall c = fwd_call(settings, gaussians, out_color, out_depth, radii, alloc, alloc_ctx, stream);
+    c.scan_binning = true;
+    return track_forward_backward_xf(
+        c, colors2, out_color2, xform, capacity, status, inst_records,
         TrackL1{gt_im, gt_depth, sil_thres, w_im, w_depth, dL_dloss, nullptr, nullptr, scratch, loss, terms});
 }
 
diff --git a/splatam_amd/csrc/gsr_forward.hip b/splatam_amd/csrc/gsr_forward.hip
--- a/splatam_amd/csrc/gsr_forward.hip
+++ b/splatam_amd/csrc/gsr_forward.hip
@@ -48,7 +48,7 @@
 }
 #endif
 
-int track_l1_fused_scratch_floats(int ntiles) { return 2 * ntiles + ARRIVE_GROUPED_WORDS; }
+int track_l1_fused_scratch_floats(int ntiles) { return 2 * ntiles + ARRIVE_GROUPED_WORDS + 2 * ntiles; }
 
 hipError_t launch_render_fwd(const Camera& cam, const uint2* ranges, uint64_t* point_list,
                              uint64_t* keys, GeomPtrs geo,
diff --git a/splatam_amd/csrc/gsr_launch.h b/splatam_amd/csrc/gsr_launch.h
--- a/splatam_amd/csrc/gsr_launch.h
+++ b/splatam_amd/csrc/gsr_launch.h
@@ -6,6 +6,8 @@
 
 hipError_t launch_preprocess(const Camera& cam, const GaussIn& g, GeomPtrs geo, int* radii, uint32_t* counts,
                              bool lds_hist, int ntiles, int nb, hipStream_t s, unsigned long long* clk = nullptr);
+hipError_t launch_preprocess_rowbins(const Camera& cam, const GaussIn& g, GeomPtrs geo, int* radii, int ntiles, int nb,
+                                     const RowBins& rb, hipStream_t s, unsigned long long* clk = nullptr);
 hipError_t launch_mark_visible(int P, const float* means3D, const float* view, uint8_t* vis, hipStream_t s);
 hipError_t launch_tile_colscan(uint32_t* counts, int nb, int ntiles, uint32_t* tot, GeomPtrs geo, uint2* ranges,
                                uint32_t* status, bool tail, hipStream_t s, unsigned long long* clk = nullptr,
@@ -52,6 +54,10 @@
                                GeomPtrs geo, float* final_T, uint32_t* n_contrib, float* out_color,
                                float* out_color2, float* out_depth, SpecGuard guard, const TrackL1& l1, float* inst,
                                hipStream_t s, unsigned long long* clk = nullptr);
+hipError_t launch_render_track_rowbins(const Camera& cam, uint64_t* point_list, GeomPtrs geo, float* final_T,
+                                       uint32_t* n_contrib, float* out_color, float* out_color2, float* out_depth,
+                                       SpecGuard guard, const TrackL1& l1, float* inst, const RowBins& rb,
+                                       hipStream_t s, unsigned long long* clk = nullptr);
 int track_records_stride();
 struct RecLayout {
     int stride;
diff --git a/splatam_amd/csrc/gsr_layout.h b/splatam_amd/csrc/gsr_layout.h
--- a/splatam_amd/csrc/gsr_layout.h
+++ b/splatam_amd/csrc/gsr_layout.h
@@ -166,6 +166,23 @@
     const uint32_t nt = (uint32_t)(cam.gx * cam.gy);
     return max(1u, (uint32_t)(4ull * counters[0] / (nt ? nt : 1u)));
 }
+constexpr int ROWBINS_MAX_TILES = 4096, ROWBINS_MAX_ROWS = 1024, ROWBINS_MAX_ROW_CAP = 65535;
+struct RowBins {
+    uint32_t* words = nullptr;
+    uint64_t* keys = nullptr;
+    uint32_t row_cap = 0;
+    uint32_t* acc = nullptr;
+    uint32_t* lens = nullptr;
+    uint32_t* plan = nullptr;
+    uint32_t* status = nullptr;
+    uint32_t* counters = nullptr;
+    uint64_t* sort_scratch = nullptr;
+    int rows = 0;
+};
+__host__ __device__ inline uint32_t rowbins_row_cap(int rows, int capacity) {
+    const uint32_t rc = (uint32_t)(capacity / (rows > 0 ? rows : 1));
+    return rc < (uint32_t)ROWBINS_MAX_ROW_CAP ? rc : (uint32_t)ROWBINS_MAX_ROW_CAP;
+}
 __device__ __forceinline__ int sched_tile(const Camera& cam) {
     return cam.tile_order ? (int)cam.tile_order[blockIdx.x] : (int)blockIdx.x;
 }
diff --git a/splatam_amd/csrc/gsr_preprocess.hip b/splatam_amd/csrc/gsr_preprocess.hip
--- a/splatam_amd/csrc/gsr_preprocess.hip
+++ b/splatam_amd/csrc/gsr_preprocess.hip
@@ -4,16 +4,26 @@
 #include "gsr_launch.h"
 #include "gsr_layout.h"
 #include "gsr_math.h"
+#include "gsr_tile_plan.h"
 #include "gsr_wave.h"
 
 namespace gsr {
 
-template <bool LDS_HIST, bool XF, bool CLK, bool EXACT>
-__global__ void __launch_bounds__(PRE_BLOCK)
-preprocess_kernel(Camera cam, GaussIn g, GeomPtrs geo, int* radii, uint32_t* __restrict__ counts, int ntiles,
-                  unsigned long long* clk) {
+template <bool LDS_HIST, bool XF, bool CLK, bool EXACT, bool RB = false>
+__device__ __forceinline__ void preprocess_body(const Camera& cam, const GaussIn& g, const GeomPtrs& geo, int* radii,
+                                                uint32_t* __restrict__ counts, int ntiles, unsigned long long* clk,
+                                                const RowBins& rb) {
 #pragma clang fp contract(off)
+    static_assert(!RB || (LDS_HIST && XF && !EXACT), "row-local bins: the fused tracking forward only");
     if (cam.gate.off()) return;
+    if constexpr (RB) {
+        if (blockIdx.x == gridDim.x - 1) {
+            __shared__ uint32_t s_plan[PLAN_BUCKETS], s_pw[PRE_BLOCK / 64];
+            if (blockDim.x == 512) tile_plan<512>(rb.lens, ntiles, cam.sched_cus, rb.plan, s_plan, s_pw);
+            else tile_plan<1024>(rb.lens, ntiles, cam.sched_cus, rb.plan, s_plan, s_pw);
+            return;
+        }
+    }
     if constexpr (CLK) kclock_begin(clk);
     extern __shared__ uint32_t s_hist[];
     __shared__ float s_pose[16];
@@ -49,6 +59,7 @@
     if (LDS_HIST || XF) __syncthreads();
     if (i == 0) geo.counters[4] = 0u;
     uint32_t tiles = 0, culled = 0;
+    [[maybe_unused]] uint32_t rb_lo = 0, rb_hi = 0, rb_live = 0, rb_z = 0;
     bool violation = false;
     float4 q0, q1, q2, q3;
     if (i < g.P) {
@@ -142,6 +153,9 @@
                 }
                 if constexpr (EXACT) culled = culled_below(live, tiles);
                 geo.bin[i] = make_uint4(rlo, rhi, __float_as_uint(pv.z), live);
+                if constexpr (RB) {
+                    rb_lo = rlo; rb_hi = rhi; rb_live = live; rb_z = __float_as_uint(pv.z);
+                }
                 if (!g.sh_staged && !g.colors) geo.clamp[i] = clamped;
                 for (int ty = y0, k = 0; ty < y1; ty++)
                     for (int tx = x0; tx < x1; tx++, k++) {
@@ -191,9 +205,84 @@
             geo.wgcull[blockIdx.x] = cw;
         }
     }
-    if (LDS_HIST)
+    if constexpr (RB) {
+        const uint32_t row = blockIdx.x, nrows = gridDim.x - 1, nw = blockDim.x >> 6;
+        uint32_t rowtot = 0;
+        for (uint32_t k = 0; k < nw; k++) rowtot += wsum[k];
+        const bool rowovf = rowtot > rb.row_cap;
+        if (i < g.P) geo.offsets[i] = row * rb.row_cap + (woff + incl - tiles);
+        __shared__ uint32_t s_ts[PRE_BLOCK / 64];
+        const int per = (ntiles + (int)blockDim.x - 1) / (int)blockDim.x;
+        const int t0 = min(ntiles, (int)threadIdx.x * per), t1 = min(ntiles, t0 + per);
+        uint32_t sum = 0;
+        for (int t = t0; t < t1; t++) sum += s_hist[t];
+        const uint32_t tincl = wave_incl_scan(sum);
+        if (lane == 63) s_ts[wv] = tincl;
+        __syncthreads();
+        uint32_t run = tincl - sum;
+        for (int k = 0; k < wv; k++) run += s_ts[k];
+        for (int t = t0; t < t1; t++) {
+            const uint32_t v = s_hist[t];
+            s_hist[t] = run;
+            run += v;
+        }
+        __syncthreads();
+        if (tiles && !rowovf) {
+            const int x0 = (int)(rb_lo & 0xFFFFu), y0 = (int)(rb_lo >> 16), x1 = (int)(rb_hi & 0xFFFFu),
+                      y1 = (int)(rb_hi >> 16);
+            const uint64_t key = ((uint64_t)rb_z << 32) | (uint64_t)(uint32_t)i;
+            uint64_t* const kr = rb.keys + (size_t)row * rb.row_cap;
+            for (int ty = y0, k = 0; ty < y1; ty++)
+                for (int tx = x0; tx < x1; tx++, k++) {
+                    if (!tile_live(rb_live, (uint32_t)k)) continue;
+                    kr[atomicAdd(&s_hist[ty * cam.gx + tx], 1u)] = key;
+                }
+        }
+        __syncthreads();
+        for (int t = threadIdx.x; t < ntiles; t += blockDim.x) {
+            const uint32_t prev = t ? s_hist[t - 1] : 0u, cur = s_hist[t];
+            rb.words[(size_t)row * ntiles + t] = rowovf ? 0u : (prev << 16) | (cur - prev);
+        }
+        if (threadIdx.x == blockDim.x - 1) {
+            geo.blocksums[row] = row * rb.row_cap;
+            const uint32_t flags = (viol ? 1u : 0u) | (rowovf ? 2u : 0u);
+            if (flags) {
+                atomicOr(rb.acc + 4, flags);
+                __threadfence();
+            }
+            constexpr unsigned long long kArrive = 1ull << 40;
+            unsigned long long* const acc = reinterpret_cast<unsigned long long*>(rb.acc + 2);
+            const unsigned long long old = atomicAdd(acc, kArrive | (unsigned long long)rowtot);
+            if ((old >> 40) == (unsigned long long)(nrows - 1)) {
+                __threadfence();
+                const unsigned long long tot = (old & (kArrive - 1ull)) + rowtot;
+                const uint32_t f = atomicExch(rb.acc + 4, 0u);
+                atomicExch(acc, 0ull);
+                const uint32_t n = tot > 0x7fffffffull ? 0x7fffffffu : (uint32_t)tot;
+                const uint32_t longest = (f & 2u) ? 0x7fffffffu : 0u;
+                geo.counters[0] = n;
+                geo.counters[1] = f & 1u;
+                geo.counters[2] = longest;
+                geo.counters[3] = (uint32_t)TILE_SORT_CAP;
+                if (rb.status) status_merge(rb.status, n, f & 1u, longest, (uint32_t)TILE_SORT_CAP);
+            }
+        }
+    } else if (LDS_HIST) {
         for (int t = threadIdx.x; t < ntiles; t += blockDim.x) counts[(size_t)blockIdx.x * ntiles + t] = s_hist[t];
+    }
     if constexpr (CLK) kclock_end(clk);
+}
+template <bool LDS_HIST, bool XF, bool CLK, bool EXACT>
+__global__ void __launch_bounds__(PRE_BLOCK)
+preprocess_kernel(Camera cam, GaussIn g, GeomPtrs geo, int* radii, uint32_t* __restrict__ counts, int ntiles,
+                  unsigned long long* clk) {
+    preprocess_body<LDS_HIST, XF, CLK, EXACT>(cam, g, geo, radii, counts, ntiles, clk, RowBins{});
+}
+template <bool CLK>
+__global__ void __launch_bounds__(PRE_BLOCK)
+preprocess_rowbins_kernel(Camera cam, GaussIn g, GeomPtrs geo, int* radii, int ntiles, unsigned long long* clk,
+                          RowBins rb) {
+    preprocess_body<true, true, CLK, false, true>(cam, g, geo, radii, nullptr, ntiles, clk, rb);
 }
 
 struct PickPreprocess {
@@ -212,6 +301,15 @@
     return hipGetLastError();
 }
 
+hipError_t launch_preprocess_rowbins(const Camera& cam, const GaussIn& g, GeomPtrs geo, int* radii, int ntiles, int nb,
+                                     const RowBins& rb, hipStream_t s, unsigned long long* clk) {
+    if (nb == 0) return hipSuccess;
+    const auto k = clk ? &preprocess_rowbins_kernel<true> : &preprocess_rowbins_kernel<false>;
+    hipLaunchKernelGGL(k, dim3(nb + 1), dim3(1 << cam.pre_shift), sizeof(uint32_t) * ntiles, s, cam, g, geo, radii,
+                       ntiles, clk, rb);
+    return hipGetLastError();
+}
+
 __global__ void mark_visible_kernel(int P, const float* __restrict__ means3D, const float* __restrict__ view,
                                     uint8_t* __restrict__ vis) {
     const int i = blockIdx.x * blockDim.x + threadIdx.x;
diff --git a/splatam_amd/csrc/gsr_render_bwd.h b/splatam_amd/csrc/gsr_render_bwd.h
--- a/splatam_amd/csrc/gsr_render_bwd.h
+++ b/splatam_amd/csrc/gsr_render_bwd.h
@@ -170,7 +170,8 @@
                                          const uint2* __restrict__ ranges, const PointEntry* __restrict__ point_list,
                                          const float4* __restrict__ rr, const uint32_t* __restrict__ blocksums,
                                          float* __restrict__ inst, const BwdGuard& guard, char* smem,
-                                         RenderDiag& dg) {
+                                         RenderDiag& dg, bool has_range = false,
+                                         uint2 range_in = uint2{0u, 0u}) {
     constexpr bool DUAL = V::DUAL, OPAC = V::OPAC, COL1 = V::COL1, COL2 = V::COL2, M2D1 = V::M2D1;
     constexpr int Q2 = V::Q2, MOM = V::MOM, C1 = V::C1;
     using L = BwdShape<V>;
@@ -192,7 +193,7 @@
     const int px = tx * TILE_X + tile_px(tid);
     const int py = ty * TILE_Y + tile_py(tid);
     const float x0 = (float)(tx * TILE_X), y0 = (float)(ty * TILE_Y);
-    const uint2 range = ranges[tile];
+    const uint2 range = has_range ? range_in : ranges[tile];
     const float T_final = pin.T_final;
     const uint32_t last = pin.last;
     const float dp0 = pin.dp0, dp1 = pin.dp1, dp2 = pin.dp2, dq0 = pin.dq0, dq1 = pin.dq1, dq2 = pin.dq2;
diff --git a/splatam_amd/csrc/gsr_render_fwd.h b/splatam_amd/csrc/gsr_render_fwd.h
--- a/splatam_amd/csrc/gsr_render_fwd.h
+++ b/splatam_amd/csrc/gsr_render_fwd.h
@@ -77,13 +77,13 @@
     else if constexpr (LK < LOGN) bitonic_net<E, LK + 1, LK>(v, base, sk);
 }
 
-template <int E, typename Emit>
+template <int E, bool LDS1 = false, typename Emit>
 __device__ void tile_sort_regs(const uint64_t* __restrict__ src, uint32_t cnt, Emit emit, uint64_t* sk) {
     static_assert(E == 1 || E == 2 || E == 4, "256 x E keys");
     const uint32_t base = threadIdx.x * E;
     uint64_t v[E];
 #pragma unroll
-    for (int e = 0; e < E; e++) v[e] = base + e < cnt ? src[base + e] : ~0ull;
+    for (int e = 0; e < E; e++) v[e] = base + e < cnt ? (LDS1 ? sk[base + e] : src[base + e]) : ~0ull;
     bitonic_net<E, 1, 0>(v, base, sk);
 #pragma unroll
     for (int e = 0; e < E; e++)
@@ -93,6 +93,7 @@
 #if GSR_FWD_ABLATE == 7
 static __device__ uint16_t g_fab_mask[1u << 23];
 #endif
+template <bool LDS1 = false>
 __device__ __forceinline__ void tile_sort_bucket(uint64_t* __restrict__ src, uint32_t cnt,
                                                  PointEntry* __restrict__ dst, uint64_t* sk) {
     auto emit = [&](uint32_t i, uint32_t gi) { dst[i] = (PointEntry)gi; };
@@ -101,15 +102,15 @@
         return;
     }
     if (cnt <= 1) {
-        if (cnt == 1 && threadIdx.x == 0) emit(0, (uint32_t)src[0]);
+        if (cnt == 1 && threadIdx.x == 0) emit(0, (uint32_t)(LDS1 ? sk[0] : src[0]));
         return;
     }
     if (cnt <= 256) {
-        tile_sort_regs<1>(src, cnt, emit, sk);
+        tile_sort_regs<1, LDS1>(src, cnt, emit, sk);
         return;
     }
     if (cnt <= 512) {
-        tile_sort_regs<2>(src, cnt, emit, sk);
+        tile_sort_regs<2, LDS1>(src, cnt, emit, sk);
         return;
     }
     const uint32_t nch = (cnt + TILE_SORT_REGS - 1) / TILE_SORT_REGS;
@@ -118,7 +119,8 @@
         const uint32_t c0 = c * TILE_SORT_REGS, len = min(TILE_SORT_REGS, cnt - c0);
         uint64_t v[4];
 #pragma unroll
-        for (int e = 0; e < 4; e++) v[e] = base + e < len ? src[c0 + base + e] : ~0ull;
+        for (int e = 0; e < 4; e++)
+            v[e] = base + e < len ? ((LDS1 && nch == 1) ? sk[base + e] : src[c0 + base + e]) : ~0ull;
         bitonic_net<4, 1, 0>(v, base, sk);
 #pragma unroll
         for (int e = 0; e < 4; e++) {
@@ -177,11 +179,64 @@
     uint32_t last16;
 };
 
-template <bool DUAL>
+constexpr int ROWBINS_RPT = ROWBINS_MAX_ROWS / TILE_SORT_THREADS;
+__device__ __forceinline__ uint32_t rowbins_gather(const RowBins& rb, int tile, int ntiles, uint64_t* sk) {
+    __shared__ uint32_t s_gw[TILE_SORT_THREADS / 64];
+    const int tid = threadIdx.x, lane = tid & 63, w = tid >> 6;
+    uint32_t wd[ROWBINS_RPT], c = 0;
+#pragma unroll
+    for (int k = 0; k < ROWBINS_RPT; k++) {
+        const int row = tid + k * TILE_SORT_THREADS;
+        wd[k] = row < rb.rows ? rb.words[(size_t)row * ntiles + tile] : 0u;
+    }
+#pragma unroll
+    for (int k = 0; k < ROWBINS_RPT; k++) c += wd[k] & 0xFFFFu;
+    const uint32_t incl = wave_incl_scan(c);
+    if (lane == 63) s_gw[w] = incl;
+    __syncthreads();
+    uint32_t pos = incl - c, total = 0;
+#pragma unroll
+    for (int k = 0; k < TILE_SORT_THREADS / 64; k++) {
+        pos += k < w ? s_gw[k] : 0u;
+        total += s_gw[k];
+    }
+    if (tid == 0 && rb.status && total > rb.status[2]) atomicMax(rb.status + 2, total);
+    if (total > (uint32_t)TILE_SORT_CAP) {
+        if (tid == 0) {
+            atomicMax(rb.counters + 2, total);
+        }
+        __syncthreads();
+        return 0u;
+    }
+    uint64_t k0[ROWBINS_RPT];
+#pragma unroll
+    for (int k = 0; k < ROWBINS_RPT; k++) {
+        const size_t at = (size_t)(tid + k * TILE_SORT_THREADS) * rb.row_cap + (wd[k] >> 16);
+        k0[k] = (wd[k] & 0xFFFFu) ? rb.keys[at] : 0ull;
+    }
+    auto put = [&](uint64_t* dst) {
+        uint32_t at = pos;
+#pragma unroll
+        for (int k = 0; k < ROWBINS_RPT; k++) {
+            const uint32_t n = wd[k] & 0xFFFFu;
+            if (n == 0u) continue;
+            const uint64_t* kr = rb.keys + (size_t)(tid + k * TILE_SORT_THREADS) * rb.row_cap + (wd[k] >> 16);
+            dst[at] = k0[k];
+            for (uint32_t j = 1; j < n; j++) dst[at + j] = kr[j];
+            at += n;
+        }
+    };
+    if (total <= TILE_SORT_REGS) put(sk);
+    else put(rb.sort_scratch + (size_t)tile * TILE_SORT_CAP);
+    __syncthreads();
+    return total;
+}
+
+template <bool DUAL, bool RB = false>
 __device__ __forceinline__ FwdPix fwd_tile(const Camera& cam, int tile, const uint2* __restrict__ ranges,
                                            PointEntry* __restrict__ point_list, uint64_t* __restrict__ keys,
                                            const float4* __restrict__ rr, const SpecGuard& guard, char* smem,
-                                           RenderDiag& dg) {
+                                           RenderDiag& dg, const RowBins& rb = RowBins{}, uint2* range_out = nullptr) {
     using L = FwdShape<DUAL>;
     constexpr int LS = L::LS;
     float4* const s_ab = reinterpret_cast<float4*>(smem + L::o_ab);
@@ -198,7 +253,19 @@
     const float x0 = (float)(tx * TILE_X), y0 = (float)(ty * TILE_Y);
     const bool inside = px < cam.W && py < cam.H;
     const v2f pix = v2f{(float)px, (float)py};
-    const uint2 range = ranges[tile];
+    uint2 range;
+    if constexpr (RB) {
+        uint64_t* const sk = reinterpret_cast<uint64_t*>(smem + L::o_ab);
+        const uint32_t n = rowbins_gather(rb, tile, cam.gx * cam.gy, sk);
+        range.x = (uint32_t)tile * (uint32_t)TILE_SORT_CAP;
+        range.y = range.x + n;
+        if (threadIdx.x == 0) rb.lens[tile] = n;
+        *range_out = range;
+        tile_sort_bucket<true>(rb.sort_scratch + (size_t)tile * TILE_SORT_CAP, n, point_list + range.x, sk);
+        __syncthreads();
+    } else {
+        range = ranges[tile];
+    }
     bool done = !inside;
     float T = 1.f, C2 = 0.f, D = 15.0f;
     float C5 = 0.f;
@@ -206,7 +273,7 @@
     uint32_t last16 = 0;
     float4 pa = make_float4(0.f, 0.f, 0.f, 0.f), pb = pa, pc = pa, pd = pa;
     uint32_t pg = 0, pgn = 0;
-    if (keys != nullptr) {
+    if (!RB && keys != nullptr) {
         tile_sort_bucket(keys + range.x, range.y - range.x, point_list + range.x,
                          reinterpret_cast<uint64_t*>(s_ab));
         __syncthreads();
diff --git a/splatam_amd/csrc/gsr_tile_plan.h b/splatam_amd/csrc/gsr_tile_plan.h
--- /dev/null
+++ b/splatam_amd/csrc/gsr_tile_plan.h
@@ -0,0 +1,68 @@
+#pragma once
+#include "gsr_layout.h"
+#include "gsr_wave.h"
+
+namespace gsr {
+
+constexpr int PLAN_BUCKETS = 1024, PLAN_SHIFT = 2;
+__device__ __forceinline__ uint32_t plan_bucket(uint32_t len) {
+    return (uint32_t)(PLAN_BUCKETS - 1) - min(len >> PLAN_SHIFT, (uint32_t)(PLAN_BUCKETS - 1));
+}
+__device__ __forceinline__ uint32_t plan_slot(uint32_t p, uint32_t n, uint32_t ncu) {
+    const uint32_t q = n / ncu, m = n - q * ncu, heavy = q * (ncu - m);
+    const bool hv = p < heavy;
+    const uint32_t g0 = hv ? m : 0u, gs = hv ? ncu - m : m, pp = hv ? p : p - heavy;
+    const uint32_t rd = pp / gs, k = pp - rd * gs;
+    return rd * ncu + g0 + ((rd & 1u) ? gs - 1u - k : k);
+}
+template <int NT, int TPT = 0>
+__device__ void tile_plan(const uint32_t* __restrict__ tot, int ntiles, int ncu, uint32_t* __restrict__ order,
+                          uint32_t* s_hist, uint32_t* s_wsum, const uint32_t* tv = nullptr, int t0 = 0,
+                          int t1 = 0) {
+    constexpr int BPT = PLAN_BUCKETS / NT;
+    static_assert(BPT * NT == PLAN_BUCKETS, "buckets per thread");
+    const int tid = threadIdx.x, lane = tid & 63, w = tid >> 6;
+#pragma unroll
+    for (int k = 0; k < BPT; k++) s_hist[tid * BPT + k] = 0u;
+    __syncthreads();
+    if constexpr (TPT > 0) {
+#pragma unroll
+        for (int k = 0; k < TPT; k++)
+            if (t0 + k < t1) atomicAdd(&s_hist[plan_bucket(tv[k])], 1u);
+    } else {
+        for (int u = tid; u < ntiles; u += NT) atomicAdd(&s_hist[plan_bucket(tot[u])], 1u);
+    }
+    __syncthreads();
+    uint32_t c[BPT], cs = 0;
+#pragma unroll
+    for (int k = 0; k < BPT; k++) {
+        c[k] = s_hist[tid * BPT + k];
+        cs += c[k];
+    }
+    const uint32_t incl = wave_incl_scan(cs);
+    if (lane == 63) s_wsum[w] = incl;
+    __syncthreads();
+    uint32_t run = incl - cs;
+    for (int k = 0; k < w; k++) run += s_wsum[k];
+#pragma unroll
+    for (int k = 0; k < BPT; k++) {
+        s_hist[tid * BPT + k] = run;
+        run += c[k];
+    }
+    __syncthreads();
+    if constexpr (TPT > 0) {
+#pragma unroll
+        for (int k = 0; k < TPT; k++)
+            if (t0 + k < t1) {
+                const uint32_t p = atomicAdd(&s_hist[plan_bucket(tv[k])], 1u);
+                order[plan_slot(p, (uint32_t)ntiles, (uint32_t)ncu)] = (uint32_t)(t0 + k);
+            }
+    } else {
+        for (int u = tid; u < ntiles; u += NT) {
+            const uint32_t p = atomicAdd(&s_hist[plan_bucket(tot[u])], 1u);
+            order[plan_slot(p, (uint32_t)ntiles, (uint32_t)ncu)] = (uint32_t)u;
+        }
+    }
+}
+
+}
```
